# H2muller/CROPSR

Hardware: NVIDIA B200
Metric: genome Gbp/s scanned+scored (higher is better)
Workload: dtype f64

## Files before the change

### cropsr_b200/csrc/cropsr_b200.cu

```cuda

#include <cuda_runtime.h>
#include <stdint.h>
#include <stdio.h>
#include <stdarg.h>
#include <string.h>
#include <stdlib.h>
#include <algorithm>
#include <atomic>
#include <mutex>
#include <new>
#include <type_traits>
#include <utility>
#include <vector>

#include "../../include/cropsr_b200.h"

#ifndef CRP_CTAS_PER_SM
#define CRP_CTAS_PER_SM 4
#endif
#include "scan.cuh"
#include "primers.cuh"
#include "extras.cuh"
#include "offtarget.cuh"

#define CRP_ABI_VERSION 10

static constexpr size_t kScanSmemFixed = (size_t)kStages * kRecBytes + 2 * (size_t)kListCap * sizeof(uint16_t);

static thread_local char g_err[512] = "";
static int fail(int code, const char *fmt, ...) {
    va_list ap;
    va_start(ap, fmt);
    vsnprintf(g_err, sizeof g_err, fmt, ap);
    va_end(ap);
    return code;
}
#define CUDA_TRY(expr)                                                                      \
    do {                                                                                    \
        cudaError_t e_ = (expr);                                                            \
        if (e_ != cudaSuccess)                                                              \
            return fail(CRP_ERR_CUDA, "%s failed: %s (%s:%d)", #expr, cudaGetErrorString(e_), \
                        __FILE__, __LINE__);                                                \
    } while (0)

struct Context {
    bool ready = false;
    int device = -1;
    int sm_count = 0;
    cudaStream_t stream = nullptr;
    cudaStream_t lanes[3] = {nullptr, nullptr, nullptr};
    cudaStream_t lane_out = nullptr;
    std::atomic<uint64_t> launches{0};
    double *d_tables = nullptr;
    unsigned int *d_fault = nullptr;
};
static Context g_ctx;

struct Perf {
    std::atomic<uint64_t> commits{0}, scans{0}, sharded_scans{0}, fused_exchanges{0}, capacity_reruns{0};
    std::atomic<uint64_t> positions{0}, candidates{0}, h2d_bytes{0}, d2h_bytes{0}, cache_hits{0}, cache_misses{0};
    double ms_h2d = 0, ms_pack = 0, ms_scan = 0, ms_kernel = 0;
};
static Perf g_perf;

struct Segment {
    uint32_t token_id;
    const uint8_t *token;
    uint64_t token_len, begin, end;
    uint64_t stage_begin, stage_end;
    uint32_t first_tile, n_tiles;
    const uint8_t *raw = nullptr;
    uint64_t raw_bytes = 0;
    uint32_t width = 0, last = 0;
    uint64_t ascii_off = 0;
};

struct crp_genome {
    std::vector<Segment> segs;
    cudaStream_t st = nullptr;
    cudaEvent_t ev[3] = {nullptr, nullptr, nullptr};
    bool committed = false;
    uint64_t n_positions = 0;
    uint4 *records = nullptr;
    unsigned char *pam = nullptr;
    TileHdr *hdr = nullptr;
    uint32_t n_tiles = 0;
    uint32_t *d_seg_first = nullptr, *d_seg_count = nullptr;
    float ms_h2d = 0.f, ms_pack = 0.f;
    uint8_t *d_ascii = nullptr;
    bool fasta = false;
    unsigned int *h_bad = nullptr;
};

struct crp_result {
    const crp_genome *g = nullptr;
    cudaStream_t st = nullptr;
    cudaEvent_t ev[3] = {nullptr, nullptr, nullptr};
    cudaEvent_t ev_kernel = nullptr;
    unsigned long long *h_counts = nullptr;
    uint32_t stride = 0;
    unsigned long long *d_gather = nullptr;
    unsigned long long *h_gather = nullptr;
    bool fused = false;
    uint32_t epoch = 0;
    unsigned int *h_xchg_error = nullptr;
    float ms_kernel = 0.f;
    int guide_len = 0;
    uint32_t flags = 0;
    uint64_t capacity = 0;
    uint64_t n_plus = 0, n_minus = 0;
    bool scored = false;
    uint32_t *pos[2] = {nullptr, nullptr};
    unsigned long long *packed[2] = {nullptr, nullptr};
    double *x[2] = {nullptr, nullptr};
    unsigned char *state = nullptr;
    size_t state_bytes = 0, zero_offset = 0;
    unsigned long long *d_counts = nullptr;
    std::vector<uint64_t> seg_plus, seg_minus;
    float ms_scan = 0.f;
    uint32_t n_launches = 0;
};

#include <chrono>
struct Trace {
    const char *what;
    bool on;
    std::chrono::steady_clock::time_point t0;
    explicit Trace(const char *w) : what(w), on(getenv("CRP_TRACE") != nullptr), t0(std::chrono::steady_clock::now()) {}
    void lap(const char *stage) {
        if (!on) return;
        const auto t1 = std::chrono::steady_clock::now();
        fprintf(stderr, "[crp] %s: %s %.3f ms\n", what, stage, std::chrono::duration<double, std::milli>(t1 - t0).count());
        t0 = t1;
    }
};

static int need_ctx() {
    if (!g_ctx.ready) return fail(CRP_ERR_STATE, "crp_init has not been called");
    return 0;
}

struct DevBlock {
    void *ptr;
    size_t bytes;
    cudaEvent_t ev;
};
static std::vector<DevBlock> g_dev_free;
static std::vector<DevBlock> g_dev_live;
static std::mutex g_mem_mu;
template <typename T>
static cudaError_t dev_alloc(T **ptr, size_t bytes, cudaStream_t st) {
    std::lock_guard<std::mutex> lock(g_mem_mu);
    const size_t want = (bytes ? bytes : 16) + 255 & ~(size_t)255;
    size_t best = g_dev_free.size(), busy = g_dev_free.size();
    for (size_t i = 0; i < g_dev_free.size(); ++i) {
        const size_t b = g_dev_free[i].bytes;
        if (b < want || b - want > want / 8 + 4096) continue;
        if (cudaEventQuery(g_dev_free[i].ev) == cudaSuccess) {
            best = i;
            break;
        } else {
            cudaGetLastError();
            if (busy == g_dev_free.size() || b < g_dev_free[busy].bytes) busy = i;
        }
    }
    DevBlock blk;
    if (best < g_dev_free.size()) {
        blk = g_dev_free[best];
        g_dev_free.erase(g_dev_free.begin() + best);
        g_perf.cache_hits++;
    } else if (cudaMalloc(&blk.ptr, want) == cudaSuccess) {
        g_perf.cache_misses++;
        blk.bytes = want;
        if (cudaError_t e = cudaEventCreateWithFlags(&blk.ev, cudaEventDisableTiming)) {
            cudaFree(blk.ptr);
            return e;
        }
    } else if (busy < g_dev_free.size()) {
        cudaGetLastError();
        blk = g_dev_free[busy];
        g_dev_free.erase(g_dev_free.begin() + busy);
        if (cudaError_t e = cudaStreamWaitEvent(st, blk.ev, 0)) return e;
    } else {
        cudaGetLastError();
        blk.bytes = want;
        if (cudaMalloc(&blk.ptr, want) != cudaSuccess) {
            cudaGetLastError();
            cudaDeviceSynchronize();
            for (DevBlock &b : g_dev_free) {
                cudaFree(b.ptr);
                cudaEventDestroy(b.ev);
            }
            g_dev_free.clear();
            if (cudaError_t e = cudaMalloc(&blk.ptr, want)) return e;
        }
        if (cudaError_t e = cudaEventCreateWithFlags(&blk.ev, cudaEventDisableTiming)) {
            cudaFree(blk.ptr);
            return e;
        }
    }
    g_dev_live.push_back(blk);
    *ptr = reinterpret_cast<T *>(blk.ptr);
    return cudaSuccess;
}
static void dev_free(void *ptr, cudaStream_t st) {
    if (!ptr) return;
    std::lock_guard<std::mutex> lock(g_mem_mu);
    for (size_t i = g_dev_live.size(); i-- > 0;)
        if (g_dev_live[i].ptr == ptr) {
            DevBlock blk = g_dev_live[i];
            g_dev_live.erase(g_dev_live.begin() + i);
            cudaEventRecord(blk.ev, st);
            g_dev_free.push_back(blk);
            return;
        }
}
static void dev_cache_release() {
    std::lock_guard<std::mutex> lock(g_mem_mu);
    for (DevBlock &b : g_dev_free) {
        cudaFree(b.ptr);
        cudaEventDestroy(b.ev);
    }
    g_dev_free.clear();
}

static std::vector<std::pair<size_t, void *>> g_pinned_free;
static void *pinned_get(size_t bytes) {
    std::lock_guard<std::mutex> lock(g_mem_mu);
    for (size_t i = 0; i < g_pinned_free.size(); ++i)
        if (g_pinned_free[i].first >= bytes) {
            void *p = g_pinned_free[i].second;
            g_pinned_free.erase(g_pinned_free.begin() + i);
            return p;
        }
    const size_t want = bytes < 4096 ? 4096 : bytes;
    void *p = nullptr;
    if (cudaHostAlloc(&p, want + sizeof(size_t) * 2, cudaHostAllocMapped) != cudaSuccess) return nullptr;
    *reinterpret_cast<size_t *>(p) = want;
    return reinterpret_cast<char *>(p) + sizeof(size_t) * 2;
}
static void pinned_put(void *p) {
    if (!p) return;
    std::lock_guard<std::mutex> lock(g_mem_mu);
    const size_t cap = *reinterpret_cast<size_t *>(reinterpret_cast<char *>(p) - sizeof(size_t) * 2);
    g_pinned_free.emplace_back(cap, p);
}


#include <dlfcn.h>
#include <nccl.h>
struct Comm {
    void *dl = nullptr;
    ncclComm_t comm = nullptr;
    int rank = 0, world = 1;
    ncclResult_t (*GetUniqueId)(ncclUniqueId *) = nullptr;
    ncclResult_t (*CommInitRank)(ncclComm_t *, int, ncclUniqueId, int) = nullptr;
    ncclResult_t (*CommDestroy)(ncclComm_t) = nullptr;
    ncclResult_t (*AllGather)(const void *, void *, size_t, ncclDataType_t, ncclComm_t, cudaStream_t) = nullptr;
    ncclResult_t (*AllReduce)(const void *, void *, size_t, ncclDataType_t, ncclRedOp_t, ncclComm_t, cudaStream_t) = nullptr;
    const char *(*GetErrorString)(ncclResult_t) = nullptr;
    unsigned long long *d_scratch = nullptr;
    unsigned char *xchg = nullptr;
    unsigned char *peer[kMaxPeers] = {};
    bool fused = false;
    int mode = 0;
    uint32_t epoch = 0;
    char why_not_fused[160] = "";
};
static Comm g_comm;
static constexpr uint32_t kXchgSlots = 32768;
static size_t xchg_gather_bytes() { return (size_t)2 * kMaxPeers * 2 * kXchgSlots * sizeof(unsigned long long); }
static size_t xchg_bytes() { return xchg_gather_bytes() + 2 * kMaxPeers * sizeof(unsigned int) + 64; }
static unsigned long long *xchg_gather(unsigned char *base, uint32_t parity, uint32_t world, uint32_t stride) {
    (void)world;
    (void)stride;
    return reinterpret_cast<unsigned long long *>(base) + (size_t)parity * kMaxPeers * 2 * kXchgSlots;
}
static unsigned int *xchg_flags(unsigned char *base, uint32_t parity) {
    return reinterpret_cast<unsigned int *>(base + xchg_gather_bytes()) + (size_t)parity * kMaxPeers;
}
static unsigned int *xchg_error(unsigned char *base) {
    return reinterpret_cast<unsigned int *>(base + xchg_gather_bytes()) + 2 * kMaxPeers;
}

static int comm_load() {
    if (g_comm.dl) return 0;
    const char *names[] = {getenv("CRP_NCCL_LIB"), "libnccl.so.2", "libnccl.so"};
    for (const char *n : names) {
        if (!n) continue;
        if ((g_comm.dl = dlopen(n, RTLD_NOW | RTLD_GLOBAL))) break;
    }
    if (!g_comm.dl) return fail(CRP_ERR_STATE, "libnccl.so.2 not found: %s", dlerror());
#define CRP_NCCL_SYM(field, name)                                                         \
    if (!(*(void **)(&g_comm.field) = dlsym(g_comm.dl, name))) {                          \
        dlclose(g_comm.dl);                                                               \
        g_comm.dl = nullptr;                                                              \
        return fail(CRP_ERR_STATE, "NCCL symbol %s missing", name);                       \
    }
    CRP_NCCL_SYM(GetUniqueId, "ncclGetUniqueId")
    CRP_NCCL_SYM(CommInitRank, "ncclCommInitRank")
    CRP_NCCL_SYM(CommDestroy, "ncclCommDestroy")
    CRP_NCCL_SYM(AllGather, "ncclAllGather")
    CRP_NCCL_SYM(AllReduce, "ncclAllReduce")
    CRP_NCCL_SYM(GetErrorString, "ncclGetErrorString")
#undef CRP_NCCL_SYM
    return 0;
}
#define NCCL_TRY(expr)                                                                                \
    do {                                                                                              \
        ncclResult_t e_ = (expr);                                                                     \
        if (e_ != ncclSuccess) return fail(CRP_ERR_CUDA, "%s failed: %s", #expr, g_comm.GetErrorString(e_)); \
    } while (0)

static int comm_allgather_u64(const unsigned long long *send, unsigned long long *recv, size_t count, cudaStream_t st) {
    if (!g_comm.comm) return fail(CRP_ERR_STATE, "crp_comm_init has not been called");
    NCCL_TRY(g_comm.AllGather(send, recv, count, ncclUint64, g_comm.comm, st));
    return 0;
}

extern "C" {

int crp_result_free(crp_result *r);
int crp_comm_shutdown(void);


int crp_abi_version(void) { return CRP_ABI_VERSION; }

int crp_tile_size(void) { return kTile; }

int crp_checked_build(void) {
#ifdef CRP_CHECKED
    return 1;
#else
    return 0;
#endif
}

const char *crp_last_error(void) { return g_err; }

int crp_debug_set_times(void *dev_ptr) {
    unsigned long long *p = (unsigned long long *)dev_ptr;
    CUDA_TRY(cudaMemcpyToSymbol(g_dbg_times, &p, sizeof p));
    return 0;
}

int crp_device_count(int *count) {
    if (!count) return fail(CRP_ERR_ARG, "count is NULL");
    CUDA_TRY(cudaGetDeviceCount(count));
    return 0;
}

int crp_init(int device) {
    if (g_ctx.ready) {
        if (g_ctx.device == device) return 0;
        return fail(CRP_ERR_STATE, "already initialised on device %d", g_ctx.device);
    }
    CUDA_TRY(cudaSetDevice(device));
    cudaDeviceProp prop;
    CUDA_TRY(cudaGetDeviceProperties(&prop, device));
    if (prop.major != 10)
        return fail(CRP_ERR_CUDA, "device %d is sm_%d%d; this library is built for sm_100a only", device,
                    prop.major, prop.minor);
    CUDA_TRY(cudaStreamCreateWithFlags(&g_ctx.stream, cudaStreamNonBlocking));
    {
        std::vector<double> tab;
        char msg[128];
        if (build_rs1_tables(tab, msg, sizeof msg)) return fail(CRP_ERR_STATE, "%s", msg);
        CUDA_TRY(cudaMalloc(&g_ctx.d_tables, tab.size() * sizeof(double)));
        CUDA_TRY(cudaMemcpy(g_ctx.d_tables, tab.data(), tab.size() * sizeof(double), cudaMemcpyHostToDevice));
    }
#ifdef CRP_CHECKED
    CUDA_TRY(cudaMalloc(&g_ctx.d_fault, sizeof(unsigned int)));
    CUDA_TRY(cudaMemset(g_ctx.d_fault, 0, sizeof(unsigned int)));
#endif
    g_ctx.device = device;
    g_ctx.sm_count = prop.multiProcessorCount;
    g_ctx.launches = 0;
    g_ctx.ready = true;
    return 0;
}

int crp_shutdown(void) {
    if (!g_ctx.ready) return 0;
    crp_comm_shutdown();
    cudaStreamSynchronize(g_ctx.stream);
    cudaDeviceSynchronize();
    dev_cache_release();
    {
        std::lock_guard<std::mutex> lock(g_mem_mu);
        for (auto &pf : g_pinned_free) cudaFreeHost(reinterpret_cast<char *>(pf.second) - sizeof(size_t) * 2);
        g_pinned_free.clear();
    }
    cudaStreamDestroy(g_ctx.stream);
    for (cudaStream_t l : g_ctx.lanes)
        if (l) cudaStreamDestroy(l);
    if (g_ctx.lane_out) cudaStreamDestroy(g_ctx.lane_out);
    cudaFree(g_ctx.d_tables);
    if (g_ctx.d_fault) cudaFree(g_ctx.d_fault);
    g_ctx.d_fault = nullptr;
    g_ctx.ready = false;
    g_ctx.device = -1;
    g_ctx.stream = nullptr;
    for (cudaStream_t &l : g_ctx.lanes) l = nullptr;
    g_ctx.lane_out = nullptr;
    g_ctx.d_tables = nullptr;
    g_ctx.launches = 0;
    return 0;
}

int crp_perf_report(char *buf, uint64_t capacity, uint64_t *needed) {
    char tmp[1536];
    size_t live = 0, idle = 0, live_bytes = 0, idle_bytes = 0;
    {
        std::lock_guard<std::mutex> lock(g_mem_mu);
        live = g_dev_live.size();
        idle = g_dev_free.size();
        for (const DevBlock &b : g_dev_live) live_bytes += b.bytes;
        for (const DevBlock &b : g_dev_free) idle_bytes += b.bytes;
    }
    const int n = snprintf(
        tmp, sizeof tmp,
        "{\"abi\": %d, \"checked_build\": %d, \"device\": %d, \"sm_count\": %d, \"kernel_launches\": %llu, "
        "\"commits\": %llu, \"scans\": %llu, \"sharded_scans\": %llu, \"fused_exchanges\": %llu, \"capacity_reruns\": %llu, "
        "\"positions_packed\": %llu, \"candidates\": %llu, \"h2d_token_bytes\": %llu, \"d2h_row_bytes\": %llu, "
        "\"ms_h2d\": %.4f, \"ms_pack\": %.4f, \"ms_scan\": %.4f, \"ms_scan_kernels\": %.4f, "
        "\"comm\": {\"rank\": %d, \"world\": %d, \"fused_exchange\": %s}, "
        "\"block_cache\": {\"live_blocks\": %zu, \"live_bytes\": %zu, \"idle_blocks\": %zu, \"idle_bytes\": %zu, \"hits\": %llu, \"misses\": %llu}}",
        CRP_ABI_VERSION, crp_checked_build(), g_ctx.device, g_ctx.sm_count, (unsigned long long)g_ctx.launches.load(),
        (unsigned long long)g_perf.commits.load(), (unsigned long long)g_perf.scans.load(),
        (unsigned long long)g_perf.sharded_scans.load(), (unsigned long long)g_perf.fused_exchanges.load(),
        (unsigned long long)g_perf.capacity_reruns.load(), (unsigned long long)g_perf.positions.load(),
        (unsigned long long)g_perf.candidates.load(), (unsigned long long)g_perf.h2d_bytes.load(),
        (unsigned long long)g_perf.d2h_bytes.load(), g_perf.ms_h2d, g_perf.ms_pack, g_perf.ms_scan, g_perf.ms_kernel,
        g_comm.comm ? g_comm.rank : 0, g_comm.comm ? g_comm.world : 1, g_comm.comm && g_comm.fused && g_comm.mode == 0 ? "true" : "false",
        live, live_bytes, idle, idle_bytes, (unsigned long long)g_perf.cache_hits.load(), (unsigned long long)g_perf.cache_misses.load());
    if (needed) *needed = (uint64_t)n + 1;
    if (!buf || capacity < (uint64_t)n + 1) return fail(CRP_ERR_RANGE, "perf report needs %d bytes", n + 1);
    memcpy(buf, tmp, (size_t)n + 1);
    return 0;
}

int crp_launch_count(uint64_t *n) {
    if (!n) return fail(CRP_ERR_ARG, "n is NULL");
    *n = g_ctx.launches;
    return 0;
}

int crp_comm_unique_id(uint8_t *id) {
    if (!id) return fail(CRP_ERR_ARG, "id is NULL");
    if (int rc = comm_load()) return rc;
    ncclUniqueId u;
    NCCL_TRY(g_comm.GetUniqueId(&u));
    static_assert(sizeof u == CRP_COMM_ID_BYTES, "ncclUniqueId size");
    memcpy(id, &u, sizeof u);
    return 0;
}

int crp_comm_init(int rank, int world, const uint8_t *id) {
    if (int rc = need_ctx()) return rc;
    if (!id || world < 1 || rank < 0 || rank >= world) return fail(CRP_ERR_ARG, "bad rank %d / world %d", rank, world);
    if (g_comm.comm) return fail(CRP_ERR_STATE, "communicator already initialised (rank %d of %d)", g_comm.rank, g_comm.world);
    if (int rc = comm_load()) return rc;
    ncclUniqueId u;
    memcpy(&u, id, sizeof u);
    CUDA_TRY(cudaSetDevice(g_ctx.device));
    NCCL_TRY(g_comm.CommInitRank(&g_comm.comm, world, u, rank));
    g_comm.rank = rank;
    g_comm.world = world;
    CUDA_TRY(cudaMalloc(&g_comm.d_scratch, 2 * sizeof(unsigned long long)));
    CUDA_TRY(cudaMemset(g_comm.d_scratch, 0, 2 * sizeof(unsigned long long)));
    g_comm.epoch = 0;
    g_comm.mode = 0;
    if (const char *e = getenv("CRP_COMM_EXCHANGE")) g_comm.mode = !strcmp(e, "nccl") ? 1 : 0;
    g_comm.fused = false;
    g_comm.why_not_fused[0] = 0;
    bool ok = world <= kMaxPeers;
    if (!ok) snprintf(g_comm.why_not_fused, sizeof g_comm.why_not_fused, "world %d > %d", world, kMaxPeers);
    cudaIpcMemHandle_t mine;
    memset(&mine, 0, sizeof mine);
    if (ok) {
        if (cudaMalloc(&g_comm.xchg, xchg_bytes()) != cudaSuccess || cudaMemset(g_comm.xchg, 0, xchg_bytes()) != cudaSuccess ||
            cudaIpcGetMemHandle(&mine, g_comm.xchg) != cudaSuccess) {
            snprintf(g_comm.why_not_fused, sizeof g_comm.why_not_fused, "exchange buffer / IPC handle: %s",
                     cudaGetErrorString(cudaGetLastError()));
            ok = false;
        }
    }
    static_assert(sizeof(cudaIpcMemHandle_t) == 64, "IPC handle size");
    std::vector<uint64_t> handles((size_t)world * 8);
    {
        unsigned long long *d = nullptr;
        CUDA_TRY(cudaMalloc(&d, ((size_t)world + 1) * 64));
        CUDA_TRY(cudaMemcpy(d, &mine, 64, cudaMemcpyHostToDevice));
        NCCL_TRY(g_comm.AllGather(d, d + 8, 8, ncclUint64, g_comm.comm, g_ctx.stream));
        CUDA_TRY(cudaStreamSynchronize(g_ctx.stream));
        CUDA_TRY(cudaMemcpy(handles.data(), d + 8, (size_t)world * 64, cudaMemcpyDeviceToHost));
        cudaFree(d);
    }
    for (int q = 0; q < world && ok; ++q) {
        if (q == rank) {
            g_comm.peer[q] = g_comm.xchg;
            continue;
        }
        cudaIpcMemHandle_t h;
        memcpy(&h, &handles[(size_t)q * 8], 64);
        void *ptr = nullptr;
        if (cudaIpcOpenMemHandle(&ptr, h, cudaIpcMemLazyEnablePeerAccess) != cudaSuccess) {
            snprintf(g_comm.why_not_fused, sizeof g_comm.why_not_fused, "cudaIpcOpenMemHandle(rank %d): %s", q,
                     cudaGetErrorString(cudaGetLastError()));
            ok = false;
        } else {
            g_comm.peer[q] = static_cast<unsigned char *>(ptr);
        }
    }
    {
        unsigned long long v = ok ? 0ull : 1ull;
        CUDA_TRY(cudaMemcpy(g_comm.d_scratch, &v, sizeof v, cudaMemcpyHostToDevice));
        NCCL_TRY(g_comm.AllReduce(g_comm.d_scratch, g_comm.d_scratch + 1, 1, ncclUint64, ncclSum, g_comm.comm, g_ctx.stream));
        CUDA_TRY(cudaStreamSynchronize(g_ctx.stream));
        CUDA_TRY(cudaMemcpy(&v, g_comm.d_scratch + 1, sizeof v, cudaMemcpyDeviceToHost));
        CUDA_TRY(cudaMemset(g_comm.d_scratch, 0, 2 * sizeof(unsigned long long)));
        if (v && ok) snprintf(g_comm.why_not_fused, sizeof g_comm.why_not_fused, "%llu other rank(s) could not map the buffers", v);
        g_comm.fused = v == 0;
    }
    return 0;
}

int crp_comm_set_exchange(int mode) {
    if (mode != 0 && mode != 1) return fail(CRP_ERR_ARG, "mode must be 0 (fused) or 1 (nccl)");
    g_comm.mode = mode;
    return 0;
}

int crp_comm_exchange_info(int *fused, const char **why) {
    if (fused) *fused = g_comm.comm && g_comm.fused && g_comm.mode == 0 ? 1 : 0;
    if (why) *why = g_comm.mode == 1 ? "NCCL exchange selected" : g_comm.why_not_fused;
    return 0;
}

int crp_comm_info(int *rank, int *world) {
    if (rank) *rank = g_comm.comm ? g_comm.rank : 0;
    if (world) *world = g_comm.comm ? g_comm.world : 1;
    return 0;
}

int crp_comm_barrier(void) {
    if (int rc = need_ctx()) return rc;
    CUDA_TRY(cudaDeviceSynchronize());
    if (!g_comm.comm) return 0;
    NCCL_TRY(g_comm.AllReduce(g_comm.d_scratch, g_comm.d_scratch + 1, 1, ncclUint64, ncclSum, g_comm.comm, g_ctx.stream));
    CUDA_TRY(cudaStreamSynchronize(g_ctx.stream));
    return 0;
}

int crp_comm_max_f64(double *v, uint32_t n) {
    if (int rc = need_ctx()) return rc;
    if (!v && n) return fail(CRP_ERR_ARG, "v is NULL");
    if (!g_comm.comm || n == 0) return 0;
    double *d = nullptr;
    CUDA_TRY(dev_alloc(&d, n * sizeof(double), g_ctx.stream));
    CUDA_TRY(cudaMemcpyAsync(d, v, n * sizeof(double), cudaMemcpyHostToDevice, g_ctx.stream));
    NCCL_TRY(g_comm.AllReduce(d, d, n, ncclDouble, ncclMax, g_comm.comm, g_ctx.stream));
    CUDA_TRY(cudaMemcpyAsync(v, d, n * sizeof(double), cudaMemcpyDeviceToHost, g_ctx.stream));
    CUDA_TRY(cudaStreamSynchronize(g_ctx.stream));
    dev_free(d, g_ctx.stream);
    return 0;
}

int crp_comm_sum_f64(double *v, uint32_t n) {
    if (int rc = need_ctx()) return rc;
    if (!v && n) return fail(CRP_ERR_ARG, "v is NULL");
    if (!g_comm.comm || n == 0) return 0;
    double *d = nullptr;
    CUDA_TRY(dev_alloc(&d, n * sizeof(double), g_ctx.stream));
    CUDA_TRY(cudaMemcpyAsync(d, v, n * sizeof(double), cudaMemcpyHostToDevice, g_ctx.stream));
    NCCL_TRY(g_comm.AllReduce(d, d, n, ncclDouble, ncclSum, g_comm.comm, g_ctx.stream));
    CUDA_TRY(cudaMemcpyAsync(v, d, n * sizeof(double), cudaMemcpyDeviceToHost, g_ctx.stream));
    CUDA_TRY(cudaStreamSynchronize(g_ctx.stream));
    dev_free(d, g_ctx.stream);
    return 0;
}

int crp_comm_allgather_u64(const uint64_t *in, uint32_t n, uint64_t *out) {
    if (int rc = need_ctx()) return rc;
    if (n && (!in || !out)) return fail(CRP_ERR_ARG, "NULL argument");
    if (n == 0) return 0;
    if (!g_comm.comm) {
        memcpy(out, in, n * sizeof(uint64_t));
        return 0;
    }
    unsigned long long *d = nullptr;
    const size_t w = (size_t)g_comm.world;
    CUDA_TRY(dev_alloc(&d, (w + 1) * n * sizeof(uint64_t), g_ctx.stream));
    CUDA_TRY(cudaMemcpyAsync(d, in, n * sizeof(uint64_t), cudaMemcpyHostToDevice, g_ctx.stream));
    if (int rc = comm_allgather_u64(d, d + n, n, g_ctx.stream)) {
        dev_free(d, g_ctx.stream);
        return rc;
    }
    CUDA_TRY(cudaMemcpyAsync(out, d + n, w * n * sizeof(uint64_t), cudaMemcpyDeviceToHost, g_ctx.stream));
    CUDA_TRY(cudaStreamSynchronize(g_ctx.stream));
    dev_free(d, g_ctx.stream);
    return 0;
}

int crp_link_probe(uint64_t h2d_bytes, uint64_t d2h_bytes, uint32_t reps, float *ms) {
    if (int rc = need_ctx()) return rc;
    if (!ms || !reps) return fail(CRP_ERR_ARG, "bad argument");
    void *h_in = nullptr, *h_out = nullptr;
    unsigned char *d_in = nullptr, *d_out = nullptr;
    cudaStream_t s2 = nullptr;
    int rc = 0;
    do {
        if (cudaHostAlloc(&h_in, h2d_bytes + 16, cudaHostAllocDefault) != cudaSuccess ||
            cudaHostAlloc(&h_out, d2h_bytes + 16, cudaHostAllocDefault) != cudaSuccess) {
            rc = fail(CRP_ERR_NOMEM, "cudaHostAlloc of the probe buffers failed");
            break;
        }
        memset(h_in, 1, h2d_bytes + 16);
        memset(h_out, 1, d2h_bytes + 16);
        if (dev_alloc(&d_in, h2d_bytes + 16, g_ctx.stream) != cudaSuccess || dev_alloc(&d_out, d2h_bytes + 16, g_ctx.stream) != cudaSuccess ||
            cudaStreamCreateWithFlags(&s2, cudaStreamNonBlocking) != cudaSuccess) {
            rc = fail(CRP_ERR_NOMEM, "device buffers of the link probe failed");
            break;
        }
        cudaStreamSynchronize(g_ctx.stream);
        double total = 0.0;
        for (uint32_t i = 0; i <= reps; ++i) {
            const auto t0 = std::chrono::steady_clock::now();
            cudaMemcpyAsync(d_in, h_in, h2d_bytes, cudaMemcpyHostToDevice, g_ctx.stream);
            cudaMemcpyAsync(h_out, d_out, d2h_bytes, cudaMemcpyDeviceToHost, s2);
            cudaStreamSynchronize(g_ctx.stream);
            cudaStreamSynchronize(s2);
            if (i) total += std::chrono::duration<double, std::milli>(std::chrono::steady_clock::now() - t0).count();
        }
        if (cudaGetLastError() != cudaSuccess) rc = fail(CRP_ERR_CUDA, "link probe copies failed");
        *ms = (float)(total / reps);
    } while (0);
    if (s2) cudaStreamDestroy(s2);
    dev_free(d_in, g_ctx.stream);
    dev_free(d_out, g_ctx.stream);
    if (h_in) cudaFreeHost(h_in);
    if (h_out) cudaFreeHost(h_out);
    return rc;
}

int crp_comm_shutdown(void) {
    if (g_comm.comm) {
        cudaDeviceSynchronize();
        g_comm.AllReduce(g_comm.d_scratch, g_comm.d_scratch + 1, 1, ncclUint64, ncclSum, g_comm.comm, g_ctx.stream);
        cudaStreamSynchronize(g_ctx.stream);
        for (int q = 0; q < g_comm.world && q < kMaxPeers; ++q)
            if (g_comm.peer[q] && q != g_comm.rank) cudaIpcCloseMemHandle(g_comm.peer[q]);
        for (auto &pp : g_comm.peer) pp = nullptr;
        if (g_comm.xchg) cudaFree(g_comm.xchg);
        g_comm.xchg = nullptr;
        g_comm.fused = false;
        g_comm.CommDestroy(g_comm.comm);
        cudaFree(g_comm.d_scratch);
        g_comm.comm = nullptr;
        g_comm.d_scratch = nullptr;
        g_comm.rank = 0;
        g_comm.world = 1;
    }
    return 0;
}

int crp_flush_l2(void) {
    if (int rc = need_ctx()) return rc;
    unsigned char *buf = nullptr;
    const size_t bytes = 512ull << 20;
    CUDA_TRY(dev_alloc(&buf, bytes, g_ctx.stream));
    cudaError_t e = cudaMemsetAsync(buf, 0, bytes, g_ctx.stream);
    dev_free(buf, g_ctx.stream);
    CUDA_TRY(e);
    CUDA_TRY(cudaStreamSynchronize(g_ctx.stream));
    return 0;
}

int crp_device_synchronize(void) {
    if (int rc = need_ctx()) return rc;
    CUDA_TRY(cudaDeviceSynchronize());
    return 0;
}

int crp_host_alloc(void **ptr, uint64_t bytes) {
    if (!ptr) return fail(CRP_ERR_ARG, "ptr is NULL");
    if (int rc = need_ctx()) return rc;
    CUDA_TRY(cudaHostAlloc(ptr, bytes ? bytes : 1, cudaHostAllocDefault));
    return 0;
}

int crp_host_free(void *ptr) {
    if (ptr) CUDA_TRY(cudaFreeHost(ptr));
    return 0;
}

static cudaStream_t stream_of(const crp_genome *g) { return g->st ? g->st : g_ctx.stream; }

int crp_genome_new(crp_genome **g) {
    if (!g) return fail(CRP_ERR_ARG, "g is NULL");
    if (int rc = need_ctx()) return rc;
    *g = new (std::nothrow) crp_genome();
    if (!*g) return fail(CRP_ERR_NOMEM, "out of host memory");
    return 0;
}

int crp_genome_add_segment(crp_genome *g, uint32_t token_id, const uint8_t *token_ascii,
                           uint64_t token_len, uint64_t seg_begin, uint64_t seg_end) {
    if (!g) return fail(CRP_ERR_ARG, "g is NULL");
    if (g->committed) return fail(CRP_ERR_STATE, "genome already committed");
    if (!token_ascii && token_len) return fail(CRP_ERR_ARG, "token_ascii is NULL");
    if (seg_begin > seg_end || seg_end > token_len)
        return fail(CRP_ERR_ARG, "segment [%llu,%llu) outside token of length %llu",
                    (unsigned long long)seg_begin, (unsigned long long)seg_end, (unsigned long long)token_len);
    if (seg_begin % kAlign) return fail(CRP_ERR_ARG, "seg_begin must be a multiple of %u", kAlign);
    if (token_len >= (1ull << 31) - (1ull << 15))
        return fail(CRP_ERR_RANGE, "token of %llu positions exceeds the 31-bit position range",
                    (unsigned long long)token_len);
    Segment s{};
    s.token_id = token_id;
    s.token = token_ascii;
    s.token_len = token_len;
    s.begin = seg_begin;
    s.end = seg_end;
    g->segs.push_back(s);
    return 0;
}

int crp_genome_add_fasta_record(crp_genome *g, uint32_t token_id, const uint8_t *seq_bytes, uint64_t n_bytes,
                                uint32_t line_width, int last_record) {
    if (!g) return fail(CRP_ERR_ARG, "g is NULL");
    if (g->committed) return fail(CRP_ERR_STATE, "genome already committed");
    if (!seq_bytes || !n_bytes || !line_width) return fail(CRP_ERR_FORMAT, "empty FASTA record");
    const uint64_t body = seq_bytes[n_bytes - 1] == '\n' ? n_bytes - 1 : n_bytes;
    const uint64_t k = body / ((uint64_t)line_width + 1), r = body % ((uint64_t)line_width + 1);
    if (r == 0) return fail(CRP_ERR_FORMAT, "FASTA record is not made of %u-base lines", line_width);
    const uint64_t n_bases = k * line_width + r, token_len = n_bases + 4;
    if (token_len >= (1ull << 31) - (1ull << 15))
        return fail(CRP_ERR_RANGE, "token of %llu positions exceeds the 31-bit position range",
                    (unsigned long long)token_len);
    Segment s{};
    s.token_id = token_id;
    s.token = nullptr;
    s.token_len = token_len;
    s.begin = 0;
    s.end = token_len;
    s.raw = seq_bytes;
    s.raw_bytes = n_bytes;
    s.width = line_width;
    s.last = last_record ? 1u : 0u;
    g->segs.push_back(s);
    g->fasta = true;
    return 0;
}

int crp_genome_token_length(const crp_genome *g, uint32_t segment, uint64_t *token_len) {
    if (!g || !token_len) return fail(CRP_ERR_ARG, "NULL argument");
    if (segment >= g->segs.size()) return fail(CRP_ERR_ARG, "segment %u out of range", segment);
    *token_len = g->segs[segment].token_len;
    return 0;
}

int crp_genome_fetch_token(const crp_genome *g, uint32_t segment, uint8_t *dst, uint64_t capacity) {
    if (!g || !dst) return fail(CRP_ERR_ARG, "NULL argument");
    if (int rc = need_ctx()) return rc;
    if (!g->committed || !g->d_ascii) return fail(CRP_ERR_STATE, "the genome keeps no tokens on the device");
    if (segment >= g->segs.size()) return fail(CRP_ERR_ARG, "segment %u out of range", segment);
    const Segment &s = g->segs[segment];
    if (!s.raw) return fail(CRP_ERR_STATE, "segment %u was not ingested from FASTA bytes", segment);
    if (capacity < s.token_len) return fail(CRP_ERR_RANGE, "token needs %llu bytes", (unsigned long long)s.token_len);
    cudaStream_t st = g->st ? g->st : g_ctx.stream;
    CUDA_TRY(cudaMemcpyAsync(dst, g->d_ascii + s.ascii_off, s.token_len, cudaMemcpyDeviceToHost, st));
    CUDA_TRY(cudaStreamSynchronize(st));
    return 0;
}

int crp_genome_release_tokens(crp_genome *g) {
    if (!g) return fail(CRP_ERR_ARG, "g is NULL");
    dev_free(g->d_ascii, g->st ? g->st : g_ctx.stream);
    g->d_ascii = nullptr;
    return 0;
}

int crp_genome_num_segments(const crp_genome *g, uint32_t *n) {
    if (!g || !n) return fail(CRP_ERR_ARG, "NULL argument");
    *n = (uint32_t)g->segs.size();
    return 0;
}

int crp_genome_num_positions(const crp_genome *g, uint64_t *n) {
    if (!g || !n) return fail(CRP_ERR_ARG, "NULL argument");
    *n = g->n_positions;
    return 0;
}

static int commit_enqueue(crp_genome *g) {
    cudaStream_t st = stream_of(g);
    const bool one = g->segs.size() == 1;
    std::vector<PackDesc> descs;
    std::vector<uint64_t> seg_ascii;
    std::vector<uint32_t> seg_first, seg_count;
    uint64_t ascii_bytes = 0, n_tiles = 0;
    g->n_positions = 0;
    for (size_t si = 0; si < g->segs.size(); ++si) {
        Segment &s = g->segs[si];
        s.stage_begin = s.begin >= 32 ? s.begin - 32 : 0;
        s.stage_end = s.end + 32 < s.token_len ? s.end + 32 : s.token_len;
        seg_ascii.push_back(ascii_bytes);
        s.first_tile = (uint32_t)n_tiles;
        s.n_tiles = (uint32_t)((s.end - s.begin + kTile - 1) / kTile);
        n_tiles += s.n_tiles;
        if (n_tiles >= (1ull << 31)) return fail(CRP_ERR_RANGE, "shard has too many tiles");
        for (uint32_t j = 0; j < (one ? (s.n_tiles ? 1u : 0u) : s.n_tiles); ++j) {
            const uint64_t t = s.begin + (uint64_t)j * kTile;
            PackDesc pd;
            pd.ascii_off = ascii_bytes;
            pd.stage_begin = (uint32_t)s.stage_begin;
            pd.stage_end = (uint32_t)s.stage_end;
            pd.td.t_start = (uint32_t)t;
            pd.td.L = (uint32_t)s.token_len;
            pd.td.n = (uint32_t)((s.end - t) < (uint64_t)kTile ? (s.end - t) : (uint64_t)kTile);
            pd.td.segment = (uint32_t)si;
            descs.push_back(pd);
        }
        seg_first.push_back(s.first_tile);
        seg_count.push_back(s.n_tiles);
        g->n_positions += s.end - s.begin;
        ascii_bytes += (s.stage_end - s.stage_begin + 15) / 16 * 16;
    }
    if (g->n_positions >= (1ull << 32))
        return fail(CRP_ERR_RANGE, "shard of %llu positions exceeds the 32-bit candidate count range",
                    (unsigned long long)g->n_positions);
    g->n_tiles = (uint32_t)n_tiles;
    g_perf.commits++;
    g_perf.positions += g->n_positions;
    g_perf.h2d_bytes += ascii_bytes;

    uint8_t *d_ascii = nullptr;
    PackDesc *d_descs = nullptr;
    const size_t rec_bytes = (size_t)g->n_tiles * kRecBytes;
    if (dev_alloc(&d_ascii, ascii_bytes + 64, st) != cudaSuccess ||
        (!one && dev_alloc(&d_descs, (descs.size() + 1) * sizeof(PackDesc), st) != cudaSuccess) ||
        dev_alloc(&g->records, rec_bytes + 16, st) != cudaSuccess ||
        dev_alloc(&g->pam, (size_t)g->n_tiles * kPamBytes + 16, st) != cudaSuccess ||
        dev_alloc(&g->hdr, ((size_t)g->n_tiles + 1) * sizeof(TileHdr), st) != cudaSuccess) {
        cudaGetLastError();
        dev_free(d_ascii, st);
        dev_free(d_descs, st);
        return fail(CRP_ERR_NOMEM, "cudaMalloc of %llu record bytes + %llu staging bytes failed",
                    (unsigned long long)rec_bytes, (unsigned long long)ascii_bytes);
    }
    for (int i = 0; i < 3; ++i)
        if (!g->ev[i]) CUDA_TRY(cudaEventCreate(&g->ev[i]));
    CUDA_TRY(cudaEventRecord(g->ev[0], st));
    uint8_t *d_raw = nullptr;
    FastaRec *d_recs = nullptr;
    unsigned int *d_bad = nullptr;
    std::vector<FastaRec> frecs;
    uint64_t raw_total = 0, strip_items = 0;
    for (size_t si = 0; si < g->segs.size(); ++si) {
        Segment &s = g->segs[si];
        s.ascii_off = seg_ascii[si];
        if (!s.raw) continue;
        FastaRec fr{};
        fr.raw_off = raw_total;
        fr.ascii_off = seg_ascii[si];
        fr.first_item = strip_items;
        fr.n_bases = (uint32_t)(s.token_len - 4);
        fr.width = s.width;
        fr.last = s.last;
        frecs.push_back(fr);
        raw_total += (s.raw_bytes + 15) / 16 * 16;
        strip_items += (s.token_len + 15) / 16;
    }
    if (!frecs.empty()) {
        if (dev_alloc(&d_raw, raw_total + 64, st) != cudaSuccess ||
            dev_alloc(&d_recs, frecs.size() * sizeof(FastaRec), st) != cudaSuccess ||
            dev_alloc(&d_bad, sizeof(unsigned int), st) != cudaSuccess) {
            cudaGetLastError();
            return fail(CRP_ERR_NOMEM, "cudaMalloc of %llu FASTA bytes failed", (unsigned long long)raw_total);
        }
        CUDA_TRY(cudaMemsetAsync(d_bad, 0, sizeof(unsigned int), st));
    }
    for (size_t si = 0, fi = 0; si < g->segs.size(); ++si) {
        const Segment &s = g->segs[si];
        if (s.raw) {
            CUDA_TRY(cudaMemcpyAsync(d_raw + frecs[fi++].raw_off, s.raw, s.raw_bytes, cudaMemcpyHostToDevice, st));
        } else if (s.stage_end > s.stage_begin && s.n_tiles) {
            CUDA_TRY(cudaMemcpyAsync(d_ascii + seg_ascii[si], s.token + s.stage_begin, s.stage_end - s.stage_begin,
                                     cudaMemcpyHostToDevice, st));
        }
    }
    if (!frecs.empty()) {
        CUDA_TRY(cudaMemcpyAsync(d_recs, frecs.data(), frecs.size() * sizeof(FastaRec), cudaMemcpyHostToDevice, st));
        const uint64_t want = (strip_items + 255) / 256, cap = (uint64_t)g_ctx.sm_count * 16;
        k_fasta_strip<<<(unsigned)(want < cap ? want : cap), 256, 0, st>>>(d_raw, d_recs, (uint32_t)frecs.size(),
                                                                           strip_items, d_ascii, d_bad);
        g_ctx.launches++;
        CUDA_TRY(cudaGetLastError());
        if (!g->h_bad) g->h_bad = static_cast<unsigned int *>(pinned_get(sizeof(unsigned int)));
        if (!g->h_bad) return fail(CRP_ERR_NOMEM, "cudaHostAlloc failed");
        *g->h_bad = 0;
        CUDA_TRY(cudaMemcpyAsync(g->h_bad, d_bad, sizeof(unsigned int), cudaMemcpyDeviceToHost, st));
        dev_free(d_raw, st);
        dev_free(d_recs, st);
        dev_free(d_bad, st);
    }
    if (!one && !descs.empty())
        CUDA_TRY(cudaMemcpyAsync(d_descs, descs.data(), descs.size() * sizeof(PackDesc), cudaMemcpyHostToDevice, st));
    CUDA_TRY(cudaEventRecord(g->ev[1], st));
    const uint64_t n_items = (uint64_t)g->n_tiles * kPackItems;
    if (n_items) {
        PackDesc first = descs[0];
        if (one) first.td.n = (uint32_t)(g->segs[0].end - g->segs[0].begin);
        const uint64_t want = (n_items + 255) / 256, cap = (uint64_t)g_ctx.sm_count * 16;
        CUDA_TRY(cudaMemsetAsync(g->hdr, 0, (size_t)g->n_tiles * sizeof(TileHdr), st));
        k_pack<<<(unsigned)(want < cap ? want : cap), 256, 0, st>>>(d_ascii, d_descs, first, n_items, g->records, g->pam, g->hdr);
        g_ctx.launches++;
        CUDA_TRY(cudaGetLastError());
    }
    CUDA_TRY(cudaEventRecord(g->ev[2], st));
    if (!one && !g->segs.empty()) {
        const size_t nb = g->segs.size() * sizeof(uint32_t);
        CUDA_TRY(dev_alloc(&g->d_seg_first, nb, st));
        CUDA_TRY(dev_alloc(&g->d_seg_count, nb, st));
        CUDA_TRY(cudaMemcpyAsync(g->d_seg_first, seg_first.data(), nb, cudaMemcpyHostToDevice, st));
        CUDA_TRY(cudaMemcpyAsync(g->d_seg_count, seg_count.data(), nb, cudaMemcpyHostToDevice, st));
    }
    if (g->fasta) g->d_ascii = d_ascii;
    else dev_free(d_ascii, st);
    dev_free(d_descs, st);
    g->committed = true;
    return 0;
}

int crp_genome_commit(crp_genome *g) {
    if (!g) return fail(CRP_ERR_ARG, "g is NULL");
    if (int rc = need_ctx()) return rc;
    if (g->committed) return fail(CRP_ERR_STATE, "genome already committed");
    Trace tr("commit");
    if (int rc = commit_enqueue(g)) return rc;
    tr.lap("enqueue");
    CUDA_TRY(cudaStreamSynchronize(stream_of(g)));
    tr.lap("sync");
    CUDA_TRY(cudaEventElapsedTime(&g->ms_h2d, g->ev[0], g->ev[1]));
    CUDA_TRY(cudaEventElapsedTime(&g->ms_pack, g->ev[1], g->ev[2]));
    g_perf.ms_h2d += g->ms_h2d;
    g_perf.ms_pack += g->ms_pack;
    for (Segment &s : g->segs) s.token = nullptr;
    if (g->h_bad && *g->h_bad)
        return fail(CRP_ERR_FORMAT, "a FASTA record is not plain fixed-width text; use the host ingest for this file");
    return 0;
}

int crp_genome_timing(const crp_genome *g, float *ms_h2d, float *ms_pack) {
    if (!g) return fail(CRP_ERR_ARG, "g is NULL");
    if (ms_h2d) *ms_h2d = g->ms_h2d;
    if (ms_pack) *ms_pack = g->ms_pack;
    return 0;
}

int crp_genome_free(crp_genome *g) {
    if (!g) return 0;
    cudaStream_t st = stream_of(g);
    dev_free(g->records, st);
    dev_free(g->pam, st);
    dev_free(g->hdr, st);
    dev_free(g->d_ascii, st);
    pinned_put(g->h_bad);
    dev_free(g->d_seg_first, st);
    dev_free(g->d_seg_count, st);
    for (cudaEvent_t e : g->ev)
        if (e) cudaEventDestroy(e);
    delete g;
    return 0;
}

static void free_streams(crp_result *r) {
    for (int s = 0; s < 2; ++s) {
        dev_free(r->pos[s], r->st);
        dev_free(r->packed[s], r->st);
        dev_free(r->x[s], r->st);
        r->pos[s] = nullptr;
        r->packed[s] = nullptr;
        r->x[s] = nullptr;
    }
}

static int alloc_streams(crp_result *r, uint64_t cap, bool scored) {
    r->capacity = cap;
    const uint64_t n = cap ? cap : 1;
    for (int s = 0; s < 2; ++s) {
        if (dev_alloc(&r->pos[s], n * sizeof(uint32_t), r->st) != cudaSuccess) goto oom;
        if (scored) {
            if (dev_alloc(&r->packed[s], n * sizeof(unsigned long long), r->st) != cudaSuccess) goto oom;
            if (dev_alloc(&r->x[s], n * sizeof(double), r->st) != cudaSuccess) goto oom;
        }
    }
    return 0;
oom:
    cudaGetLastError();
    free_streams(r);
    return fail(CRP_ERR_NOMEM, "cudaMalloc of candidate streams (%llu entries per strand) failed",
                (unsigned long long)cap);
}

struct ScanPlan {
    const void *fn;
    unsigned grid, threads;
    size_t smem;
};

static int plan_scan(const crp_genome *g, bool scored, ScanPlan *p) {
    p->threads = kThreads;
    p->fn = scored ? (const void *)k_scan_score<true> : (const void *)k_scan_score<false>;
    const unsigned grid_max = (unsigned)g_ctx.sm_count * CRP_CTAS_PER_SM;
    p->smem = kScanSmemFixed + (size_t)grid_max * sizeof(unsigned long long);
    static_assert(kScanSmemFixed >= (size_t)kHdrBatch * sizeof(TileHdr), "the count phase stages its tile headers in the emit phase's tile slots");
    static int per_sm_cache[2] = {0, 0};
    int &per_sm = per_sm_cache[scored ? 1 : 0];
    if (per_sm == 0) {
        CUDA_TRY(cudaFuncSetAttribute(p->fn, cudaFuncAttributeMaxDynamicSharedMemorySize, (int)p->smem));
        CUDA_TRY(cudaOccupancyMaxActiveBlocksPerMultiprocessor(&per_sm, p->fn, kThreads, p->smem));
        if (per_sm < 1) return fail(CRP_ERR_CUDA, "scan kernel does not fit on an SM");
        if (per_sm > CRP_CTAS_PER_SM) per_sm = CRP_CTAS_PER_SM;
    }
    uint64_t grid = (uint64_t)g_ctx.sm_count * per_sm;
    if (const char *e = getenv("CRP_SCAN_GRID")) {
        const long v = atol(e);
        if (v > 0 && (uint64_t)v < grid) grid = (uint64_t)v;
    }
    if (grid > g->n_tiles) grid = g->n_tiles;
    if (grid < 1) grid = 1;
    p->grid = (unsigned)grid;
    return 0;
}

static int launch_scan(const crp_genome *g, crp_result *r, const ScanPlan &p) {
    cudaStream_t st = r->st;
    ScanArgs a;
    a.records = g->records;
    a.pam = g->pam;
    a.hdr = g->hdr;
    a.n_tiles = g->n_tiles;
    a.static_eighths = 4;
    if (const char *e = getenv("CRP_STATIC_EIGHTHS")) a.static_eighths = (uint32_t)atoi(e) > 8 ? 8 : (uint32_t)atoi(e);
    a.guide_len = r->guide_len;
    a.flags = r->flags;
    a.tables = g_ctx.d_tables;
    a.capacity = r->capacity < 0xFFFFFFFFull ? r->capacity : 0xFFFFFFFFull;
    a.pos_plus = r->pos[0];
    a.pos_minus = r->pos[1];
    a.packed_plus = r->packed[0];
    a.packed_minus = r->packed[1];
    a.x_plus = r->x[0];
    a.x_minus = r->x[1];
    const uint32_t n_seg = (uint32_t)g->segs.size();
    unsigned long long *s64 = reinterpret_cast<unsigned long long *>(r->state);
    a.warp_pref = s64;
    a.cta_tot = s64 + (size_t)g->n_tiles * kPrefWords;
    a.seg_counts = r->d_counts;
    a.tickets = reinterpret_cast<unsigned int *>(r->d_counts + 2 * (size_t)r->stride);
    a.n_seg = n_seg;
    a.seg_stride = r->stride;
    a.seg_first_tile = g->d_seg_first;
    a.seg_tile_count = g->d_seg_count;
    a.seg_counts_host = r->h_counts;
    a.fault = g_ctx.d_fault;
    a.world = 1;
    a.rank = 0;
    a.epoch = 0;
    a.xchg_error = nullptr;
    a.xchg_timeout_ns = 20ull * 1000 * 1000 * 1000;
    for (int q = 0; q < kMaxPeers; ++q) {
        a.peer_gather[q] = nullptr;
        a.peer_flags[q] = nullptr;
    }
    const unsigned long long *gathered = r->d_gather;
    if (r->fused) {
        a.world = (uint32_t)g_comm.world;
        a.rank = (uint32_t)g_comm.rank;
        a.epoch = r->epoch;
        a.xchg_error = xchg_error(g_comm.xchg);
        if (const char *e = getenv("CRP_XCHG_TIMEOUT_MS")) a.xchg_timeout_ns = strtoull(e, nullptr, 10) * 1000000ull;
        for (int q = 0; q < g_comm.world; ++q) {
            a.peer_gather[q] = xchg_gather(g_comm.peer[q], r->epoch & 1u, a.world, r->stride);
            a.peer_flags[q] = xchg_flags(g_comm.peer[q], r->epoch & 1u);
        }
        gathered = xchg_gather(g_comm.xchg, r->epoch & 1u, a.world, r->stride);
    }
    CUDA_TRY(cudaEventRecord(r->ev[0], st));
    if (g->n_tiles) {
        void *params[] = {(void *)&a};
        CUDA_TRY(cudaLaunchCooperativeKernel(p.fn, dim3(p.grid), dim3(p.threads), params, p.smem, st));
        g_ctx.launches++;
        CUDA_TRY(cudaGetLastError());
    } else if (r->fused) {
        k_exchange_empty<<<1, 256, 0, st>>>(a);
        g_ctx.launches++;
        CUDA_TRY(cudaGetLastError());
    } else if (r->stride) {
        CUDA_TRY(cudaMemsetAsync(r->d_counts, 0, 2 * (size_t)r->stride * sizeof(unsigned long long), st));
        memset(r->h_counts, 0, 2 * (size_t)r->stride * sizeof(unsigned long long));
    }
    if (r->ev_kernel) CUDA_TRY(cudaEventRecord(r->ev_kernel, st));
    if (r->d_gather && !r->fused) {
        if (int rc = comm_allgather_u64(r->d_counts, r->d_gather, 2 * (size_t)r->stride, st)) return rc;
    }
    CUDA_TRY(cudaEventRecord(r->ev[1], st));
    if (r->h_gather && gathered)
        CUDA_TRY(cudaMemcpyAsync(r->h_gather, gathered, (size_t)g_comm.world * 2 * r->stride * sizeof(unsigned long long),
                                 cudaMemcpyDeviceToHost, st));
    if (r->fused)
        CUDA_TRY(cudaMemcpyAsync(r->h_xchg_error, xchg_error(g_comm.xchg), sizeof(unsigned int), cudaMemcpyDeviceToHost, st));
    CUDA_TRY(cudaEventRecord(r->ev[2], st));
    return 0;
}

static int scan_enqueue(crp_genome *g, int guide_len, uint32_t flags, crp_result **res, uint32_t slots = 0) {
    crp_result *r = new (std::nothrow) crp_result();
    if (!r) return fail(CRP_ERR_NOMEM, "out of host memory");
    r->g = g;
    r->st = stream_of(g);
    r->guide_len = guide_len;
    r->flags = flags;
    r->scored = guide_len == 20 && !(flags & CRP_SCAN_NO_SCORE);
    const uint32_t n_seg = (uint32_t)g->segs.size();
    int rc = 0;
    auto bail = [&](int code) {
        crp_result_free(r);
        return code;
    };
    ScanPlan plan = {};
    if ((rc = plan_scan(g, r->scored, &plan))) return bail(rc);
    r->stride = slots ? slots : n_seg;
    r->zero_offset = ((size_t)g->n_tiles * kPrefWords + (size_t)plan.grid) * sizeof(unsigned long long);
    r->state_bytes = r->zero_offset + 2 * (size_t)r->stride * sizeof(unsigned long long) +
                     4 * sizeof(unsigned int);
    if (dev_alloc(&r->state, r->state_bytes, r->st) != cudaSuccess)
        return bail(fail(CRP_ERR_NOMEM, "cudaMalloc of scan state failed"));
    r->d_counts = reinterpret_cast<unsigned long long *>(r->state + r->zero_offset);
    r->h_counts = static_cast<unsigned long long *>(pinned_get((2 * (size_t)r->stride + 1) * sizeof(unsigned long long)));
    if (!r->h_counts) return bail(fail(CRP_ERR_NOMEM, "cudaHostAlloc of the counts failed"));
    if (slots) {
        const size_t gb = (size_t)g_comm.world * 2 * slots * sizeof(unsigned long long);
        r->fused = g_comm.fused && g_comm.mode == 0 && slots <= kXchgSlots;
        r->epoch = ++g_comm.epoch;
        if (r->fused) {
            r->h_xchg_error = static_cast<unsigned int *>(pinned_get(sizeof(unsigned int)));
            if (!r->h_xchg_error) return bail(fail(CRP_ERR_NOMEM, "cudaHostAlloc failed"));
            *r->h_xchg_error = 0;
        }
        if (dev_alloc(&r->d_gather, gb, r->st) != cudaSuccess)
            return bail(fail(CRP_ERR_NOMEM, "cudaMalloc of the gathered counts failed"));
        r->h_gather = static_cast<unsigned long long *>(pinned_get(gb));
        if (!r->h_gather) return bail(fail(CRP_ERR_NOMEM, "cudaHostAlloc of the gathered counts failed"));
        if (cudaEventCreate(&r->ev_kernel) != cudaSuccess) return bail(fail(CRP_ERR_CUDA, "cudaEventCreate failed"));
    }
    if (cudaEventCreate(&r->ev[0]) != cudaSuccess || cudaEventCreate(&r->ev[1]) != cudaSuccess ||
        cudaEventCreateWithFlags(&r->ev[2], cudaEventDisableTiming) != cudaSuccess)
        return bail(fail(CRP_ERR_CUDA, "cudaEventCreate failed"));
    if ((rc = alloc_streams(r, g->n_positions / 8 + 4096, r->scored))) return bail(rc);
    if ((rc = launch_scan(g, r, plan))) return bail(rc);
    *res = r;
    return 0;
}

static int scan_finish(crp_genome *g, crp_result *r, cudaStream_t post = nullptr) {
    const uint32_t n_seg = (uint32_t)g->segs.size();
    for (int attempt = 0; attempt < 2; ++attempt) {
        if (cudaError_t e = cudaEventSynchronize(r->ev[2]))
            return fail(CRP_ERR_CUDA, "scan kernels failed: %s", cudaGetErrorString(e));
        r->n_plus = r->n_minus = 0;
        r->seg_plus.assign(n_seg, 0);
        r->seg_minus.assign(n_seg, 0);
        for (uint32_t s = 0; s < n_seg; ++s) {
            r->seg_plus[s] = r->h_counts[s];
            r->seg_minus[s] = r->h_counts[r->stride + s];
            r->n_plus += r->seg_plus[s];
            r->n_minus += r->seg_minus[s];
        }
        {
            float ms = 0.f;
            cudaEventElapsedTime(&ms, r->ev[0], r->ev[1]);
            r->ms_scan += ms;
            if (r->ev_kernel) cudaEventElapsedTime(&ms, r->ev[0], r->ev_kernel);
            r->ms_kernel += ms;
            r->n_launches++;
        }
#ifdef CRP_CHECKED
        {
            unsigned int fault = 0;
            cudaMemcpy(&fault, g_ctx.d_fault, sizeof fault, cudaMemcpyDeviceToHost);
            if (fault) {
                cudaMemset(g_ctx.d_fault, 0, sizeof fault);
                return fail(CRP_ERR_STATE, "checked build: kernel invariant %u violated (scan.cuh:%u)", fault & 0xFFu, fault >> 8);
            }
        }
#endif
        if (r->fused && *r->h_xchg_error)
            return fail(CRP_ERR_CUDA, "sharded scan: the counts of rank %u did not arrive (peer not scanning?)", *r->h_xchg_error - 1);
        const uint64_t need = r->n_plus > r->n_minus ? r->n_plus : r->n_minus;
        if (need <= r->capacity) break;
        if (attempt == 1) return fail(CRP_ERR_STATE, "candidate streams overflowed twice");
        r->fused = false;
        if (r->d_gather) {
            dev_free(r->d_gather, r->st);
            r->d_gather = nullptr;
        }
        free_streams(r);
        if (int rc = alloc_streams(r, need, r->scored)) return rc;
        ScanPlan plan = {};
        if (int rc = plan_scan(g, r->scored, &plan)) return rc;
        if (int rc = launch_scan(g, r, plan)) return rc;
    }
    g_perf.scans++;
    if (r->stride != (uint32_t)g->segs.size() || r->h_gather) g_perf.sharded_scans++;
    if (r->epoch && g_comm.fused && g_comm.mode == 0) g_perf.fused_exchanges++;
    g_perf.capacity_reruns += r->n_launches - 1;
    g_perf.candidates += r->n_plus + r->n_minus;
    g_perf.ms_scan += r->ms_scan;
    g_perf.ms_kernel += r->ms_kernel;
    if (r->scored && (r->flags & CRP_SCAN_LOGISTIC)) {
        const uint64_t n[2] = {r->n_plus, r->n_minus};
        for (int s = 0; s < 2; ++s)
            if (n[s]) {
                const uint64_t want = (n[s] + 255) / 256, cap = (uint64_t)g_ctx.sm_count * 16;
                k_logistic<<<(unsigned)(want < cap ? want : cap), 256, 0, post ? post : r->st>>>(r->x[s], n[s]);
                g_ctx.launches++;
            }
        CUDA_TRY(cudaGetLastError());
        CUDA_TRY(cudaEventRecord(r->ev[2], post ? post : r->st));
    }
    return 0;
}

int crp_scan_score(crp_genome *g, int guide_len, uint32_t flags, crp_result **res) {
    if (!g || !res) return fail(CRP_ERR_ARG, "NULL argument");
    if (int rc = need_ctx()) return rc;
    if (!g->committed) return fail(CRP_ERR_STATE, "genome not committed");
    if (guide_len < 1 || guide_len > 1000000) return fail(CRP_ERR_ARG, "guide_len %d out of range", guide_len);
    Trace tr("scan");
    crp_result *r = nullptr;
    if (int rc = scan_enqueue(g, guide_len, flags, &r)) return rc;
    tr.lap("enqueue");
    if (int rc = scan_finish(g, r)) {
        crp_result_free(r);
        return rc;
    }
    tr.lap("finish");
    *res = r;
    return 0;
}

int crp_scan_score_sharded(crp_genome *g, int guide_len, uint32_t flags, uint32_t slots, crp_result **res) {
    if (!g || !res) return fail(CRP_ERR_ARG, "NULL argument");
    if (int rc = need_ctx()) return rc;
    if (!g_comm.comm) return fail(CRP_ERR_STATE, "crp_comm_init has not been called");
    if (!g->committed) return fail(CRP_ERR_STATE, "genome not committed");
    if (guide_len < 1 || guide_len > 1000000) return fail(CRP_ERR_ARG, "guide_len %d out of range", guide_len);
    if (slots == 0 || slots < g->segs.size())
        return fail(CRP_ERR_ARG, "slots = %u is smaller than the %zu segments of this shard", slots, g->segs.size());
    crp_result *r = nullptr;
    if (int rc = scan_enqueue(g, guide_len, flags, &r, slots)) return rc;
    if (int rc = scan_finish(g, r)) {
        crp_result_free(r);
        return rc;
    }
    *res = r;
    return 0;
}

int crp_result_gathered_counts(const crp_result *res, uint64_t *counts) {
    if (!res || !counts) return fail(CRP_ERR_ARG, "NULL argument");
    if (!res->h_gather) return fail(CRP_ERR_STATE, "not the result of a sharded scan");
    memcpy(counts, res->h_gather, (size_t)g_comm.world * 2 * res->stride * sizeof(uint64_t));
    return 0;
}

static int rs1_rows(uint64_t n, const uint8_t *rows, const uint8_t *cls, double *score, int logistic);
int crp_rs1_score(uint64_t n, const uint8_t *rows, const uint8_t *cls, double *score) {
    return rs1_rows(n, rows, cls, score, 1);
}
int crp_rs1_preactivation(uint64_t n, const uint8_t *rows, const uint8_t *cls, double *x) {
    return rs1_rows(n, rows, cls, x, 0);
}
static int rs1_rows(uint64_t n, const uint8_t *rows, const uint8_t *cls, double *score, int logistic) {
    if (n && (!rows || !cls || !score)) return fail(CRP_ERR_ARG, "NULL argument");
    if (int rc = need_ctx()) return rc;
    if (!n) return 0;
    cudaStream_t st = g_ctx.stream;
    uint8_t *d_rows = nullptr;
    double *d_out = nullptr;
    if (dev_alloc(&d_rows, 31 * n, st) != cudaSuccess || dev_alloc(&d_out, n * sizeof(double), st) != cudaSuccess) {
        cudaGetLastError();
        dev_free(d_rows, st);
        return fail(CRP_ERR_NOMEM, "cudaMalloc for %llu rows failed", (unsigned long long)n);
    }
    CUDA_TRY(cudaMemcpyAsync(d_rows, rows, 30 * n, cudaMemcpyHostToDevice, st));
    CUDA_TRY(cudaMemcpyAsync(d_rows + 30 * n, cls, n, cudaMemcpyHostToDevice, st));
    k_rs1_rows<<<(unsigned)((n + 127) / 128), 128, 0, st>>>(d_rows, d_rows + 30 * n, n, d_out, logistic);
    g_ctx.launches++;
    CUDA_TRY(cudaGetLastError());
    CUDA_TRY(cudaMemcpyAsync(score, d_out, n * sizeof(double), cudaMemcpyDeviceToHost, st));
    dev_free(d_rows, st);
    dev_free(d_out, st);
    CUDA_TRY(cudaStreamSynchronize(st));
    return 0;
}

int crp_logistic(uint64_t n, const double *x, double *score) {
    if (n && (!x || !score)) return fail(CRP_ERR_ARG, "NULL argument");
    if (int rc = need_ctx()) return rc;
    if (!n) return 0;
    cudaStream_t st = g_ctx.stream;
    double *d = nullptr;
    if (dev_alloc(&d, n * sizeof(double), st) != cudaSuccess) {
        cudaGetLastError();
        return fail(CRP_ERR_NOMEM, "cudaMalloc of %llu doubles failed", (unsigned long long)n);
    }
    CUDA_TRY(cudaMemcpyAsync(d, x, n * sizeof(double), cudaMemcpyHostToDevice, st));
    const uint64_t want = (n + 255) / 256, cap = (uint64_t)g_ctx.sm_count * 16;
    k_logistic<<<(unsigned)(want < cap ? want : cap), 256, 0, st>>>(d, n);
    g_ctx.launches++;
    CUDA_TRY(cudaGetLastError());
    CUDA_TRY(cudaMemcpyAsync(score, d, n * sizeof(double), cudaMemcpyDeviceToHost, st));
    dev_free(d, st);
    CUDA_TRY(cudaStreamSynchronize(st));
    return 0;
}

int crp_result_totals(const crp_result *res, uint64_t *n_plus, uint64_t *n_minus) {
    if (!res) return fail(CRP_ERR_ARG, "res is NULL");
    if (n_plus) *n_plus = res->n_plus;
    if (n_minus) *n_minus = res->n_minus;
    return 0;
}

int crp_result_segment_counts(const crp_result *res, uint64_t *n_plus, uint64_t *n_minus) {
    if (!res) return fail(CRP_ERR_ARG, "res is NULL");
    for (size_t s = 0; s < res->seg_plus.size(); ++s) {
        if (n_plus) n_plus[s] = res->seg_plus[s];
        if (n_minus) n_minus[s] = res->seg_minus[s];
    }
    return 0;
}

int crp_result_device_counts(const crp_result *res, void **dev_ptr) {
    if (!res || !dev_ptr) return fail(CRP_ERR_ARG, "NULL argument");
    *dev_ptr = res->d_counts;
    return 0;
}

static int fetch_enqueue(const crp_result *res, int s, uint64_t first, uint64_t count, uint32_t *pos, uint64_t *packed,
                         double *x, cudaStream_t st = nullptr) {
    if (!st) st = res->st;
    g_perf.d2h_bytes += count * ((pos ? 4 : 0) + (packed ? 8 : 0) + (x ? 8 : 0));
    if (count) {
        if (pos) CUDA_TRY(cudaMemcpyAsync(pos, res->pos[s] + first, count * sizeof(uint32_t), cudaMemcpyDeviceToHost, st));
        if (packed)
            CUDA_TRY(cudaMemcpyAsync(packed, res->packed[s] + first, count * sizeof(uint64_t), cudaMemcpyDeviceToHost, st));
        if (x) CUDA_TRY(cudaMemcpyAsync(x, res->x[s] + first, count * sizeof(double), cudaMemcpyDeviceToHost, st));
    }
    return 0;
}

int crp_result_fetch(const crp_result *res, char strand, uint64_t first, uint64_t count, uint32_t *pos,
                     uint64_t *packed, double *x) {
    if (!res) return fail(CRP_ERR_ARG, "res is NULL");
    if (int rc = need_ctx()) return rc;
    if (strand != '+' && strand != '-') return fail(CRP_ERR_ARG, "strand must be '+' or '-'");
    const int s = strand == '+' ? 0 : 1;
    const uint64_t total = s == 0 ? res->n_plus : res->n_minus;
    if (first > total || count > total - first)
        return fail(CRP_ERR_ARG, "range [%llu,+%llu) outside stream of %llu candidates", (unsigned long long)first,
                    (unsigned long long)count, (unsigned long long)total);
    if ((packed || x) && !res->scored && count)
        return fail(CRP_ERR_STATE, "this result carries positions only (guide_len != 20 or CRP_SCAN_NO_SCORE)");
    if (int rc = fetch_enqueue(res, s, first, count, pos, packed, x)) return rc;
    CUDA_TRY(cudaStreamSynchronize(res->st));
    return 0;
}

int crp_result_timing(const crp_result *res, float *ms_scan) {
    if (!res) return fail(CRP_ERR_ARG, "res is NULL");
    if (ms_scan) *ms_scan = res->ms_scan;
    return 0;
}

int crp_result_timing_detail(const crp_result *res, float *ms_kernels, float *ms_total, uint32_t *n_launches) {
    if (!res) return fail(CRP_ERR_ARG, "res is NULL");
    if (ms_kernels) *ms_kernels = res->ms_kernel;
    if (ms_total) *ms_total = res->ms_scan;
    if (n_launches) *n_launches = res->n_launches;
    return 0;
}

int crp_result_free(crp_result *r) {
    if (!r) return 0;
    free_streams(r);
    dev_free(r->state, r->st);
    dev_free(r->d_gather, r->st);
    pinned_put(r->h_counts);
    pinned_put(r->h_gather);
    pinned_put(r->h_xchg_error);
    if (r->ev_kernel) cudaEventDestroy(r->ev_kernel);
    for (cudaEvent_t e : r->ev)
        if (e) cudaEventDestroy(e);
    delete r;
    return 0;
}

int crp_scan_segments(uint32_t n_segments, const crp_segment_desc *segments, int guide_len, uint32_t flags,
                      uint64_t capacity, uint32_t *pos_plus, uint64_t *packed_plus, double *x_plus,
                      uint32_t *pos_minus, uint64_t *packed_minus, double *x_minus, uint64_t *n_plus,
                      uint64_t *n_minus, float *ms_device) {
    if (int rc = need_ctx()) return rc;
    if (n_segments && (!segments || !n_plus || !n_minus)) return fail(CRP_ERR_ARG, "NULL argument");
    if (guide_len < 1 || guide_len > 1000000) return fail(CRP_ERR_ARG, "guide_len %d out of range", guide_len);
    const bool scored = guide_len == 20 && !(flags & CRP_SCAN_NO_SCORE);
    for (uint32_t k = 0; k < n_segments; ++k) n_plus[k] = n_minus[k] = 0;
    for (uint32_t k = 0; k < n_segments; ++k) {
        const crp_segment_desc &sd = segments[k];
        if (!sd.token && sd.token_len) return fail(CRP_ERR_ARG, "segment %u: token is NULL", k);
        if (sd.begin > sd.end || sd.end > sd.token_len)
            return fail(CRP_ERR_ARG, "segment %u: [%llu,%llu) outside token of length %llu", k,
                        (unsigned long long)sd.begin, (unsigned long long)sd.end, (unsigned long long)sd.token_len);
        if (sd.begin % kAlign) return fail(CRP_ERR_ARG, "segment %u: begin must be a multiple of %u", k, kAlign);
        if (sd.token_len >= (1ull << 31) - (1ull << 15))
            return fail(CRP_ERR_ARG, "segment %u: token of %llu positions exceeds the 31-bit position range", k,
                        (unsigned long long)sd.token_len);
    }
    constexpr int kLanes = 3;
    if (!g_ctx.lanes[0])
        for (int i = 0; i < kLanes; ++i) CUDA_TRY(cudaStreamCreateWithFlags(&g_ctx.lanes[i], cudaStreamNonBlocking));
    Trace tr("scan_segments");
    uint64_t piece_bytes = 32ull << 20;
    if (const char *e = getenv("CRP_PIECE_POSITIONS")) {
        const unsigned long long v = strtoull(e, nullptr, 10);
        if (v >= (unsigned long long)kTile) piece_bytes = v / kTile * kTile;
    }
    struct Piece {
        uint32_t seg;
        uint64_t begin, end;
    };
    std::vector<Piece> pieces;
    for (uint32_t k = 0; k < n_segments; ++k) {
        const uint64_t end = segments[k].end;
        uint64_t b0 = segments[k].begin;
        if (end <= b0) {
            pieces.push_back(Piece{k, b0, end});
            continue;
        }
        while (b0 < end) {
            uint64_t e0 = b0 + piece_bytes;
            if (e0 + piece_bytes / 4 >= end) e0 = end;
            pieces.push_back(Piece{k, b0, e0});
            b0 = e0;
        }
    }
    struct Group {
        uint32_t first, count;
        uint64_t bytes;
    };
    std::vector<Group> groups;
    for (uint32_t k = 0; k < (uint32_t)pieces.size(); ++k) {
        const uint64_t nb = pieces[k].end > pieces[k].begin ? pieces[k].end - pieces[k].begin : 0;
        if (groups.empty() || groups.back().bytes + nb > piece_bytes + piece_bytes / 4 || groups.back().count >= 4096)
            groups.push_back(Group{k, 0, 0});
        groups.back().count++;
        groups.back().bytes += nb;
    }
    const uint32_t n_groups = (uint32_t)groups.size();
    std::vector<crp_genome *> gs(n_groups, nullptr);
    std::vector<crp_result *> rs(n_groups, nullptr);
    int rc = 0;
    uint64_t off[2] = {0, 0};
    float ms = 0.f;
    bool overflow = false;
    constexpr uint64_t kAheadBytes = 512ull << 20;
    if (!g_ctx.lane_out) CUDA_TRY(cudaStreamCreateWithFlags(&g_ctx.lane_out, cudaStreamNonBlocking));
    auto finish = [&](uint32_t q) -> int {
        if (int e = scan_finish(gs[q], rs[q], g_ctx.lane_out)) return e;
        for (uint32_t j = 0; j < groups[q].count; ++j) {
            n_plus[pieces[groups[q].first + j].seg] += rs[q]->seg_plus[j];
            n_minus[pieces[groups[q].first + j].seg] += rs[q]->seg_minus[j];
        }
        ms += rs[q]->ms_scan;
        if (off[0] + rs[q]->n_plus > capacity || off[1] + rs[q]->n_minus > capacity) {
            overflow = true;
        } else {
            if (cudaError_t e = cudaStreamWaitEvent(g_ctx.lane_out, rs[q]->ev[2], 0))
                return fail(CRP_ERR_CUDA, "cudaStreamWaitEvent failed: %s", cudaGetErrorString(e));
            if (int e = fetch_enqueue(rs[q], 0, 0, rs[q]->n_plus, pos_plus ? pos_plus + off[0] : nullptr,
                                      scored && packed_plus ? packed_plus + off[0] : nullptr,
                                      scored && x_plus ? x_plus + off[0] : nullptr, g_ctx.lane_out)) return e;
            if (int e = fetch_enqueue(rs[q], 1, 0, rs[q]->n_minus, pos_minus ? pos_minus + off[1] : nullptr,
                                      scored && packed_minus ? packed_minus + off[1] : nullptr,
                                      scored && x_minus ? x_minus + off[1] : nullptr, g_ctx.lane_out)) return e;
        }
        off[0] += rs[q]->n_plus;
        off[1] += rs[q]->n_minus;
        return 0;
    };
    auto enqueue = [&](uint32_t q) -> int {
        if (int e = crp_genome_new(&gs[q])) return e;
        gs[q]->st = g_ctx.lanes[q % kLanes];
        for (uint32_t j = 0; j < groups[q].count; ++j) {
            const Piece &pc = pieces[groups[q].first + j];
            const crp_segment_desc &sd = segments[pc.seg];
            if (int e = crp_genome_add_segment(gs[q], sd.token_id, sd.token, sd.token_len, pc.begin, pc.end)) return e;
        }
        if (int e = commit_enqueue(gs[q])) return e;
        return scan_enqueue(gs[q], guide_len, flags, &rs[q]);
    };
    uint32_t next_enq = 0;
    uint64_t ahead = 0;
    for (uint32_t q = 0; q < n_groups && !rc; ++q) {
        while (!rc && next_enq < n_groups && (next_enq < q + 2 || ahead + groups[next_enq].bytes <= kAheadBytes)) {
            rc = enqueue(next_enq);
            ahead += groups[next_enq].bytes;
            ++next_enq;
        }
        tr.lap("enqueue");
        if (!rc) rc = finish(q);
        ahead -= groups[q].bytes;
        tr.lap("finish");
    }
    for (int i = 0; i < kLanes; ++i) cudaStreamSynchronize(g_ctx.lanes[i]);
    cudaStreamSynchronize(g_ctx.lane_out);
    tr.lap("drain");
    for (uint32_t q = 0; q < n_groups; ++q) {
        crp_result_free(rs[q]);
        crp_genome_free(gs[q]);
    }
    tr.lap("free");
    if (ms_device) *ms_device = ms;
    if (rc) return rc;
    if (overflow)
        return fail(CRP_ERR_RANGE, "arena capacity %llu rows per strand is too small: need %llu / %llu",
                    (unsigned long long)capacity, (unsigned long long)off[0], (unsigned long long)off[1]);
    return 0;
}

static int segment_rows(const crp_result *res, uint32_t segment, char strand, uint64_t *first, uint64_t *count) {
    if (strand != '+' && strand != '-') return fail(CRP_ERR_ARG, "strand must be '+' or '-'");
    const std::vector<uint64_t> &c = strand == '+' ? res->seg_plus : res->seg_minus;
    if (segment >= c.size()) return fail(CRP_ERR_ARG, "segment %u out of range", segment);
    uint64_t f = 0;
    for (uint32_t s = 0; s < segment; ++s) f += c[s];
    *first = f;
    *count = c[segment];
    return 0;
}

int crp_result_extras(const crp_result *res, uint32_t segment, char strand, uint32_t flank, uint8_t *gc,
                      uint8_t *flags, uint8_t *run, uint32_t *cut, uint32_t *flank_lo, uint32_t *flank_hi) {
    if (!res) return fail(CRP_ERR_ARG, "res is NULL");
    if (int rc = need_ctx()) return rc;
    if (res->guide_len != 20) return fail(CRP_ERR_STATE, "extras are defined for guide_len 20 (30-base windows) only");
    uint64_t first = 0, n = 0;
    if (int rc = segment_rows(res, segment, strand, &first, &n)) return rc;
    if (n == 0) return 0;
    const crp_genome *g = res->g;
    const Segment &sg = g->segs[segment];
    cudaStream_t st = res->st;
    const int s = strand == '+' ? 0 : 1;
    uint8_t *d8 = nullptr;
    uint32_t *d32 = nullptr;
    CUDA_TRY(dev_alloc(&d8, 3 * n, st));
    if (dev_alloc(&d32, 3 * n * sizeof(uint32_t), st) != cudaSuccess) {
        dev_free(d8, st);
        return fail(CRP_ERR_NOMEM, "cudaMalloc failed");
    }
    ExtrasArgs a;
    a.records = g->records;
    a.pos = res->pos[s] + first;
    a.n = n;
    a.first_tile = sg.first_tile;
    a.seg_begin = (uint32_t)sg.begin;
    a.L = (uint32_t)sg.token_len;
    a.flank = flank;
    a.minus = s;
    a.gc = d8;
    a.flags = d8 + n;
    a.run = d8 + 2 * n;
    a.cut = d32;
    a.flank_lo = d32 + n;
    a.flank_hi = d32 + 2 * n;
    k_extras<<<(unsigned)((n + 255) / 256), 256, 0, st>>>(a);
    g_ctx.launches++;
    int rc = 0;
    auto back = [&](void *dst, const void *src, size_t bytes) {
        if (dst && !rc && cudaMemcpyAsync(dst, src, bytes, cudaMemcpyDeviceToHost, st) != cudaSuccess)
            rc = fail(CRP_ERR_CUDA, "D2H of extras failed");
    };
    back(gc, a.gc, n);
    back(flags, a.flags, n);
    back(run, a.run, n);
    back(cut, a.cut, n * 4);
    back(flank_lo, a.flank_lo, n * 4);
    back(flank_hi, a.flank_hi, n * 4);
    if (!rc && cudaStreamSynchronize(st) != cudaSuccess)
        rc = fail(CRP_ERR_CUDA, "extras kernel failed: %s", cudaGetErrorString(cudaGetLastError()));
    dev_free(d8, st);
    dev_free(d32, st);
    return rc;
}

int crp_result_extras_strand(const crp_result *res, char strand, uint32_t flank, uint8_t *gc, uint8_t *flags,
                             uint8_t *run, uint32_t *cut, uint32_t *flank_lo, uint32_t *flank_hi) {
    if (!res) return fail(CRP_ERR_ARG, "res is NULL");
    if (int rc = need_ctx()) return rc;
    if (strand != '+' && strand != '-') return fail(CRP_ERR_ARG, "strand must be '+' or '-'");
    if (res->guide_len != 20) return fail(CRP_ERR_STATE, "extras are defined for guide_len 20 (30-base windows) only");
    const int s = strand == '+' ? 0 : 1;
    const uint64_t n = s == 0 ? res->n_plus : res->n_minus;
    if (n == 0) return 0;
    const crp_genome *g = res->g;
    const std::vector<uint64_t> &cnt = s == 0 ? res->seg_plus : res->seg_minus;
    cudaStream_t st = res->st;
    uint8_t *d8 = nullptr;
    uint32_t *d32 = nullptr;
    CUDA_TRY(dev_alloc(&d8, 3 * n, st));
    if (dev_alloc(&d32, 3 * n * sizeof(uint32_t), st) != cudaSuccess) {
        dev_free(d8, st);
        return fail(CRP_ERR_NOMEM, "cudaMalloc failed");
    }
    uint64_t first = 0;
    for (size_t sgi = 0; sgi < cnt.size(); ++sgi) {
        const uint64_t m = cnt[sgi];
        if (m) {
            const Segment &sg = g->segs[sgi];
            ExtrasArgs a;
            a.records = g->records;
            a.pos = res->pos[s] + first;
            a.n = m;
            a.first_tile = sg.first_tile;
            a.seg_begin = (uint32_t)sg.begin;
            a.L = (uint32_t)sg.token_len;
            a.flank = flank;
            a.minus = s;
            a.gc = d8 + first;
            a.flags = d8 + n + first;
            a.run = d8 + 2 * n + first;
            a.cut = d32 + first;
            a.flank_lo = d32 + n + first;
            a.flank_hi = d32 + 2 * n + first;
            k_extras<<<(unsigned)((m + 255) / 256), 256, 0, st>>>(a);
            g_ctx.launches++;
        }
        first += m;
    }
    int rc = 0;
    auto back = [&](void *dst, const void *src, size_t bytes) {
        if (dst && !rc && cudaMemcpyAsync(dst, src, bytes, cudaMemcpyDeviceToHost, st) != cudaSuccess)
            rc = fail(CRP_ERR_CUDA, "D2H of extras failed");
    };
    back(gc, d8, n);
    back(flags, d8 + n, n);
    back(run, d8 + 2 * n, n);
    back(cut, d32, n * 4);
    back(flank_lo, d32 + n, n * 4);
    back(flank_hi, d32 + 2 * n, n * 4);
    if (!rc && cudaStreamSynchronize(st) != cudaSuccess)
        rc = fail(CRP_ERR_CUDA, "extras kernels failed: %s", cudaGetErrorString(cudaGetLastError()));
    dev_free(d8, st);
    dev_free(d32, st);
    return rc;
}

int crp_result_annotate_strand(const crp_result *res, char strand, const uint64_t *iv_offset, const uint32_t *start,
                               const uint32_t *end, int32_t *feature) {
    if (!res) return fail(CRP_ERR_ARG, "res is NULL");
    if (int rc = need_ctx()) return rc;
    if (strand != '+' && strand != '-') return fail(CRP_ERR_ARG, "strand must be '+' or '-'");
    const int s = strand == '+' ? 0 : 1;
    const uint64_t n = s == 0 ? res->n_plus : res->n_minus;
    if (n == 0) return 0;
    if (!feature || !iv_offset) return fail(CRP_ERR_ARG, "NULL argument");
    const std::vector<uint64_t> &cnt = s == 0 ? res->seg_plus : res->seg_minus;
    const uint64_t n_iv = iv_offset[cnt.size()];
    if (n_iv && (!start || !end)) return fail(CRP_ERR_ARG, "NULL interval arrays");
    std::vector<uint32_t> host(3 * (size_t)n_iv + 1);
    for (size_t sgi = 0; sgi < cnt.size(); ++sgi) {
        uint32_t running = 0;
        if (iv_offset[sgi + 1] < iv_offset[sgi]) return fail(CRP_ERR_ARG, "iv_offset must not decrease");
        for (uint64_t j = iv_offset[sgi]; j < iv_offset[sgi + 1]; ++j) {
            if (j > iv_offset[sgi] && start[j] < start[j - 1]) return fail(CRP_ERR_ARG, "intervals must be sorted by start");
            if (end[j] < start[j]) return fail(CRP_ERR_ARG, "interval %llu has end < start", (unsigned long long)j);
            running = end[j] > running ? end[j] : running;
            host[j] = start[j];
            host[n_iv + j] = end[j];
            host[2 * (size_t)n_iv + j] = running;
        }
    }
    cudaStream_t st = res->st;
    uint32_t *d_iv = nullptr;
    int32_t *d_f = nullptr;
    CUDA_TRY(dev_alloc(&d_iv, host.size() * sizeof(uint32_t), st));
    if (dev_alloc(&d_f, n * sizeof(int32_t), st) != cudaSuccess) {
        dev_free(d_iv, st);
        return fail(CRP_ERR_NOMEM, "cudaMalloc failed");
    }
    int rc = 0;
    if (cudaMemcpyAsync(d_iv, host.data(), host.size() * sizeof(uint32_t), cudaMemcpyHostToDevice, st) != cudaSuccess)
        rc = fail(CRP_ERR_CUDA, "H2D of intervals failed");
    uint64_t first = 0;
    for (size_t sgi = 0; sgi < cnt.size() && !rc; ++sgi) {
        const uint64_t m = cnt[sgi];
        if (m) {
            const uint64_t o = iv_offset[sgi];
            k_annotate<<<(unsigned)((m + 255) / 256), 256, 0, st>>>(res->pos[s] + first, m, s, d_iv + o, d_iv + n_iv + o,
                                                                   d_iv + 2 * (size_t)n_iv + o,
                                                                   (uint32_t)(iv_offset[sgi + 1] - o), d_f + first);
            g_ctx.launches++;
        }
        first += m;
    }
    if (!rc && (cudaMemcpyAsync(feature, d_f, n * sizeof(int32_t), cudaMemcpyDeviceToHost, st) != cudaSuccess ||
                cudaStreamSynchronize(st) != cudaSuccess))
        rc = fail(CRP_ERR_CUDA, "annotate failed: %s", cudaGetErrorString(cudaGetLastError()));
    dev_free(d_iv, st);
    dev_free(d_f, st);
    return rc;
}

int crp_genome_other_runs(const crp_genome *g, uint32_t segment, uint32_t min_len, uint64_t capacity, uint32_t *start,
                          uint32_t *length, uint64_t *n_runs) {
    if (!g || !n_runs) return fail(CRP_ERR_ARG, "NULL argument");
    if (int rc = need_ctx()) return rc;
    if (!g->committed) return fail(CRP_ERR_STATE, "genome is not committed");
    if (segment >= g->segs.size()) return fail(CRP_ERR_ARG, "segment %u out of range", segment);
    if (capacity && (!start || !length)) return fail(CRP_ERR_ARG, "NULL output arrays");
    const Segment &sg = g->segs[segment];
    *n_runs = 0;
    if (!sg.n_tiles) return 0;
    cudaStream_t st = stream_of(g);
    uint32_t cap = 1u << 16;
    std::vector<uint32_t> hs, he;
    for (int attempt = 0; attempt < 2; ++attempt) {
        uint32_t *d = nullptr;
        unsigned int *d_n = nullptr;
        CUDA_TRY(dev_alloc(&d, 2 * (size_t)cap * sizeof(uint32_t), st));
        if (dev_alloc(&d_n, 2 * sizeof(unsigned int), st) != cudaSuccess) {
            dev_free(d, st);
            return fail(CRP_ERR_NOMEM, "cudaMalloc failed");
        }
        RunArgs a;
        a.records = g->records;
        a.first_tile = sg.first_tile;
        a.n_tiles = sg.n_tiles;
        a.seg_begin = (uint32_t)sg.begin;
        a.seg_end = (uint32_t)sg.end;
        a.starts = d;
        a.ends = d + cap;
        a.n_starts = d_n;
        a.n_ends = d_n + 1;
        a.capacity = cap;
        unsigned int n[2] = {0, 0};
        int rc = 0;
        const uint64_t items = (uint64_t)sg.n_tiles * kTileWords;
        if (cudaMemsetAsync(d_n, 0, 2 * sizeof(unsigned int), st) != cudaSuccess) rc = fail(CRP_ERR_CUDA, "memset failed");
        if (!rc) {
            k_other_runs<<<(unsigned)((items + 255) / 256), 256, 0, st>>>(a);
            g_ctx.launches++;
            if (cudaMemcpyAsync(n, d_n, sizeof n, cudaMemcpyDeviceToHost, st) != cudaSuccess || cudaStreamSynchronize(st) != cudaSuccess)
                rc = fail(CRP_ERR_CUDA, "run kernel failed: %s", cudaGetErrorString(cudaGetLastError()));
        }
        if (!rc && n[0] != n[1]) rc = fail(CRP_ERR_STATE, "run boundaries do not pair up (%u starts, %u ends)", n[0], n[1]);
        if (!rc && n[0] <= cap) {
            hs.resize(n[0]);
            he.resize(n[0]);
            if (n[0] && (cudaMemcpyAsync(hs.data(), a.starts, n[0] * sizeof(uint32_t), cudaMemcpyDeviceToHost, st) != cudaSuccess ||
                         cudaMemcpyAsync(he.data(), a.ends, n[0] * sizeof(uint32_t), cudaMemcpyDeviceToHost, st) != cudaSuccess ||
                         cudaStreamSynchronize(st) != cudaSuccess))
                rc = fail(CRP_ERR_CUDA, "D2H of run boundaries failed");
        }
        dev_free(d, st);
        dev_free(d_n, st);
        if (rc) return rc;
        if (n[0] <= cap) break;
        if (attempt == 1) return fail(CRP_ERR_RANGE, "more than %u runs in one segment", cap);
        cap = n[0];
    }
    std::sort(hs.begin(), hs.end());
    std::sort(he.begin(), he.end());
    uint64_t kept = 0;
    for (size_t i = 0; i < hs.size(); ++i) {
        const uint32_t len = he[i] - hs[i] + 1;
        if (len < min_len) continue;
        if (kept < capacity) {
            start[kept] = hs[i];
            length[kept] = len;
        }
        ++kept;
    }
    *n_runs = kept;
    if (kept > capacity) return fail(CRP_ERR_RANGE, "%llu runs, room for %llu", (unsigned long long)kept, (unsigned long long)capacity);
    return 0;
}

int crp_primer_windows(const crp_genome *g, uint64_t n, const uint32_t *segment, const uint32_t *lo, const uint32_t *hi,
                       const crp_primer_params *prm, uint32_t *n_fwd, uint32_t *n_rev, uint64_t *n_pairs,
                       uint16_t *first, uint8_t *status) {
    if (!g || !prm) return fail(CRP_ERR_ARG, "NULL argument");
    if (int rc = need_ctx()) return rc;
    if (!g->committed) return fail(CRP_ERR_STATE, "genome is not committed");
    if (n == 0) return 0;
    if (!segment || !lo || !hi) return fail(CRP_ERR_ARG, "NULL window arrays");
    if (prm->e < 1 || prm->e + prm->l > (uint32_t)kPrimerMaxRegion)
        return fail(CRP_ERR_ARG, "primer extension e=%u with l=%u unsupported: need 1 <= e and e + l <= %d", prm->e, prm->l,
                    kPrimerMaxRegion);
    PrimerClasses pc;
    memset(&pc, 0, sizeof pc);
    char msg[160];
    if (build_primer_classes((int)prm->s, (int)prm->l, prm->m, prm->x, prm->M, prm->X, prm->D, &pc, msg, sizeof msg))
        return fail(CRP_ERR_ARG, "%s", msg);
    std::vector<uint32_t> h(4 * n);
    for (uint64_t i = 0; i < n; ++i) {
        if (segment[i] >= g->segs.size()) return fail(CRP_ERR_ARG, "window %llu: segment %u out of range", (unsigned long long)i, segment[i]);
        const Segment &sg = g->segs[segment[i]];
        if (lo[i] > hi[i] || lo[i] < sg.begin || hi[i] > sg.end)
            return fail(CRP_ERR_ARG, "window %llu [%u, %u) is not inside the positions [%llu, %llu) segment %u owns",
                        (unsigned long long)i, lo[i], hi[i], (unsigned long long)sg.begin, (unsigned long long)sg.end, segment[i]);
        h[i] = sg.first_tile;
        h[n + i] = (uint32_t)sg.begin;
        h[2 * n + i] = lo[i];
        h[3 * n + i] = hi[i];
    }
    cudaStream_t st = stream_of(g);
    uint32_t *d_in = nullptr, *d_cnt = nullptr;
    unsigned long long *d_pairs = nullptr;
    uint16_t *d_first = nullptr;
    uint8_t *d_status = nullptr;
    PrimerClasses *d_cls = nullptr;
    int rc = 0;
    if (dev_alloc(&d_in, 4 * n * sizeof(uint32_t), st) || dev_alloc(&d_cnt, 2 * n * sizeof(uint32_t), st) ||
        dev_alloc(&d_pairs, n * sizeof(unsigned long long), st) || dev_alloc(&d_first, 4 * n * sizeof(uint16_t), st) ||
        dev_alloc(&d_status, n, st) || dev_alloc(&d_cls, sizeof(PrimerClasses), st)) {
        cudaGetLastError();
        rc = fail(CRP_ERR_NOMEM, "cudaMalloc of primer buffers failed");
    }
    if (!rc) {
        PrimerArgs a;
        a.records = g->records;
        a.cls = d_cls;
        a.first_tile = d_in;
        a.seg_begin = d_in + n;
        a.lo = d_in + 2 * n;
        a.hi = d_in + 3 * n;
        a.n = n;
        a.e = prm->e;
        a.n_fwd = d_cnt;
        a.n_rev = d_cnt + n;
        a.n_pairs = d_pairs;
        a.first = d_first;
        a.status = d_status;
        const uint64_t want = (n + 7) / 8, cap = (uint64_t)g_ctx.sm_count * 8;
        if (cudaMemcpyAsync(d_in, h.data(), 4 * n * sizeof(uint32_t), cudaMemcpyHostToDevice, st) != cudaSuccess ||
            cudaMemcpyAsync(d_cls, &pc, sizeof pc, cudaMemcpyHostToDevice, st) != cudaSuccess)
            rc = fail(CRP_ERR_CUDA, "H2D of primer windows failed");
        if (!rc) {
            k_primers<<<(unsigned)(want < cap ? want : cap), 256, 0, st>>>(a);
            g_ctx.launches++;
            auto back = [&](void *dst, const void *src, size_t bytes) {
                if (dst && !rc && cudaMemcpyAsync(dst, src, bytes, cudaMemcpyDeviceToHost, st) != cudaSuccess)
                    rc = fail(CRP_ERR_CUDA, "D2H of primer results failed");
            };
            back(n_fwd, a.n_fwd, n * 4);
            back(n_rev, a.n_rev, n * 4);
            back(n_pairs, a.n_pairs, n * 8);
            back(first, a.first, n * 8);
            back(status, a.status, n);
            if (!rc && cudaStreamSynchronize(st) != cudaSuccess)
                rc = fail(CRP_ERR_CUDA, "primer kernel failed: %s", cudaGetErrorString(cudaGetLastError()));
        }
    }
    dev_free(d_in, st);
    dev_free(d_cnt, st);
    dev_free(d_pairs, st);
    dev_free(d_first, st);
    dev_free(d_status, st);
    dev_free(d_cls, st);
    return rc;
}

int crp_result_annotate(const crp_result *res, uint32_t segment, char strand, uint32_t n_intervals,
                        const uint32_t *start, const uint32_t *end, int32_t *feature) {
    if (!res) return fail(CRP_ERR_ARG, "res is NULL");
    if (int rc = need_ctx()) return rc;
    uint64_t first = 0, n = 0;
    if (int rc = segment_rows(res, segment, strand, &first, &n)) return rc;
    if (n == 0) return 0;
    if (!feature || (n_intervals && (!start || !end))) return fail(CRP_ERR_ARG, "NULL argument");
    std::vector<uint32_t> host(3 * (size_t)n_intervals + 1);
    uint32_t running = 0;
    for (uint32_t j = 0; j < n_intervals; ++j) {
        if (j && start[j] < start[j - 1]) return fail(CRP_ERR_ARG, "intervals must be sorted by start");
        if (end[j] < start[j]) return fail(CRP_ERR_ARG, "interval %u has end < start", j);
        running = end[j] > running ? end[j] : running;
        host[j] = start[j];
        host[n_intervals + j] = end[j];
        host[2 * (size_t)n_intervals + j] = running;
    }
    cudaStream_t st = res->st;
    uint32_t *d_iv = nullptr;
    int32_t *d_f = nullptr;
    CUDA_TRY(dev_alloc(&d_iv, host.size() * sizeof(uint32_t), st));
    if (dev_alloc(&d_f, n * sizeof(int32_t), st) != cudaSuccess) {
        dev_free(d_iv, st);
        return fail(CRP_ERR_NOMEM, "cudaMalloc failed");
    }
    int rc = 0;
    const int s = strand == '+' ? 0 : 1;
    if (cudaMemcpyAsync(d_iv, host.data(), host.size() * sizeof(uint32_t), cudaMemcpyHostToDevice, st) != cudaSuccess)
        rc = fail(CRP_ERR_CUDA, "H2D of intervals failed");
    if (!rc) {
        k_annotate<<<(unsigned)((n + 255) / 256), 256, 0, st>>>(res->pos[s] + first, n, s, d_iv, d_iv + n_intervals,
                                                               d_iv + 2 * (size_t)n_intervals, n_intervals, d_f);
        g_ctx.launches++;
        if (cudaMemcpyAsync(feature, d_f, n * sizeof(int32_t), cudaMemcpyDeviceToHost, st) != cudaSuccess ||
            cudaStreamSynchronize(st) != cudaSuccess)
            rc = fail(CRP_ERR_CUDA, "annotate failed: %s", cudaGetErrorString(cudaGetLastError()));
    }
    dev_free(d_iv, st);
    dev_free(d_f, st);
    return rc;
}

int crp_rescore(const crp_genome *g, uint64_t n, const uint32_t *segment, const uint32_t *t, const char *strand,
                const uint8_t *cls, double *x_out) {
    if (!g) return fail(CRP_ERR_ARG, "g is NULL");
    if (int rc = need_ctx()) return rc;
    if (!g->committed) return fail(CRP_ERR_STATE, "genome not committed");
    if (n == 0) return 0;
    if (!segment || !t || !strand || !cls || !x_out) return fail(CRP_ERR_ARG, "NULL argument");
    std::vector<RescoreItem> items(n);
    for (uint64_t i = 0; i < n; ++i) {
        if (segment[i] >= g->segs.size()) return fail(CRP_ERR_ARG, "item %llu: bad segment", (unsigned long long)i);
        const Segment &s = g->segs[segment[i]];
        if (t[i] < s.begin || t[i] >= s.end)
            return fail(CRP_ERR_ARG, "item %llu: t=%u outside segment", (unsigned long long)i, t[i]);
        if (strand[i] != '+' && strand[i] != '-') return fail(CRP_ERR_ARG, "item %llu: bad strand", (unsigned long long)i);
        if ((cls[i] & 15u) > CRP_CLASS_SINGLE || (cls[i] >> 4) > CRP_CLASS_SINGLE) return fail(CRP_ERR_ARG, "item %llu: bad class", (unsigned long long)i);
        const uint64_t rel = t[i] - s.begin;
        items[i].tile = s.first_tile + (uint32_t)(rel / kTile);
        items[i].pl = (uint32_t)(rel % kTile);
        items[i].strand = (uint32_t)strand[i];
        items[i].cls = cls[i];
    }
    cudaStream_t st = stream_of(g);
    RescoreItem *d_items = nullptr;
    double *d_x = nullptr;
    CUDA_TRY(dev_alloc(&d_items, n * sizeof(RescoreItem), st));
    if (dev_alloc(&d_x, n * sizeof(double), st) != cudaSuccess) {
        dev_free(d_items, st);
        return fail(CRP_ERR_NOMEM, "cudaMalloc failed");
    }
    int rc = 0;
    do {
        if (cudaMemcpyAsync(d_items, items.data(), n * sizeof(RescoreItem), cudaMemcpyHostToDevice, st) != cudaSuccess) {
            rc = fail(CRP_ERR_CUDA, "H2D of rescore items failed");
            break;
        }
        k_rescore<<<(unsigned)((n + 127) / 128), 128, 0, st>>>(g->records, d_items, n, d_x);
        g_ctx.launches++;
        if (cudaMemcpyAsync(x_out, d_x, n * sizeof(double), cudaMemcpyDeviceToHost, st) != cudaSuccess ||
            cudaStreamSynchronize(st) != cudaSuccess) {
            rc = fail(CRP_ERR_CUDA, "rescore failed: %s", cudaGetErrorString(cudaGetLastError()));
            break;
        }
    } while (0);
    dev_free(d_items, st);
    dev_free(d_x, st);
    return rc;
}

}


static std::vector<uint32_t> ot_segment_table(const crp_result *res, int s) {
    const std::vector<uint64_t> &cnt = s == 0 ? res->seg_plus : res->seg_minus;
    const uint32_t n_seg = (uint32_t)cnt.size();
    std::vector<uint32_t> seg(3 * (size_t)n_seg + 1);
    uint64_t row = 0;
    for (uint32_t i = 0; i < n_seg; ++i) {
        seg[i] = (uint32_t)row;
        row += cnt[i];
        seg[n_seg + 1 + i] = res->g->segs[i].first_tile;
        seg[2 * (size_t)n_seg + 1 + i] = (uint32_t)res->g->segs[i].begin;
    }
    seg[n_seg] = (uint32_t)row;
    return seg;
}

struct crp_offtarget {
    cudaStream_t st = nullptr;
    cudaEvent_t ev[5] = {nullptr, nullptr, nullptr, nullptr, nullptr};
    std::vector<const crp_genome *> genomes;
    unsigned long long *keys = nullptr;
    unsigned long long *loci = nullptr;
    bool with_loci = false;
    uint64_t n_sites = 0;
    float ms_sites = 0.f, ms_count = 0.f;
    uint64_t comparisons = 0;
};

template <class Op>
static int ot_join(crp_offtarget *ix, const unsigned long long *d_keys, uint64_t n, uint32_t k, const Op &op) {
    using Site = typename Op::Site;
    cudaStream_t st = ix->st;
    const size_t tbl = kOtBuckets + 1;
    uint32_t *d_tbl = nullptr;
    Site *d_sites = nullptr;
    uint2 *d_q = nullptr;
    unsigned long long *d_misc = nullptr;
    if (dev_alloc(&d_tbl, 7 * tbl * sizeof(uint32_t), st) != cudaSuccess ||
        dev_alloc(&d_sites, (ix->n_sites + 8) * sizeof(Site), st) != cudaSuccess ||
        dev_alloc(&d_q, (n + 1) * sizeof(uint2), st) != cudaSuccess ||
        dev_alloc(&d_misc, 2 * sizeof(unsigned long long), st) != cudaSuccess) {
        cudaGetLastError();
        dev_free(d_tbl, st);
        dev_free(d_sites, st);
        dev_free(d_q, st);
        return fail(CRP_ERR_NOMEM, "cudaMalloc of the off-target work buffers failed");
    }
    uint32_t *hist_s = d_tbl, *hist_q = d_tbl + tbl;
    OtScanArgs sa;
    sa.hist[0] = hist_s;
    sa.hist[1] = hist_q;
    sa.off[0] = d_tbl + 2 * tbl;
    sa.off[1] = d_tbl + 3 * tbl;
    sa.cursor[0] = d_tbl + 4 * tbl;
    sa.cursor[1] = d_tbl + 5 * tbl;
    sa.item_off = d_tbl + 6 * tbl;
    sa.comparisons = d_misc;
    sa.overflow = reinterpret_cast<unsigned int *>(d_misc + 1);
    OtJoin ja;
    ja.sites = d_sites;
    ja.queries = d_q;
    ja.soff = sa.off[0];
    ja.qoff = sa.off[1];
    ja.item_off = sa.item_off;
    ja.k = k;
    auto grid = [](uint64_t items) { return (unsigned)std::max<uint64_t>(1, std::min<uint64_t>((items + 255) / 256, (uint64_t)g_ctx.sm_count * 16)); };
    int rc = 0;
    unsigned long long misc[2] = {0, 0};
    if (cudaMemsetAsync(d_misc, 0, 2 * sizeof(unsigned long long), st) != cudaSuccess ||
        cudaEventRecord(ix->ev[2], st) != cudaSuccess)
        rc = fail(CRP_ERR_CUDA, "off-target setup failed");
    for (int p = 0; p < kOtPairs && !rc && n && ix->n_sites; ++p) {
        int i = 0, j = 0;
        ot_pair(p, i, j);
        ja.jm1 = (uint32_t)(j - 1);
        ja.pi = i;
        ja.pj = j;
        if (cudaMemsetAsync(d_tbl, 0, 2 * tbl * sizeof(uint32_t), st) != cudaSuccess) {
            rc = fail(CRP_ERR_CUDA, "memset failed");
            break;
        }
        k_ot_hist<<<grid(ix->n_sites), 256, 0, st>>>(ix->keys, ix->n_sites, i, j, hist_s);
        k_ot_hist<<<grid(n), 256, 0, st>>>(d_keys, n, i, j, hist_q);
        k_ot_scan<<<3, kOtScanThreads, 0, st>>>(sa);
        if constexpr (std::is_same_v<Site, uint2>)
            k_ot_scatter<<<grid(ix->n_sites), 256, 0, st>>>(ix->keys, ix->n_sites, i, j, sa.cursor[0], nullptr, d_sites);
        else
            k_ot_scatter<<<grid(ix->n_sites), 256, 0, st>>>(ix->keys, ix->n_sites, i, j, sa.cursor[0], d_sites, nullptr);
        k_ot_scatter<<<grid(n), 256, 0, st>>>(d_keys, n, i, j, sa.cursor[1], nullptr, d_q);
        k_ot_join<Op><<<(unsigned)g_ctx.sm_count * 8, kOtThreads, 0, st>>>(ja, op);
        g_ctx.launches += 6;
        if (cudaGetLastError() != cudaSuccess) rc = fail(CRP_ERR_CUDA, "off-target launch failed");
    }
    if (!rc && (cudaEventRecord(ix->ev[3], st) != cudaSuccess ||
                cudaMemcpyAsync(misc, d_misc, sizeof misc, cudaMemcpyDeviceToHost, st) != cudaSuccess ||
                cudaStreamSynchronize(st) != cudaSuccess ||
                cudaEventElapsedTime(&ix->ms_count, ix->ev[2], ix->ev[3]) != cudaSuccess))
        rc = fail(CRP_ERR_CUDA, "off-target join failed: %s", cudaGetErrorString(cudaGetLastError()));
    if (!rc && misc[1]) rc = fail(CRP_ERR_RANGE, "a part pair needs 2^32 work items or more");
    if (!rc) ix->comparisons = misc[0];
    dev_free(d_tbl, st);
    dev_free(d_sites, st);
    dev_free(d_q, st);
    dev_free(d_misc, st);
    return rc;
}

static int ot_check_candidates(const crp_offtarget *ix, const crp_result *res, char strand, uint32_t max_mm,
                               const char *what, bool loci) {
    if (!ix || !res) return fail(CRP_ERR_ARG, "NULL argument");
    if (int rc = need_ctx()) return rc;
    if (strand != '+' && strand != '-') return fail(CRP_ERR_ARG, "strand must be '+' or '-'");
    if (max_mm > 3) return fail(CRP_ERR_ARG, "max_mm %u: at most 3 mismatches", max_mm);
    if (loci && !ix->with_loci) return fail(CRP_ERR_STATE, "listing needs an index with loci (crp_offtarget_new_with_loci)");
    if (res->guide_len != 20) return fail(CRP_ERR_STATE, "off-target %s are defined for guide_len 20 only", what);
    if (std::find(ix->genomes.begin(), ix->genomes.end(), res->g) == ix->genomes.end())
        return fail(CRP_ERR_STATE, "the result's genome has not been added to the index");
    return 0;
}

static int ot_candidate_keys(crp_offtarget *ix, const crp_result *res, int s, uint32_t *d_counts, uint32_t k1,
                             unsigned long long **d_keys, uint32_t **d_seg) {
    const uint64_t n = s == 0 ? res->n_plus : res->n_minus;
    const uint32_t n_seg = (uint32_t)(s == 0 ? res->seg_plus : res->seg_minus).size();
    const std::vector<uint32_t> seg = ot_segment_table(res, s);
    cudaStream_t st = ix->st;
    CUDA_TRY(cudaEventRecord(ix->ev[4], res->st));
    CUDA_TRY(cudaStreamWaitEvent(st, ix->ev[4], 0));
    if (dev_alloc(d_seg, seg.size() * sizeof(uint32_t), st) != cudaSuccess ||
        dev_alloc(d_keys, n * sizeof(unsigned long long), st) != cudaSuccess) {
        cudaGetLastError();
        return fail(CRP_ERR_NOMEM, "cudaMalloc of %llu query rows failed", (unsigned long long)n);
    }
    if (cudaMemcpyAsync(*d_seg, seg.data(), seg.size() * sizeof(uint32_t), cudaMemcpyHostToDevice, st) != cudaSuccess)
        return fail(CRP_ERR_CUDA, "H2D of the segment table failed");
    OtQueryArgs a;
    a.records = res->g->records;
    a.pos = res->pos[s];
    a.n = n;
    a.seg_row = *d_seg;
    a.seg_tile = *d_seg + n_seg + 1;
    a.seg_begin = *d_seg + 2 * (size_t)n_seg + 1;
    a.n_seg = n_seg;
    a.k1 = k1;
    a.minus = s;
    a.keys = *d_keys;
    a.counts = d_counts;
    k_ot_queries<<<(unsigned)((n + 255) / 256), 256, 0, st>>>(a);
    g_ctx.launches++;
    if (cudaGetLastError() != cudaSuccess) return fail(CRP_ERR_CUDA, "off-target query keys failed");
    return 0;
}

static int ot_check_keys(uint64_t n, const uint64_t *keys) {
    if (!keys) return fail(CRP_ERR_ARG, "keys is NULL");
    if (n > 0xFFFFFFFFull) return fail(CRP_ERR_RANGE, "at most 2^32 - 1 keys per call");
    for (uint64_t i = 0; i < n; ++i)
        if (keys[i] >> 40) return fail(CRP_ERR_ARG, "key %llu has bits above bit 39", (unsigned long long)i);
    return 0;
}

static int ot_upload_keys(crp_offtarget *ix, uint64_t n, const uint64_t *keys, unsigned long long **d_keys) {
    if (dev_alloc(d_keys, n * sizeof(unsigned long long), ix->st) != cudaSuccess) {
        cudaGetLastError();
        return fail(CRP_ERR_NOMEM, "cudaMalloc of %llu keys failed", (unsigned long long)n);
    }
    if (cudaMemcpyAsync(*d_keys, keys, n * sizeof(uint64_t), cudaMemcpyHostToDevice, ix->st) != cudaSuccess)
        return fail(CRP_ERR_CUDA, "H2D of the keys failed");
    return 0;
}

static int ot_count(crp_offtarget *ix, const unsigned long long *d_keys, uint64_t n, uint32_t k, uint32_t *d_counts,
                    uint32_t *counts) {
    cudaStream_t st = ix->st;
    int rc = ot_join(ix, d_keys, n, k, OtCount{d_counts});
    if (!rc && (cudaMemcpyAsync(counts, d_counts, n * (k + 1) * sizeof(uint32_t), cudaMemcpyDeviceToHost, st) != cudaSuccess ||
                cudaStreamSynchronize(st) != cudaSuccess))
        rc = fail(CRP_ERR_CUDA, "D2H of the off-target counts failed");
    return rc;
}

extern "C" {

int crp_offtarget_new(crp_offtarget **ix) {
    if (!ix) return fail(CRP_ERR_ARG, "ix is NULL");
    if (int rc = need_ctx()) return rc;
    crp_offtarget *o = new (std::nothrow) crp_offtarget();
    if (!o) return fail(CRP_ERR_NOMEM, "out of host memory");
    if (cudaStreamCreateWithFlags(&o->st, cudaStreamNonBlocking) != cudaSuccess) {
        delete o;
        return fail(CRP_ERR_CUDA, "cudaStreamCreate failed");
    }
    for (int i = 0; i < 5; ++i)
        if (cudaEventCreateWithFlags(&o->ev[i], i == 4 ? cudaEventDisableTiming : cudaEventDefault) != cudaSuccess) {
            crp_offtarget_free(o);
            return fail(CRP_ERR_CUDA, "cudaEventCreate failed");
        }
    *ix = o;
    return 0;
}

int crp_offtarget_new_with_loci(crp_offtarget **ix) {
    if (int rc = crp_offtarget_new(ix)) return rc;
    (*ix)->with_loci = true;
    return 0;
}

int crp_offtarget_add_genome(crp_offtarget *ix, const crp_genome *g) {
    if (!ix || !g) return fail(CRP_ERR_ARG, "NULL argument");
    if (int rc = need_ctx()) return rc;
    if (!g->committed) return fail(CRP_ERR_STATE, "genome is not committed");
    if (std::find(ix->genomes.begin(), ix->genomes.end(), g) != ix->genomes.end())
        return fail(CRP_ERR_STATE, "genome already added to this index");
    if (ix->with_loci && g->segs.size() >= kOtMaxSegments)
        return fail(CRP_ERR_RANGE, "%zu segments: a locus holds 24 bits of segment index", g->segs.size());
    if (ix->with_loci && ix->genomes.size() >= kOtMaxGenomes)
        return fail(CRP_ERR_RANGE, "an index with loci takes at most %u genome handles", kOtMaxGenomes);
    cudaStream_t st = ix->st;
    CUDA_TRY(cudaEventRecord(ix->ev[4], stream_of(g)));
    CUDA_TRY(cudaStreamWaitEvent(st, ix->ev[4], 0));
    const uint64_t items = (uint64_t)g->n_tiles * kTileWords;
    unsigned long long *d_n = nullptr, *h_n = static_cast<unsigned long long *>(pinned_get(sizeof(unsigned long long)));
    if (!h_n) return fail(CRP_ERR_NOMEM, "cudaHostAlloc failed");
    CUDA_TRY(dev_alloc(&d_n, sizeof(unsigned long long), st));
    OtSiteArgs a;
    a.records = g->records;
    a.n_tiles = g->n_tiles;
    a.keys = nullptr;
    a.base = ix->n_sites;
    a.n = d_n;
    a.loci = nullptr;
    a.genome = (uint32_t)ix->genomes.size();
    int rc = 0;
    *h_n = 0;
    if (cudaEventRecord(ix->ev[0], st) != cudaSuccess || cudaMemsetAsync(d_n, 0, sizeof *d_n, st) != cudaSuccess)
        rc = fail(CRP_ERR_CUDA, "off-target setup failed");
    if (!rc && items) {
        k_ot_sites<false><<<(unsigned)((items + 255) / 256), 256, 0, st>>>(a);
        g_ctx.launches++;
    }
    if (!rc && (cudaMemcpyAsync(h_n, d_n, sizeof *d_n, cudaMemcpyDeviceToHost, st) != cudaSuccess ||
                cudaStreamSynchronize(st) != cudaSuccess))
        rc = fail(CRP_ERR_CUDA, "site count failed: %s", cudaGetErrorString(cudaGetLastError()));
    const uint64_t add = *h_n, total = ix->n_sites + add;
    if (!rc && total > 0xFFFFFFFFull) rc = fail(CRP_ERR_RANGE, "%llu sites exceed 2^32 - 1", (unsigned long long)total);
    if (!rc && add) {
        unsigned long long *keys = nullptr, *loci = nullptr;
        if (dev_alloc(&keys, total * sizeof(unsigned long long), st) != cudaSuccess ||
            (ix->with_loci && dev_alloc(&loci, total * sizeof(unsigned long long), st) != cudaSuccess)) {
            cudaGetLastError();
            dev_free(keys, st);
            rc = fail(CRP_ERR_NOMEM, "cudaMalloc of %llu site keys failed", (unsigned long long)total);
        } else {
            if (ix->n_sites && cudaMemcpyAsync(keys, ix->keys, ix->n_sites * sizeof(unsigned long long), cudaMemcpyDeviceToDevice,
                                               st) != cudaSuccess)
                rc = fail(CRP_ERR_CUDA, "copy of the site keys failed");
            if (!rc && loci && ix->n_sites &&
                cudaMemcpyAsync(loci, ix->loci, ix->n_sites * sizeof(unsigned long long), cudaMemcpyDeviceToDevice, st) != cudaSuccess)
                rc = fail(CRP_ERR_CUDA, "copy of the site loci failed");
            dev_free(ix->keys, st);
            dev_free(ix->loci, st);
            ix->keys = keys;
            ix->loci = loci;
            a.keys = keys;
            a.loci = loci;
            if (!rc && cudaMemsetAsync(d_n, 0, sizeof *d_n, st) != cudaSuccess) rc = fail(CRP_ERR_CUDA, "memset failed");
            if (!rc) {
                if (loci)
                    k_ot_sites<true><<<(unsigned)((items + 255) / 256), 256, 0, st>>>(a);
                else
                    k_ot_sites<false><<<(unsigned)((items + 255) / 256), 256, 0, st>>>(a);
                g_ctx.launches++;
            }
            if (!rc && (cudaMemcpyAsync(h_n, d_n, sizeof *d_n, cudaMemcpyDeviceToHost, st) != cudaSuccess ||
                        cudaEventRecord(ix->ev[1], st) != cudaSuccess || cudaStreamSynchronize(st) != cudaSuccess))
                rc = fail(CRP_ERR_CUDA, "site keys failed: %s", cudaGetErrorString(cudaGetLastError()));
            if (!rc && *h_n != add) rc = fail(CRP_ERR_STATE, "site passes disagree (%llu, %llu)", (unsigned long long)add, *h_n);
            if (rc) {
                dev_free(ix->keys, st);
                dev_free(ix->loci, st);
                ix->keys = nullptr;
                ix->loci = nullptr;
                ix->n_sites = 0;
                ix->genomes.clear();
            }
        }
    } else if (!rc) {
        rc = cudaEventRecord(ix->ev[1], st) == cudaSuccess && cudaEventSynchronize(ix->ev[1]) == cudaSuccess
                 ? 0 : fail(CRP_ERR_CUDA, "event failed");
    }
    float ms = 0.f;
    if (!rc && cudaEventElapsedTime(&ms, ix->ev[0], ix->ev[1]) == cudaSuccess) ix->ms_sites += ms;
    if (!rc) {
        ix->n_sites = total;
        ix->genomes.push_back(g);
    }
    dev_free(d_n, st);
    pinned_put(h_n);
    return rc;
}

int crp_offtarget_num_sites(const crp_offtarget *ix, uint64_t *n) {
    if (!ix || !n) return fail(CRP_ERR_ARG, "NULL argument");
    *n = ix->n_sites;
    return 0;
}

int crp_offtarget_fetch_sites(const crp_offtarget *ix, uint64_t capacity, uint64_t *keys, uint64_t *n) {
    if (!ix || !n) return fail(CRP_ERR_ARG, "NULL argument");
    *n = ix->n_sites;
    if (capacity < ix->n_sites) return fail(CRP_ERR_RANGE, "%llu sites, room for %llu", (unsigned long long)ix->n_sites,
                                            (unsigned long long)capacity);
    if (!ix->n_sites) return 0;
    if (!keys) return fail(CRP_ERR_ARG, "keys is NULL");
    CUDA_TRY(cudaMemcpyAsync(keys, ix->keys, ix->n_sites * sizeof(uint64_t), cudaMemcpyDeviceToHost, ix->st));
    CUDA_TRY(cudaStreamSynchronize(ix->st));
    return 0;
}

int crp_offtarget_count_candidates(crp_offtarget *ix, const crp_result *res, char strand, uint32_t max_mm, uint32_t *counts) {
    if (int rc = ot_check_candidates(ix, res, strand, max_mm, "counts", false)) return rc;
    const int s = strand == '+' ? 0 : 1;
    const uint64_t n = s == 0 ? res->n_plus : res->n_minus;
    if (n == 0) return 0;
    if (!counts) return fail(CRP_ERR_ARG, "counts is NULL");
    cudaStream_t st = ix->st;
    const uint32_t k1 = max_mm + 1;
    uint32_t *d_seg = nullptr, *d_counts = nullptr;
    unsigned long long *d_keys = nullptr;
    int rc = 0;
    if (dev_alloc(&d_counts, n * k1 * sizeof(uint32_t), st) != cudaSuccess) {
        cudaGetLastError();
        rc = fail(CRP_ERR_NOMEM, "cudaMalloc of %llu query rows failed", (unsigned long long)n);
    }
    if (!rc) rc = ot_candidate_keys(ix, res, s, d_counts, k1, &d_keys, &d_seg);
    if (!rc) rc = ot_count(ix, d_keys, n, max_mm, d_counts, counts);
    dev_free(d_seg, st);
    dev_free(d_keys, st);
    dev_free(d_counts, st);
    return rc;
}

int crp_offtarget_count_keys(crp_offtarget *ix, uint64_t n, const uint64_t *keys, uint32_t max_mm, uint32_t *counts) {
    if (!ix) return fail(CRP_ERR_ARG, "ix is NULL");
    if (int rc = need_ctx()) return rc;
    if (max_mm > 3) return fail(CRP_ERR_ARG, "max_mm %u: at most 3 mismatches", max_mm);
    if (n == 0) return 0;
    if (!counts) return fail(CRP_ERR_ARG, "counts is NULL");
    if (int rc = ot_check_keys(n, keys)) return rc;
    cudaStream_t st = ix->st;
    const uint32_t k1 = max_mm + 1;
    unsigned long long *d_keys = nullptr;
    uint32_t *d_counts = nullptr;
    int rc = ot_upload_keys(ix, n, keys, &d_keys);
    if (!rc && dev_alloc(&d_counts, n * k1 * sizeof(uint32_t), st) != cudaSuccess) {
        cudaGetLastError();
        rc = fail(CRP_ERR_NOMEM, "cudaMalloc of %llu keys failed", (unsigned long long)n);
    }
    if (!rc && cudaMemsetAsync(d_counts, 0, n * k1 * sizeof(uint32_t), st) != cudaSuccess)
        rc = fail(CRP_ERR_CUDA, "memset failed");
    if (!rc) rc = ot_count(ix, d_keys, n, max_mm, d_counts, counts);
    dev_free(d_keys, st);
    dev_free(d_counts, st);
    return rc;
}

int crp_offtarget_fetch_loci(const crp_offtarget *ix, uint64_t capacity, uint64_t *loci, uint64_t *n) {
    if (!ix || !n) return fail(CRP_ERR_ARG, "NULL argument");
    if (!ix->with_loci) return fail(CRP_ERR_STATE, "the index keeps no loci (crp_offtarget_new_with_loci)");
    *n = ix->n_sites;
    if (capacity < ix->n_sites) return fail(CRP_ERR_RANGE, "%llu sites, room for %llu", (unsigned long long)ix->n_sites,
                                            (unsigned long long)capacity);
    if (!ix->n_sites) return 0;
    if (!loci) return fail(CRP_ERR_ARG, "loci is NULL");
    CUDA_TRY(cudaMemcpyAsync(loci, ix->loci, ix->n_sites * sizeof(uint64_t), cudaMemcpyDeviceToHost, ix->st));
    CUDA_TRY(cudaStreamSynchronize(ix->st));
    return 0;
}

}

static int ot_list(crp_offtarget *ix, const unsigned long long *d_keys, const unsigned long long *d_own, uint64_t n,
                   uint32_t k, const uint64_t *first, uint32_t *sites) {
    cudaStream_t st = ix->st;
    const uint64_t total = first[n];
    unsigned long long *d_first = nullptr;
    uint32_t *d_cursor = nullptr, *d_out = nullptr;
    unsigned int *d_flag = nullptr;
    if (dev_alloc(&d_first, (n + 1) * sizeof(unsigned long long), st) != cudaSuccess ||
        dev_alloc(&d_cursor, n * sizeof(uint32_t), st) != cudaSuccess ||
        dev_alloc(&d_out, std::max<uint64_t>(total, 1) * sizeof(uint32_t), st) != cudaSuccess ||
        dev_alloc(&d_flag, sizeof(unsigned int), st) != cudaSuccess) {
        cudaGetLastError();
        dev_free(d_first, st);
        dev_free(d_cursor, st);
        dev_free(d_out, st);
        return fail(CRP_ERR_NOMEM, "cudaMalloc of a listing of %llu sites failed", (unsigned long long)total);
    }
    int rc = 0;
    if (cudaMemcpyAsync(d_first, first, (n + 1) * sizeof(uint64_t), cudaMemcpyHostToDevice, st) != cudaSuccess ||
        cudaMemsetAsync(d_cursor, 0, n * sizeof(uint32_t), st) != cudaSuccess ||
        cudaMemsetAsync(d_flag, 0, sizeof(unsigned int), st) != cudaSuccess)
        rc = fail(CRP_ERR_CUDA, "listing setup failed");
    if (!rc) rc = ot_join(ix, d_keys, n, k, OtList{ix->loci, d_own, d_first, d_cursor, d_out, d_flag});
    std::vector<uint32_t> found(rc ? 0 : n);
    unsigned int flag = 0;
    if (!rc && (cudaMemcpyAsync(found.data(), d_cursor, n * sizeof(uint32_t), cudaMemcpyDeviceToHost, st) != cudaSuccess ||
                cudaMemcpyAsync(&flag, d_flag, sizeof flag, cudaMemcpyDeviceToHost, st) != cudaSuccess ||
                cudaStreamSynchronize(st) != cudaSuccess))
        rc = fail(CRP_ERR_CUDA, "D2H of the listing cursors failed");
    for (uint64_t i = 0; i < n && !rc; ++i)
        if (found[i] != first[i + 1] - first[i])
            rc = fail(CRP_ERR_STATE, "row %llu: %u sites found, its slice holds %llu", (unsigned long long)i, found[i],
                      (unsigned long long)(first[i + 1] - first[i]));
    if (!rc && flag) rc = fail(CRP_ERR_STATE, "a row found more sites than its slice holds");
    if (!rc && total && (cudaMemcpyAsync(sites, d_out, total * sizeof(uint32_t), cudaMemcpyDeviceToHost, st) != cudaSuccess ||
                         cudaStreamSynchronize(st) != cudaSuccess))
        rc = fail(CRP_ERR_CUDA, "D2H of the listing failed");
    dev_free(d_first, st);
    dev_free(d_cursor, st);
    dev_free(d_out, st);
    dev_free(d_flag, st);
    return rc;
}

static int ot_check_first(uint64_t n, const uint64_t *first) {
    if (!first) return fail(CRP_ERR_ARG, "first is NULL");
    if (first[0] != 0) return fail(CRP_ERR_ARG, "first[0] must be 0");
    for (uint64_t i = 0; i < n; ++i)
        if (first[i + 1] < first[i]) return fail(CRP_ERR_ARG, "first[%llu] < first[%llu]", (unsigned long long)i + 1,
                                                 (unsigned long long)i);
    return 0;
}

extern "C" {

int crp_offtarget_list_candidates(crp_offtarget *ix, const crp_result *res, char strand, uint32_t max_mm, uint64_t n_rows,
                                  const uint32_t *rows, const uint64_t *first, uint32_t *sites) {
    if (int rc = ot_check_candidates(ix, res, strand, max_mm, "listings", true)) return rc;
    if (n_rows == 0) return 0;
    if (!rows) return fail(CRP_ERR_ARG, "rows is NULL");
    if (int rc = ot_check_first(n_rows, first)) return rc;
    if (first[n_rows] && !sites) return fail(CRP_ERR_ARG, "sites is NULL");
    const int s = strand == '+' ? 0 : 1;
    const uint64_t n = s == 0 ? res->n_plus : res->n_minus;
    for (uint64_t i = 0; i < n_rows; ++i)
        if (rows[i] >= n || (i && rows[i] <= rows[i - 1]))
            return fail(CRP_ERR_ARG, "rows[%llu] = %u: rows must be ascending, distinct and below %llu", (unsigned long long)i,
                        rows[i], (unsigned long long)n);
    cudaStream_t st = ix->st;
    uint32_t *d_seg = nullptr, *d_rows = nullptr;
    unsigned long long *d_keys = nullptr, *d_sel = nullptr;
    unsigned int *d_invalid = nullptr;
    int rc = ot_candidate_keys(ix, res, s, nullptr, 0, &d_keys, &d_seg);
    if (!rc && (dev_alloc(&d_rows, n_rows * sizeof(uint32_t), st) != cudaSuccess ||
                dev_alloc(&d_sel, 2 * n_rows * sizeof(unsigned long long), st) != cudaSuccess ||
                dev_alloc(&d_invalid, sizeof(unsigned int), st) != cudaSuccess)) {
        cudaGetLastError();
        rc = fail(CRP_ERR_NOMEM, "cudaMalloc of %llu selected rows failed", (unsigned long long)n_rows);
    }
    if (!rc && (cudaMemcpyAsync(d_rows, rows, n_rows * sizeof(uint32_t), cudaMemcpyHostToDevice, st) != cudaSuccess ||
                cudaMemsetAsync(d_invalid, 0, sizeof(unsigned int), st) != cudaSuccess))
        rc = fail(CRP_ERR_CUDA, "H2D of the listing rows failed");
    unsigned int invalid = 0;
    if (!rc) {
        OtGatherArgs ga;
        ga.keys = d_keys;
        ga.pos = res->pos[s];
        ga.rows = d_rows;
        ga.seg_row = d_seg;
        ga.n = n_rows;
        ga.n_seg = (uint32_t)(s == 0 ? res->seg_plus : res->seg_minus).size();
        ga.genome = (uint32_t)(std::find(ix->genomes.begin(), ix->genomes.end(), res->g) - ix->genomes.begin());
        ga.minus = s;
        ga.sel_keys = d_sel;
        ga.own = d_sel + n_rows;
        ga.invalid = d_invalid;
        k_ot_gather<<<(unsigned)((n_rows + 255) / 256), 256, 0, st>>>(ga);
        g_ctx.launches++;
        if (cudaGetLastError() != cudaSuccess ||
            cudaMemcpyAsync(&invalid, d_invalid, sizeof invalid, cudaMemcpyDeviceToHost, st) != cudaSuccess ||
            cudaStreamSynchronize(st) != cudaSuccess)
            rc = fail(CRP_ERR_CUDA, "off-target query keys failed: %s", cudaGetErrorString(cudaGetLastError()));
    }
    if (!rc && invalid) rc = fail(CRP_ERR_ARG, "a selected row has no protospacer (its counts are 0xFFFFFFFF)");
    if (!rc) rc = ot_list(ix, d_sel, d_sel + n_rows, n_rows, max_mm, first, sites);
    dev_free(d_seg, st);
    dev_free(d_keys, st);
    dev_free(d_rows, st);
    dev_free(d_sel, st);
    dev_free(d_invalid, st);
    return rc;
}

int crp_offtarget_list_keys(crp_offtarget *ix, uint64_t n, const uint64_t *keys, uint32_t max_mm, const uint64_t *first,
                            uint32_t *sites) {
    if (!ix) return fail(CRP_ERR_ARG, "ix is NULL");
    if (int rc = need_ctx()) return rc;
    if (max_mm > 3) return fail(CRP_ERR_ARG, "max_mm %u: at most 3 mismatches", max_mm);
    if (!ix->with_loci) return fail(CRP_ERR_STATE, "listing needs an index with loci (crp_offtarget_new_with_loci)");
    if (n == 0) return 0;
    if (int rc = ot_check_keys(n, keys)) return rc;
    if (int rc = ot_check_first(n, first)) return rc;
    if (first[n] && !sites) return fail(CRP_ERR_ARG, "sites is NULL");
    unsigned long long *d_keys = nullptr;
    int rc = ot_upload_keys(ix, n, keys, &d_keys);
    if (!rc) rc = ot_list(ix, d_keys, nullptr, n, max_mm, first, sites);
    dev_free(d_keys, ix->st);
    return rc;
}

}

static int ot_check_weights(uint32_t k, const uint32_t *weights) {
    static const uint32_t used[4] = {1, 21, 211, kOtScoreSets};
    if (!weights) return fail(CRP_ERR_ARG, "weights is NULL");
    for (uint32_t r = 0; r < used[k]; ++r)
        if (weights[r] >> 31) return fail(CRP_ERR_ARG, "weights[%u] = %u: at most 2^31 - 1", r, weights[r]);
    return 0;
}

static int ot_score(crp_offtarget *ix, const unsigned long long *d_keys, uint64_t n, uint32_t k, const uint32_t *weights,
                    unsigned long long *d_sums, uint64_t *sums) {
    cudaStream_t st = ix->st;
    uint32_t *d_w = nullptr;
    if (dev_alloc(&d_w, kOtScoreSets * sizeof(uint32_t), st) != cudaSuccess) {
        cudaGetLastError();
        return fail(CRP_ERR_NOMEM, "cudaMalloc of the weight table failed");
    }
    int rc = 0;
    if (cudaMemcpyAsync(d_w, weights, kOtScoreSets * sizeof(uint32_t), cudaMemcpyHostToDevice, st) != cudaSuccess)
        rc = fail(CRP_ERR_CUDA, "H2D of the weight table failed");
    if (!rc) rc = ot_join(ix, d_keys, n, k, OtScore{d_w, d_sums});
    if (!rc && (cudaMemcpyAsync(sums, d_sums, n * sizeof(uint64_t), cudaMemcpyDeviceToHost, st) != cudaSuccess ||
                cudaStreamSynchronize(st) != cudaSuccess))
        rc = fail(CRP_ERR_CUDA, "D2H of the off-target scores failed");
    dev_free(d_w, st);
    return rc;
}

extern "C" {

int crp_offtarget_score_candidates(crp_offtarget *ix, const crp_result *res, char strand, uint32_t max_mm,
                                   const uint32_t *weights, uint64_t *sums) {
    if (int rc = ot_check_candidates(ix, res, strand, max_mm, "scores", false)) return rc;
    if (int rc = ot_check_weights(max_mm, weights)) return rc;
    const int s = strand == '+' ? 0 : 1;
    const uint64_t n = s == 0 ? res->n_plus : res->n_minus;
    if (n == 0) return 0;
    if (!sums) return fail(CRP_ERR_ARG, "sums is NULL");
    cudaStream_t st = ix->st;
    uint32_t *d_seg = nullptr;
    unsigned long long *d_keys = nullptr, *d_sums = nullptr;
    int rc = 0;
    if (dev_alloc(&d_sums, n * sizeof(unsigned long long), st) != cudaSuccess) {
        cudaGetLastError();
        rc = fail(CRP_ERR_NOMEM, "cudaMalloc of %llu query rows failed", (unsigned long long)n);
    }
    if (!rc) rc = ot_candidate_keys(ix, res, s, nullptr, 0, &d_keys, &d_seg);
    if (!rc) {
        k_ot_score_prime<<<(unsigned)((n + 255) / 256), 256, 0, st>>>(d_keys, n, 0ull - weights[0], d_sums);
        g_ctx.launches++;
        if (cudaGetLastError() != cudaSuccess) rc = fail(CRP_ERR_CUDA, "off-target score priming failed");
    }
    if (!rc) rc = ot_score(ix, d_keys, n, max_mm, weights, d_sums, sums);
    dev_free(d_seg, st);
    dev_free(d_keys, st);
    dev_free(d_sums, st);
    return rc;
}

int crp_offtarget_score_keys(crp_offtarget *ix, uint64_t n, const uint64_t *keys, uint32_t max_mm, const uint32_t *weights,
                             uint64_t *sums) {
    if (!ix) return fail(CRP_ERR_ARG, "ix is NULL");
    if (int rc = need_ctx()) return rc;
    if (max_mm > 3) return fail(CRP_ERR_ARG, "max_mm %u: at most 3 mismatches", max_mm);
    if (int rc = ot_check_weights(max_mm, weights)) return rc;
    if (n == 0) return 0;
    if (!sums) return fail(CRP_ERR_ARG, "sums is NULL");
    if (int rc = ot_check_keys(n, keys)) return rc;
    cudaStream_t st = ix->st;
    unsigned long long *d_keys = nullptr, *d_sums = nullptr;
    int rc = ot_upload_keys(ix, n, keys, &d_keys);
    if (!rc && dev_alloc(&d_sums, n * sizeof(unsigned long long), st) != cudaSuccess) {
        cudaGetLastError();
        rc = fail(CRP_ERR_NOMEM, "cudaMalloc of %llu keys failed", (unsigned long long)n);
    }
    if (!rc && cudaMemsetAsync(d_sums, 0, n * sizeof(unsigned long long), st) != cudaSuccess)
        rc = fail(CRP_ERR_CUDA, "memset failed");
    if (!rc) rc = ot_score(ix, d_keys, n, max_mm, weights, d_sums, sums);
    dev_free(d_keys, st);
    dev_free(d_sums, st);
    return rc;
}

int crp_offtarget_timing(const crp_offtarget *ix, float *ms_sites, float *ms_count, uint64_t *comparisons) {
    if (!ix) return fail(CRP_ERR_ARG, "ix is NULL");
    if (ms_sites) *ms_sites = ix->ms_sites;
    if (ms_count) *ms_count = ix->ms_count;
    if (comparisons) *comparisons = ix->comparisons;
    return 0;
}

int crp_offtarget_free(crp_offtarget *ix) {
    if (!ix) return 0;
    if (ix->st) {
        dev_free(ix->keys, ix->st);
        dev_free(ix->loci, ix->st);
        cudaStreamSynchronize(ix->st);
    }
    for (cudaEvent_t e : ix->ev)
        if (e) cudaEventDestroy(e);
    if (ix->st) cudaStreamDestroy(ix->st);
    delete ix;
    return 0;
}

}
```

### cropsr_b200/csrc/scan.cuh

```cuda
#pragma once
#include <cooperative_groups.h>
#include <cuda_runtime.h>
#include <stdint.h>

#include "npexp.cuh"
#include "rs1.cuh"

namespace cg = cooperative_groups;

#ifndef CRP_CTAS_PER_SM
#define CRP_CTAS_PER_SM 4
#endif
static constexpr int kThreads = 256;
static constexpr int kWarps = kThreads / 32;
static constexpr int kTileWords = 2 * kThreads;
static constexpr int kTile = kTileWords * 32;
static constexpr int kRecWords = kTileWords + 3;
static constexpr uint32_t kRecBytes = kRecWords * 16;
static constexpr int kStages = 2;
static constexpr int kListCap = 1024;
static constexpr int kPrefWords = 10;
static constexpr uint32_t kNoTile = 0xFFFFFFFFu;
static constexpr int kMaxPeers = 8;
static constexpr uint32_t kAlign = 128;

static constexpr int kPamWords = kTileWords + 1;
static constexpr uint32_t kPamBytes = (16 + kPamWords * 8 + 15) / 16 * 16;
static constexpr int kCountStages = 6;
struct __align__(16) TileHdr {
    uint4 desc;
    uint32_t cnt[8];
};
static_assert(sizeof(TileHdr) == 48, "bulk copies move multiples of 16 bytes");
static constexpr uint32_t kPackItems = 544;
static_assert(kPackItems % 32 == 0 && kPackItems >= (uint32_t)kRecWords, "whole warps per tile");
static constexpr int kHdrBatch = 256;
static_assert(kRecBytes % 16 == 0, "bulk copies move multiples of 16 bytes");

struct TileDesc {
    uint32_t t_start;
    uint32_t L;
    uint32_t n;
    uint32_t segment;
};

struct PackDesc {
    uint64_t ascii_off;
    uint32_t stage_begin, stage_end;
    TileDesc td;
};

CRP_HD uint32_t range_mask(int32_t t0, int32_t lo, int32_t hi) {
    int32_t a = lo - t0, b = hi - t0;
    if (a < 0) a = 0;
    if (b > 31) b = 31;
    if (a > b) return 0u;
    return (0xFFFFFFFFu >> (31 - b)) & (0xFFFFFFFFu << a);
}

CRP_HD uint32_t pack_word_hits(uint32_t g, uint32_t c, uint32_t gn, uint32_t cn, int32_t tw, const TileDesc td) {
    uint32_t hp = crp_funnel_r(g, gn, 1) & crp_funnel_r(g, gn, 2), hm = c & crp_funnel_r(c, cn, 1);
    const int32_t hi_p = min((int32_t)td.L - 3, (int32_t)td.t_start + (int32_t)td.n - 1);
    if (tw < 2 || tw + 31 > hi_p) {
        hp &= range_mask(tw, 0, hi_p);
        hm &= range_mask(tw, 2, hi_p);
    }
    return (uint32_t)crp_popc(hp) | ((uint32_t)crp_popc(hm) << 16);
}

__host__ __device__ inline uint32_t classify(uint32_t c) {
    uint32_t up = c & 0xDFu;
    uint32_t r = 8u;
    if (up == 'A') r = 0u;
    else if (up == 'T') r = 1u;
    else if (up == 'C') r = 2u;
    else if (up == 'G') r = 3u;
    if (r < 8u) return r | ((c & 0x20u) >> 3);
    if (c == 'U') return 8u | 1u;
    if (c == 'Z') return 8u | 3u;
    return 8u;
}

__global__ void __launch_bounds__(256, 8)
k_pack(const uint8_t *__restrict__ ascii, const PackDesc *__restrict__ descs, const PackDesc one, uint64_t n_items,
       uint4 *__restrict__ records, unsigned char *__restrict__ pam, TileHdr *__restrict__ hdr) {
    __shared__ uint32_t lut[256];
    {
        const uint32_t nib = classify(threadIdx.x);
        lut[threadIdx.x] = (nib & 1u) | ((nib >> 1) & 1u) << 8 | ((nib >> 2) & 1u) << 16 | ((nib >> 3) & 1u) << 24;
    }
    __syncthreads();
    const uint64_t stride = (uint64_t)gridDim.x * blockDim.x;
    for (uint64_t item = (uint64_t)blockIdx.x * blockDim.x + threadIdx.x; item < n_items; item += stride) {
        const uint64_t tile = item / kPackItems;
        const uint32_t i = (uint32_t)(item - tile * kPackItems);
        const uint32_t k = i < (uint32_t)kTileWords ? i + 2u : i == (uint32_t)kTileWords ? 0u : i == (uint32_t)kTileWords + 1u ? 1u : (uint32_t)kTileWords + 2u;
        const uint64_t it = tile * kRecWords + k;
        uint32_t hits = 0;
        uint32_t pg = 0, pc = 0;
        TileDesc td = {0u, 0u, 0u, 0u};
        uint64_t ascii_off = 0;
        uint32_t stage_lo = 0, stage_hi = 0;
        if (i < (uint32_t)kTileWords + 3u) {
            PackDesc pd;
            if (descs) {
                pd = descs[tile];
            } else {
                pd = one;
                const uint32_t done = (uint32_t)tile * (uint32_t)kTile;
                pd.td.t_start = one.td.t_start + done;
                pd.td.n = one.td.n - done < (uint32_t)kTile ? one.td.n - done : (uint32_t)kTile;
            }
            td = pd.td, ascii_off = pd.ascii_off, stage_lo = pd.stage_begin, stage_hi = pd.stage_end;
            if (k == 0) {
                const uint4 d = make_uint4(pd.td.t_start, pd.td.L, pd.td.n, pd.td.segment);
                records[it] = d;
                *reinterpret_cast<uint4 *>(pam + tile * kPamBytes) = d;
                hdr[tile].desc = d;
            } else {
                const int64_t p0 = (int64_t)pd.td.t_start + ((int64_t)k - 2) * 32;
                const int64_t lo = pd.stage_begin, hi = pd.stage_end;
                uint32_t o0 = 0, o1 = 0, ol = 0, oo = 0;
                if (p0 >= lo && p0 + 32 <= hi) {
                    const uint4 *src = reinterpret_cast<const uint4 *>(ascii + pd.ascii_off + (uint64_t)(p0 - lo));
                    const uint4 a = __ldg(src), b = __ldg(src + 1);
                    const uint32_t v[8] = {a.x, a.y, a.z, a.w, b.x, b.y, b.z, b.w};
                    uint32_t acc[4];
#pragma unroll
                    for (int g = 0; g < 4; ++g) {
                        uint32_t s = 0;
#pragma unroll
                        for (int j = 0; j < 8; ++j) s += lut[(v[2 * g + (j >> 2)] >> (8 * (j & 3))) & 0xFFu] << j;
                        acc[g] = s;
                    }
                    const uint32_t t01 = __byte_perm(acc[0], acc[1], 0x5140), t23 = __byte_perm(acc[2], acc[3], 0x5140);
                    const uint32_t u01 = __byte_perm(acc[0], acc[1], 0x7362), u23 = __byte_perm(acc[2], acc[3], 0x7362);
                    o0 = __byte_perm(t01, t23, 0x5410);
                    o1 = __byte_perm(t01, t23, 0x7632);
                    ol = __byte_perm(u01, u23, 0x5410);
                    oo = __byte_perm(u01, u23, 0x7632);
                } else {
                    for (int bit = 0; bit < 32; ++bit) {
                        const int64_t p = p0 + bit;
                        uint32_t e = 1u << 24;
                        if (p >= lo && p < hi) e = lut[ascii[pd.ascii_off + (uint64_t)(p - lo)]];
                        o0 |= (e & 1u) << bit;
                        o1 |= ((e >> 8) & 1u) << bit;
                        ol |= ((e >> 16) & 1u) << bit;
                        oo |= ((e >> 24) & 1u) << bit;
                    }
                }
                records[it] = make_uint4(o0, o1, ol, oo);
                if (k >= 2) {
                    const uint32_t up = ~(ol | oo);
                    const uint32_t g = o0 & o1 & up, c = ~o0 & o1 & up;
                    reinterpret_cast<uint2 *>(pam + tile * kPamBytes + 16)[k - 2] = make_uint2(g, c);
                    pg = g, pc = c;
                }
            }
        }
        if (i < (uint32_t)kTileWords) {
            uint32_t gn = __shfl_down_sync(0xFFFFFFFFu, pg, 1), cn = __shfl_down_sync(0xFFFFFFFFu, pc, 1);
            const int64_t p0 = (int64_t)td.t_start + (int64_t)i * 32;
            if ((threadIdx.x & 31) == 31) {
                gn = 0, cn = 0;
#pragma unroll
                for (int j = 0; j < 2; ++j) {
                    const int64_t q = p0 + 32 + j;
                    if (q >= (int64_t)stage_lo && q < (int64_t)stage_hi) {
                        const uint32_t ch = ascii[ascii_off + (uint64_t)(q - stage_lo)];
                        gn |= (uint32_t)(ch == 'G') << j;
                        cn |= (uint32_t)(ch == 'C') << j;
                    }
                }
            }
            hits = pack_word_hits(pg, pc, gn, cn, (int32_t)p0, td);
        }
        const uint32_t sum = __reduce_add_sync(0xFFFFFFFFu, hits);
        if ((threadIdx.x & 31) == 0 && sum) atomicAdd(&hdr[tile].cnt[i / 64u], sum);
    }
}

struct FastaRec {
    uint64_t raw_off;
    uint64_t ascii_off;
    uint64_t first_item;
    uint32_t n_bases, width;
    uint32_t last, pad;
};

__global__ void __launch_bounds__(256)
k_fasta_strip(const uint8_t *__restrict__ raw, const FastaRec *__restrict__ recs, uint32_t n_recs, uint64_t n_items,
              uint8_t *__restrict__ ascii, unsigned int *__restrict__ bad) {
    const uint64_t stride = (uint64_t)gridDim.x * blockDim.x;
    for (uint64_t it = (uint64_t)blockIdx.x * blockDim.x + threadIdx.x; it < n_items; it += stride) {
        uint32_t lo = 0, hi = n_recs;
        while (hi - lo > 1) {
            const uint32_t mid = (lo + hi) >> 1;
            if (recs[mid].first_item <= it) lo = mid;
            else hi = mid;
        }
        const FastaRec r = recs[lo];
        const uint64_t p0 = (it - r.first_item) * 16;
        const uint64_t n = r.n_bases, L = n + 4;
        uint64_t b = p0 ? p0 - 1 : 0;
        uint64_t line = b / r.width;
        uint32_t col = (uint32_t)(b - line * r.width);
        const uint8_t *src = raw + r.raw_off + b + line;
        uint32_t w[4] = {0, 0, 0, 0};
        unsigned int err = 0;
#pragma unroll
        for (int i = 0; i < 16; ++i) {
            const uint64_t p = p0 + i;
            uint32_t c = 0;
            if (p == 0 || p == n + 1) c = '\'';
            else if (p == n + 2) c = ')';
            else if (p == n + 3) c = r.last ? ']' : ',';
            else if (p < L) {
                if (col == r.width) {
                    if (__ldg(src) != '\n') err = 1;
                    ++src;
                    col = 0;
                }
                c = __ldg(src++);
                ++col;
                if (c <= 0x20 || c >= 0x7F || c == '\'' || c == '"' || c == '\\' || c == '>') err = 1;
            }
            w[i >> 2] |= c << (8 * (i & 3));
        }
        *reinterpret_cast<uint4 *>(ascii + r.ascii_off + p0) = make_uint4(w[0], w[1], w[2], w[3]);
        if (err) atomicOr(bad, 1u);
    }
}

__device__ __forceinline__ uint32_t smem_u32(const void *p) { return (uint32_t)__cvta_generic_to_shared(p); }

__device__ __forceinline__ void mbar_init(unsigned long long *bar, uint32_t count) {
    asm volatile("mbarrier.init.shared::cta.b64 [%0], %1;" ::"r"(smem_u32(bar)), "r"(count) : "memory");
}
__device__ __forceinline__ void mbar_wait(unsigned long long *bar, uint32_t parity) {
    const uint32_t b = smem_u32(bar);
    asm volatile(
        "{\n"
        ".reg .pred p;\n"
        "WAIT_%=:\n"
        "mbarrier.try_wait.parity.shared::cta.b64 p, [%0], %1;\n"
        "@p bra DONE_%=;\n"
        "bra WAIT_%=;\n"
        "DONE_%=:\n"
        "}\n" ::"r"(b),
        "r"(parity)
        : "memory");
}

struct Hits {
    uint32_t pA, mA, pB, mB;
};

CRP_HD Hits hits_from_planes(uint32_t gA, uint32_t gAn, uint32_t cA, uint32_t cAn, uint32_t gB, uint32_t gBn, uint32_t cB,
                             uint32_t cBn, const TileDesc td, int l, int wordA) {
    Hits h;
    h.pA = crp_funnel_r(gA, gAn, 1) & crp_funnel_r(gA, gAn, 2);
    h.pB = crp_funnel_r(gB, gBn, 1) & crp_funnel_r(gB, gBn, 2);
    h.mA = cA & crp_funnel_r(cA, cAn, 1);
    h.mB = cB & crp_funnel_r(cB, cBn, 1);
    const int32_t t0 = (int32_t)td.t_start, L = (int32_t)td.L;
    const int32_t last_owned = t0 + (int32_t)td.n - 1;
    const int32_t hi_p = min(L - 3, last_owned);
    const int32_t hi_m = min(L - l + 7, hi_p);
    if (t0 < l + 5 || t0 + kTile - 1 > hi_m) {
        const int32_t tA = t0 + 32 * wordA, tB = tA + 32 * 32;
        h.pA &= range_mask(tA, l + 5, hi_p);
        h.pB &= range_mask(tB, l + 5, hi_p);
        h.mA &= range_mask(tA, 2, hi_m);
        h.mB &= range_mask(tB, 2, hi_m);
    }
    return h;
}

CRP_HD Hits tile_hits(const uint4 *__restrict__ rec, const TileDesc td, int l, int wordA) {
    const uint4 a = rec[2 + wordA], an = rec[3 + wordA], b = rec[34 + wordA], bn = rec[35 + wordA];
    const uint32_t uA = ~(a.z | a.w), uAn = ~(an.z | an.w), uB = ~(b.z | b.w), uBn = ~(bn.z | bn.w);
    return hits_from_planes(a.x & a.y & uA, an.x & an.y & uAn, ~a.x & a.y & uA, ~an.x & an.y & uAn, b.x & b.y & uB,
                            bn.x & bn.y & uBn, ~b.x & b.y & uB, ~bn.x & bn.y & uBn, td, l, wordA);
}

__device__ __forceinline__ void warp_count_tile(const unsigned char *__restrict__ rec, int l, int lane,
                                                uint32_t *__restrict__ cnt) {
    const uint4 d = __ldg(reinterpret_cast<const uint4 *>(rec));
    const uint2 *w = reinterpret_cast<const uint2 *>(rec + 16);
    const int32_t t0 = (int32_t)d.x, L = (int32_t)d.y;
    const int32_t last_owned = t0 + (int32_t)d.z - 1;
    const int32_t hi_p = min(L - 3, last_owned);
    const int32_t hi_m = min(L - l + 7, hi_p);
    const bool edge = t0 < l + 5 || t0 + kTile - 1 > hi_m;
#pragma unroll
    for (int half = 0; half < 2; ++half) {
        uint2 a[8], an[8];
#pragma unroll
        for (int i = 0; i < 8; ++i) {
            const int word = 32 * (8 * half + i) + lane;
            a[i] = __ldg(w + word);
            an[i] = __ldg(w + word + 1);
        }
#pragma unroll
        for (int c = 0; c < 4; ++c) {
            uint32_t n = 0;
#pragma unroll
            for (int h = 0; h < 2; ++h) {
                const int i = 2 * c + h, word = 32 * (8 * half + i) + lane;
                uint32_t p = __funnelshift_r(a[i].x, an[i].x, 1) & __funnelshift_r(a[i].x, an[i].x, 2);
                uint32_t m = a[i].y & __funnelshift_r(a[i].y, an[i].y, 1);
                if (edge) {
                    const int32_t tw = t0 + 32 * word;
                    p &= range_mask(tw, l + 5, hi_p);
                    m &= range_mask(tw, 2, hi_m);
                }
                n += __popc(p) | (__popc(m) << 16);
            }
            n = __reduce_add_sync(0xFFFFFFFFu, n);
            if (lane == 0) cnt[4 * half + c] = n;
        }
    }
}

struct ScanArgs {
    const uint4 *records;
    const unsigned char *pam;
    const TileHdr *hdr;
    uint32_t n_tiles;
    uint32_t static_eighths;
    int guide_len;
    uint32_t flags;
    const double *tables;
    uint64_t capacity;
    uint32_t *pos_plus, *pos_minus;
    unsigned long long *packed_plus, *packed_minus;
    double *x_plus, *x_minus;
    unsigned long long *warp_pref;
    unsigned long long *cta_tot;
    unsigned int *tickets;
    unsigned long long *seg_counts;
    unsigned long long *seg_counts_host;
    unsigned int *fault;
    const uint32_t *seg_first_tile, *seg_tile_count;
    uint32_t n_seg, seg_stride;
    uint32_t world, rank, epoch;
    unsigned long long *peer_gather[kMaxPeers];
    unsigned int *peer_flags[kMaxPeers];
    unsigned int *xchg_error;
    unsigned long long xchg_timeout_ns;
};

#ifdef CRP_CHECKED
#define CRP_CHECK(a, cond, code)                                                            \
    do {                                                                                    \
        if (!(cond) && (a).fault) atomicCAS((a).fault, 0u, (unsigned)(code) | ((unsigned)__LINE__ << 8)); \
    } while (0)
#else
#define CRP_CHECK(a, cond, code) \
    do {                         \
    } while (0)
#endif

__device__ __forceinline__ void xchg_wait(const ScanArgs &a) {
    if (threadIdx.x < a.world) {
        volatile unsigned int *flag = a.peer_flags[a.rank] + threadIdx.x;
        unsigned long long t0, t1;
        asm volatile("mov.u64 %0, %%globaltimer;" : "=l"(t0));
        while (*flag != a.epoch) {
            __nanosleep(200);
            asm volatile("mov.u64 %0, %%globaltimer;" : "=l"(t1));
            if (t1 - t0 > a.xchg_timeout_ns) {
                atomicExch(a.xchg_error, 1u + threadIdx.x);
                break;
            }
        }
        __threadfence_system();
    }
}

__device__ __forceinline__ void xchg_publish(const ScanArgs &a) {
    __threadfence_system();
    for (uint32_t p = 0; p < a.world; ++p) *reinterpret_cast<volatile unsigned int *>(a.peer_flags[p] + a.rank) = a.epoch;
}

__global__ void k_exchange_empty(const ScanArgs a) {
    for (uint32_t sg = threadIdx.x; sg < 2 * a.seg_stride; sg += blockDim.x) {
        a.seg_counts[sg] = 0ull;
        if (a.seg_counts_host) a.seg_counts_host[sg] = 0ull;
        for (uint32_t p = 0; p < a.world; ++p) a.peer_gather[p][(size_t)a.rank * 2 * a.seg_stride + sg] = 0ull;
    }
    __syncthreads();
    if (threadIdx.x == 0 && a.world > 1) xchg_publish(a);
    if (a.world > 1) xchg_wait(a);
}

__device__ unsigned long long *g_dbg_times = nullptr;
__device__ __forceinline__ void dbg_stamp(int slot) {
    unsigned long long *p = g_dbg_times;
    if (p && threadIdx.x == 0) {
        unsigned long long t;
        asm volatile("mov.u64 %0, %%globaltimer;" : "=l"(t));
        p[8ull * blockIdx.x + slot] = t;
    }
}

struct Window {
    uint32_t s0, s1, valid;
    unsigned long long packed;
};

static constexpr uint32_t kWinBiasPlus = 7u, kWinBiasMinus = 30u;
template <bool kMinus>
CRP_HD Window extract_window(const uint4 *__restrict__ rec, uint32_t ws, uint32_t t, uint32_t L) {
    const uint32_t wi = 1u + (ws >> 5), sh = ws;
    const uint4 lo = rec[wi], hi = rec[wi + 1];
    const uint32_t p0 = crp_funnel_r(lo.x, hi.x, sh), p1 = crp_funnel_r(lo.y, hi.y, sh);
    const uint32_t lw = crp_funnel_r(lo.z, hi.z, sh), ot = crp_funnel_r(lo.w, hi.w, sh);
    const uint32_t special = ot & p0;
    const uint32_t valid = ~ot | special;
    Window w;
    if (kMinus) {
        w.s0 = (p0 ^ special) & 0x3FFFFFFFu;
        w.s1 = p1 & 0x3FFFFFFFu;
        w.valid = valid & 0x3FFFFFFFu;
    } else {
        w.s0 = crp_brev(p0 ^ ~(lw | ot)) >> 2;
        w.s1 = crp_brev(p1) >> 2;
        w.valid = crp_brev(valid) >> 2;
    }
    const uint32_t hi32 = w.s1 | (~(w.valid + 1u) & (uint32_t)(CRP_PACKED_UNSCORED >> 32));
    const uint32_t irr = (lw | ot) & 0x3FFFFFFFu;
    uint32_t lo32 = w.s0 | ((irr + 0x3FFFFFFFu) & (uint32_t)CRP_PACKED_IRREGULAR);
    if (t + (kMinus ? 28u : 5u) > L) lo32 |= (uint32_t)CRP_PACKED_TRUNCATED;
    w.packed = ((unsigned long long)hi32 << 32) | lo32;
    return w;
}

__device__ __forceinline__ unsigned long long unpack_counts(uint32_t c) {
    return ((unsigned long long)(c & 0xFFFFu) << 32) | (c >> 16);
}

static constexpr uint32_t kWinBiasPlusHot = kWinBiasPlus - 2u;
template <bool kMinus>
CRP_HD double score_hit(const double *__restrict__ tab, const uint4 *__restrict__ rec, uint32_t ws, uint32_t xt,
                        unsigned long long &packed) {
    const uint32_t wbyte = crp_umulhi(ws, 1u << 27) * 16u;
    const uint4 lo = *reinterpret_cast<const uint4 *>(reinterpret_cast<const char *>(rec) + 16 + wbyte);
    const uint4 hi = *reinterpret_cast<const uint4 *>(reinterpret_cast<const char *>(rec) + 32 + wbyte);
    const uint32_t p0 = crp_funnel_r(lo.x, hi.x, ws), p1 = crp_funnel_r(lo.y, hi.y, ws);
    const uint32_t lw = crp_funnel_r(lo.z, hi.z, ws), ot = crp_funnel_r(lo.w, hi.w, ws);
    uint32_t xs;
#ifdef __CUDA_ARCH__
    asm("mad.lo.u32 %0, %1, 0xFFFFFFFF, %2;" : "=r"(xs) : "r"(ws), "r"(xt));
#else
    xs = xt - ws;
#endif
    const uint32_t trunc = crp_umulhi(xs, 2u);
    constexpr uint32_t kWin = kMinus ? 0x3FFFFFFFu : 0xFFFFFFFCu;
    uint32_t mA, mT, mC, mG, w0, w1;
    if (kMinus) {
        const uint32_t s0 = p0 & ~ot;
        const uint32_t e = ~(p0 ^ ot);
        mA = e & ~p1, mC = e & p1, mT = s0 & ~p1, mG = s0 & p1;
        w0 = s0, w1 = p1;
    } else {
        uint32_t q0;
#ifdef __CUDA_ARCH__
        asm("lop3.b32 %0, %1, %2, %3, 0xE1;" : "=r"(q0) : "r"(p0), "r"(lw), "r"(ot));
#else
        q0 = p0 ^ ~(lw | ot);
#endif
        const uint32_t s0 = crp_brev(q0), s1 = crp_brev(p1), valid = crp_brev(~ot | p0);
        mA = ~s1 & ~s0 & valid, mT = ~s1 & s0 & valid, mC = s1 & ~s0 & valid, mG = s1 & s0 & valid;
        w0 = s0, w1 = s1;
    }
    const uint32_t irr = (lw | ot) & kWin, uns = ot & ~p0 & kWin;
    const uint32_t y0 = (kMinus ? irr : crp_umulhi(irr, 1u << 30)) + 0x3FFFFFFFu;
    const uint32_t f1 = (kMinus ? uns : crp_umulhi(uns, 1u << 30)) + 0x3FFFFFFFu;
    static_assert(CRP_PACKED_IRREGULAR == (1ull << 30) && CRP_PACKED_TRUNCATED == (1ull << 31) && CRP_PACKED_UNSCORED == (1ull << 62),
                  "flag bits of the packed word");
    uint32_t f0, lo32, hi32;
#ifdef __CUDA_ARCH__
    asm("mad.lo.u32 %0, %1, 0x80000000, %2;" : "=r"(f0) : "r"(trunc), "r"(y0));
    asm("lop3.b32 %0, %1, 0x3FFFFFFF, %2, 0xE2;" : "=r"(lo32) : "r"(w0), "r"(f0));
    asm("lop3.b32 %0, %1, 0x3FFFFFFF, %2, 0xE2;" : "=r"(hi32) : "r"(w1), "r"(f1));
#else
    f0 = trunc * 0x80000000u + y0;
    lo32 = (w0 & 0x3FFFFFFFu) | (f0 & 0xC0000000u);
    hi32 = (w1 & 0x3FFFFFFFu) | (f1 & 0xC0000000u);
#endif
    packed = ((unsigned long long)hi32 << 32) | lo32;
    return rs1_canonical_masks(tab, mA, mT, mC, mG);
}

__device__ __forceinline__ void st_list_if(uint16_t *p, uint32_t cond, uint32_t v) {
    asm volatile(
        "{\n"
        ".reg .pred q;\n"
        "setp.ne.u32 q, %0, 0;\n"
        "@q st.shared.u16 [%1], %2;\n"
        "}\n" ::"r"(cond),
        "r"(smem_u32(p)), "h"((unsigned short)v)
        : "memory");
}
__device__ __forceinline__ void list_hits(uint16_t *__restrict__ first, uint32_t m, uint32_t pos0) {
    const uint32_t l0 = m & (0u - m);
    st_list_if(first, l0, pos0 + 31u - (uint32_t)__clz(l0));
    m ^= l0;
    const uint32_t l1 = m & (0u - m);
    st_list_if(first + 1, l1, pos0 + 31u - (uint32_t)__clz(l1));
    m ^= l1;
    const uint32_t l2 = m & (0u - m);
    st_list_if(first + 2, l2, pos0 + 31u - (uint32_t)__clz(l2));
    m ^= l2;
    first += 3;
    while (m) {
        const uint32_t lb = m & (0u - m);
        *first++ = (uint16_t)(pos0 + 31u - (uint32_t)__clz(lb));
        m ^= lb;
    }
}
__device__ __forceinline__ void list_hits_window(uint16_t *__restrict__ list, uint32_t m, uint32_t rank_first,
                                                 uint32_t pos0, uint32_t lo) {
    uint32_t r = rank_first;
    while (m) {
        const uint32_t lb = m & (0u - m);
        if (r - lo < (uint32_t)kListCap) list[r - lo] = (uint16_t)(pos0 + 31u - (uint32_t)__clz(lb));
        m ^= lb;
        ++r;
    }
}

template <bool kScore, bool kMinus>
__device__ __forceinline__ void emit_one(const ScanArgs &a, const double *__restrict__ tab, const uint4 *__restrict__ rec,
                                         const uint16_t *__restrict__ list, uint32_t i, uint32_t row0, uint32_t t_start,
                                         uint32_t L) {
    uint32_t *const pos = kMinus ? a.pos_minus : a.pos_plus;
    unsigned long long *const packed = kMinus ? a.packed_minus : a.packed_plus;
    double *const xs = kMinus ? a.x_minus : a.x_plus;
    constexpr uint32_t kBias = kMinus ? kWinBiasMinus : kWinBiasPlusHot;
    const uint32_t xt = L - (kMinus ? 28u : 5u) - (t_start - kBias);
    const uint32_t ws = list[i], t = t_start - kBias + ws;
    const uint32_t row = row0 + i;
    CRP_CHECK(a, i < (uint32_t)kListCap, 1);
    CRP_CHECK(a, ws >= kBias && 2u + (ws >> 5) < (uint32_t)kRecWords, 2);
    CRP_CHECK(a, row < (uint32_t)a.capacity && t < L, 3);
    CRP_CHECK(a, i == 0 || list[i - 1] < ws, 4);
    __stcs(pos + row, t);
    if (kScore) {
        unsigned long long word;
        const double x = score_hit<kMinus>(tab, rec, ws, xt, word);
#ifdef CRP_CHECKED
        {
            const Window w = extract_window<kMinus>(rec, ws + (kMinus ? 0u : 2u), t, L);
            CRP_CHECK(a, w.packed == word, 14);
            CRP_CHECK(a, __double_as_longlong(rs1_canonical(tab, w.s0, w.s1, w.valid)) == __double_as_longlong(x), 15);
        }
#endif
        __stcs(packed + row, word);
        __stcs(xs + row, x);
    }
}

__device__ __forceinline__ uint32_t rows_left(const ScanArgs &a, uint32_t count, uint32_t row0) {
    const uint32_t cap = (uint32_t)a.capacity;
    return row0 >= cap ? 0u : min(count, cap - row0);
}

template <bool kScore, bool kMinus>
__device__ __forceinline__ void emit_strand(const ScanArgs &a, const double *__restrict__ tab,
                                            const uint4 *__restrict__ rec, const uint16_t *__restrict__ list,
                                            uint32_t count, uint32_t row0, uint32_t t_start, uint32_t L, uint32_t slot) {
    count = rows_left(a, count, row0);
    for (uint32_t i = slot; i < count; i += kThreads) emit_one<kScore, kMinus>(a, tab, rec, list, i, row0, t_start, L);
}

struct __align__(16) Ring {
    unsigned long long pref[kStages][kPrefWords];
    unsigned long long full[kCountStages];
    unsigned long long pre;
    unsigned long long rbase[kStages];
    uint32_t tile[kCountStages];
    uint32_t done[kCountStages];
};
static_assert(kCountStages >= kStages, "the ring control block holds the emit phase's slots");

__device__ __forceinline__ void mbar_inval(unsigned long long *bar) {
    asm volatile("mbarrier.inval.shared::cta.b64 [%0];" ::"r"(smem_u32(bar)) : "memory");
}
__device__ __forceinline__ void mbar_arrive(unsigned long long *bar) {
    asm volatile("mbarrier.arrive.shared::cta.b64 _, [%0];" ::"r"(smem_u32(bar)) : "memory");
}
__device__ __forceinline__ void mbar_expect(unsigned long long *bar, uint32_t bytes) {
    asm volatile("mbarrier.arrive.expect_tx.shared::cta.b64 _, [%0], %1;" ::"r"(smem_u32(bar)), "r"(bytes) : "memory");
}
__device__ __forceinline__ void bulk_copy(void *dst, const void *src, uint32_t bytes, unsigned long long *bar) {
    asm volatile("cp.async.bulk.shared::cluster.global.mbarrier::complete_tx::bytes [%0], [%1], %2, [%3];" ::"r"(
                     smem_u32(dst)),
                 "l"(src), "r"(bytes), "r"(smem_u32(bar))
                 : "memory");
}

__device__ __forceinline__ void ring_reset(Ring &ring, bool first, bool wave_start) {
    __syncthreads();
    if (threadIdx.x == 0) {
#pragma unroll
        for (int s = 0; s < kCountStages; ++s) {
            if (!first) mbar_inval(&ring.full[s]);
            mbar_init(&ring.full[s], 1);
            ring.done[s] = 0;
            ring.tile[s] = kNoTile;
        }
        if (wave_start) {
            if (!first) mbar_inval(&ring.pre);
            mbar_init(&ring.pre, 1);
        }
        asm volatile("fence.mbarrier_init.release.cluster;" ::: "memory");
    }
    __syncthreads();
}

template <bool kScore>
__global__ void __launch_bounds__(kThreads, CRP_CTAS_PER_SM)
k_scan_score(const ScanArgs a) {
    extern __shared__ __align__(128) unsigned char s_dyn[];
    auto stage = [&](int s) { return reinterpret_cast<uint4 *>(s_dyn + (size_t)s * kRecBytes); };
    uint16_t *const s_list = reinterpret_cast<uint16_t *>(s_dyn + kStages * kRecBytes);
    unsigned long long *const s_rangepref =
        reinterpret_cast<unsigned long long *>(s_dyn + kStages * kRecBytes + 2 * (size_t)kListCap * sizeof(uint16_t));
    __shared__ __align__(16) double s_tab[kScore ? RS1_TABLE_DOUBLES : 1];
    __shared__ Ring ring;
    __shared__ unsigned long long s_scan[kWarps];

    cg::grid_group grid = cg::this_grid();
    const int tid = threadIdx.x, lane = tid & 31, warp = tid >> 5;
    const int l = a.guide_len;
    const uint32_t G = gridDim.x, cta = blockIdx.x;

    dbg_stamp(0);
    __shared__ __align__(8) unsigned long long s_tabbar;
    if (tid == 0) {
        mbar_init(&s_tabbar, 1);
        asm volatile("fence.mbarrier_init.release.cluster;" ::: "memory");
        if (kScore) {
            mbar_expect(&s_tabbar, (uint32_t)kRs1TableBytes);
            bulk_copy(s_tab, a.tables, (uint32_t)kRs1TableBytes, &s_tabbar);
        }
    }

    auto record = [&](uint32_t tile) { return a.records + (size_t)tile * kRecWords; };
    const uint32_t nt = a.n_tiles;
    const uint32_t k = (nt + G - 1) / G;

    const uint32_t r_lo = min(nt, cta * k), n_mine = min(nt, r_lo + k) - r_lo;
    if (cta == 0 && tid == 0) {
        a.tickets[0] = 0;
        a.tickets[1] = 0;
    }
    ring_reset(ring, true, true);
    dbg_stamp(1);
    TileHdr *const s_hdr = reinterpret_cast<TileHdr *>(s_dyn);
    static_assert(kHdrBatch == kThreads, "one tile header per thread");
    unsigned long long range_run = 0;
    for (uint32_t h_lo = 0, hb = 0; h_lo < n_mine; h_lo += kHdrBatch, ++hb) {
        const uint32_t h_n = min(n_mine - h_lo, (uint32_t)kHdrBatch);
        if (tid == 0) {
            mbar_expect(&ring.full[0], h_n * (uint32_t)sizeof(TileHdr));
            bulk_copy(s_dyn, a.hdr + (size_t)(r_lo + h_lo), h_n * (uint32_t)sizeof(TileHdr), &ring.full[0]);
        }
        mbar_wait(&ring.full[0], hb & 1u);
        for (uint32_t j = warp; j < h_n; j += kWarps) {
            const uint4 d = s_hdr[j].desc;
            const int32_t t0 = (int32_t)d.x, L = (int32_t)d.y;
            if (t0 < l + 5 || t0 + kTile - 1 > L - l + 7) {
                CRP_CHECK(a, r_lo + h_lo + j < nt, 5);
                CRP_CHECK(a, reinterpret_cast<const uint32_t *>(a.pam + (size_t)(r_lo + h_lo + j) * kPamBytes)[0] == d.x, 6);
                warp_count_tile(a.pam + (size_t)(r_lo + h_lo + j) * kPamBytes, l, lane, s_hdr[j].cnt);
            }
        }
        __syncthreads();
        {
            unsigned long long c[kWarps], mine = 0ull;
#pragma unroll
            for (int q = 0; q < kWarps; ++q) {
                c[q] = (uint32_t)tid < h_n ? unpack_counts(s_hdr[tid].cnt[q]) : 0ull;
                mine += c[q];
            }
            unsigned long long incl = mine;
#pragma unroll
            for (int o = 1; o < 32; o <<= 1) {
                const unsigned long long v = __shfl_up_sync(0xFFFFFFFFu, incl, o);
                if (lane >= o) incl += v;
            }
            if (lane == 31) s_scan[warp] = incl;
            __syncthreads();
            unsigned long long before = range_run, total = 0;
#pragma unroll
            for (int q = 0; q < kWarps; ++q) {
                const unsigned long long x = s_scan[q];
                if (q < warp) before += x;
                total += x;
            }
            if ((uint32_t)tid < h_n) {
                unsigned long long *pf = a.warp_pref + (size_t)(r_lo + h_lo + tid) * kPrefWords;
                unsigned long long run = before + incl - mine;
#pragma unroll
                for (int q = 0; q < kWarps; ++q) {
                    pf[q] = run;
                    run += c[q];
                }
                pf[kWarps] = run;
                asm volatile("fence.proxy.async.global;" ::: "memory");
            }
            range_run += total;
            __syncthreads();
        }
    }
    if (tid == 0) a.cta_tot[cta] = range_run;
    const uint32_t ns = (uint32_t)((unsigned long long)nt * a.static_eighths / 8 / G);
    const bool pre = ns > 0;
    const uint32_t t_pre = cta;
    if (pre && tid == 0) {
        mbar_expect(&ring.pre, kRecBytes + kPrefWords * 8);
        bulk_copy(stage(0), record(t_pre), kRecBytes, &ring.pre);
    }
    dbg_stamp(2);
    grid.sync();
    dbg_stamp(3);
    if (pre && tid == 0) bulk_copy(ring.pref[0], a.warp_pref + (size_t)t_pre * kPrefWords, kPrefWords * 8, &ring.pre);

    {
        unsigned long long v[4] = {0, 0, 0, 0}, mine = 0;
#pragma unroll
        for (int q = 0; q < 4; ++q) {
            const uint32_t i = 4u * tid + q;
            if (i < G) v[q] = a.cta_tot[i];
            mine += v[q];
        }
        unsigned long long incl = mine;
#pragma unroll
        for (int o = 1; o < 32; o <<= 1) {
            const unsigned long long x = __shfl_up_sync(0xFFFFFFFFu, incl, o);
            if (lane >= o) incl += x;
        }
        if (lane == 31) s_scan[warp] = incl;
        __syncthreads();
        unsigned long long before = 0;
#pragma unroll
        for (int q = 0; q < kWarps; ++q) {
            const unsigned long long x = s_scan[q];
            if (q < warp) before += x;
        }
        unsigned long long run = before + incl - mine;
#pragma unroll
        for (int q = 0; q < 4; ++q) {
            const uint32_t i = 4u * tid + q;
            if (i < G) s_rangepref[i] = run;
            run += v[q];
        }
    }

    const uint32_t dyn_lo = ns * G, n_dyn = nt - dyn_lo;
    unsigned int *const ticket = a.tickets;
    auto produce_emit = [&](uint32_t n, int s) {
        uint32_t t;
        if (n < ns) {
            t = n * G + cta;
        } else {
            const uint32_t q = atomicAdd(ticket, 1u);
            t = q < n_dyn ? dyn_lo + q : kNoTile;
        }
        ring.tile[s] = t;
        if (t != kNoTile) {
            CRP_CHECK(a, t < nt && t / k < G, 11);
            ring.rbase[s] = s_rangepref[t / k];
            mbar_expect(&ring.full[s], kRecBytes + kPrefWords * 8);
            bulk_copy(stage(s), record(t), kRecBytes, &ring.full[s]);
            bulk_copy(ring.pref[s], a.warp_pref + (size_t)t * kPrefWords, kPrefWords * 8, &ring.full[s]);
        } else {
            mbar_arrive(&ring.full[s]);
        }
    };
    ring_reset(ring, false, false);
    dbg_stamp(4);
    if (kScore) mbar_wait(&s_tabbar, 0);
    {
        const bool xchg = a.world > 1;
        for (uint32_t sg = cta * kThreads + tid; sg < a.seg_stride; sg += G * kThreads) {
            unsigned long long plus = 0, minus = 0;
            if (sg < a.n_seg) {
                const uint32_t f = a.seg_first_tile ? a.seg_first_tile[sg] : 0u;
                const uint32_t c = a.seg_tile_count ? a.seg_tile_count[sg] : a.n_tiles;
                if (c) {
                    const unsigned long long cnt = s_rangepref[(f + c - 1) / k] + a.warp_pref[(size_t)(f + c - 1) * kPrefWords + kWarps] -
                                                   (s_rangepref[f / k] + a.warp_pref[(size_t)f * kPrefWords]);
                    plus = cnt >> 32;
                    minus = cnt & 0xFFFFFFFFull;
                }
            }
            a.seg_counts[sg] = plus;
            a.seg_counts[a.seg_stride + sg] = minus;
            if (a.seg_counts_host) {
                a.seg_counts_host[sg] = plus;
                a.seg_counts_host[a.seg_stride + sg] = minus;
            }
            if (xchg) {
                CRP_CHECK(a, (size_t)(a.rank + 1) * 2 * a.seg_stride <= (size_t)kMaxPeers * 2 * 32768, 12);
                const size_t at = (size_t)a.rank * 2 * a.seg_stride + sg;
                for (uint32_t p = 0; p < a.world; ++p) {
                    a.peer_gather[p][at] = plus;
                    a.peer_gather[p][at + a.seg_stride] = minus;
                }
            }
        }
        if (xchg && cta * kThreads < a.seg_stride) {
            __threadfence_system();
            __syncthreads();
            if (tid == 0) {
                const uint32_t writers = min(G, (a.seg_stride + kThreads - 1) / kThreads);
                __threadfence_system();
                if (atomicAdd(a.tickets + 1, 1u) == writers - 1) xchg_publish(a);
            }
        }
    }
    if (tid == 0) {
        if (pre) mbar_arrive(&ring.full[0]);
        else produce_emit(0, 0);
    }
    uint16_t *const list_p = s_list, *const list_m = s_list + kListCap;
    for (uint32_t n = 0;; ++n) {
        const int s = n % kStages;
        if (tid == 0) produce_emit(n + 1, s ^ 1);
        const bool first_pre = pre && n == 0;
        if (first_pre) mbar_wait(&ring.pre, 0u);
        else mbar_wait(&ring.full[s], (n / kStages) & 1u);
        if (!first_pre && ring.tile[s] == kNoTile) break;
        const uint4 *rec = stage(s);
        const uint4 d = rec[0];
        const TileDesc td = {d.x, d.y, d.z, d.w};
        const unsigned long long tile_pref = ring.pref[s][0];
        const unsigned long long base = (first_pre ? s_rangepref[t_pre / k] : ring.rbase[s]) + tile_pref;
        const unsigned long long off = ring.pref[s][warp] - tile_pref;
        const unsigned long long tot = ring.pref[s][kWarps] - tile_pref;
        const uint32_t np = (uint32_t)(tot >> 32), nm = (uint32_t)tot;
        const uint32_t base_p = (uint32_t)(base >> 32), base_m = (uint32_t)base;
        const uint32_t wordA = 64 * warp + lane;
        const bool busy = ring.pref[s][warp + 1] != ring.pref[s][warp];
        Hits h = {0u, 0u, 0u, 0u};
        uint32_t epA = 0, emA = 0, epB = 0, emB = 0;
        if (busy) {
            h = tile_hits(rec, td, l, wordA);
            const uint32_t cA = __popc(h.pA) | (__popc(h.mA) << 16), cB = __popc(h.pB) | (__popc(h.mB) << 16);
            uint32_t iA = cA, iB = cB;
#pragma unroll
            for (int o = 1; o < 32; o <<= 1) {
                const uint32_t vA = __shfl_up_sync(0xFFFFFFFFu, iA, o), vB = __shfl_up_sync(0xFFFFFFFFu, iB, o);
                if (lane >= o) {
                    iA += vA;
                    iB += vB;
                }
            }
            const uint32_t totA = __shfl_sync(0xFFFFFFFFu, iA, 31);
            const uint32_t xA = iA - cA, xB = totA + iB - cB;
            const uint32_t op = (uint32_t)(off >> 32), om = (uint32_t)off;
            epA = op + (xA & 0xFFFFu), emA = om + (xA >> 16), epB = op + (xB & 0xFFFFu), emB = om + (xB >> 16);
#ifdef CRP_CHECKED
            {
                const uint32_t mine = totA + __shfl_sync(0xFFFFFFFFu, iB, 31);
                const unsigned long long nxt = ring.pref[s][warp + 1] - ring.pref[s][warp];
                CRP_CHECK(a, (uint32_t)(nxt >> 32) == (mine & 0xFFFFu) && (uint32_t)nxt == (mine >> 16), 7);
                if (np <= (uint32_t)kListCap && nm <= (uint32_t)kListCap)
                    CRP_CHECK(a, epA + __popc(h.pA) <= np && epB + __popc(h.pB) <= np && emA + __popc(h.mA) <= nm && emB + __popc(h.mB) <= nm, 10);
            }
#endif
        }
#ifdef CRP_CHECKED
        else {
            const Hits hh = tile_hits(rec, td, l, wordA);
            CRP_CHECK(a, (hh.pA | hh.pB | hh.mA | hh.mB) == 0u, 13);
        }
        CRP_CHECK(a, ring.tile[s] == kNoTile || first_pre || ring.tile[s] < nt, 8);
        CRP_CHECK(a, (unsigned long long)base_p + np <= 0xFFFFFFFFull && (unsigned long long)base_m + nm <= 0xFFFFFFFFull, 9);
#endif
        if (np <= (uint32_t)kListCap && nm <= (uint32_t)kListCap) {
            if (busy) {
                list_hits(list_p + epA, h.pA, 32u * wordA + kWinBiasPlusHot);
                list_hits(list_p + epB, h.pB, 32u * (wordA + 32) + kWinBiasPlusHot);
                list_hits(list_m + emA, h.mA, 32u * wordA + kWinBiasMinus);
                list_hits(list_m + emB, h.mB, 32u * (wordA + 32) + kWinBiasMinus);
            }
            __syncthreads();
            emit_strand<kScore, false>(a, s_tab, rec, list_p, np, base_p, td.t_start, td.L, tid);
            emit_strand<kScore, true>(a, s_tab, rec, list_m, nm, base_m, td.t_start, td.L, tid ^ (kThreads / 2));
        } else {
            for (uint32_t lo = 0; lo < np || lo < nm; lo += kListCap) {
                const uint32_t cp = np > lo ? min(np - lo, (uint32_t)kListCap) : 0u;
                const uint32_t cm = nm > lo ? min(nm - lo, (uint32_t)kListCap) : 0u;
                if (lo) __syncthreads();
                if (busy) {
                    list_hits_window(list_p, h.pA, epA, 32u * wordA + kWinBiasPlusHot, lo);
                    list_hits_window(list_p, h.pB, epB, 32u * (wordA + 32) + kWinBiasPlusHot, lo);
                    list_hits_window(list_m, h.mA, emA, 32u * wordA + kWinBiasMinus, lo);
                    list_hits_window(list_m, h.mB, emB, 32u * (wordA + 32) + kWinBiasMinus, lo);
                }
                __syncthreads();
                emit_strand<kScore, false>(a, s_tab, rec, list_p, cp, base_p + lo, td.t_start, td.L, tid);
                emit_strand<kScore, true>(a, s_tab, rec, list_m, cm, base_m + lo, td.t_start, td.L, tid);
            }
        }
        __syncthreads();
    }
    dbg_stamp(5);
    if (a.world > 1 && cta == 0) xchg_wait(a);
}

__global__ void k_logistic(double *__restrict__ x, uint64_t n) {
    const uint64_t stride = (uint64_t)gridDim.x * blockDim.x;
    for (uint64_t i = (uint64_t)blockIdx.x * blockDim.x + threadIdx.x; i < n; i += stride) x[i] = np_logistic_f64(x[i]);
}

__global__ void k_rs1_rows(const uint8_t *__restrict__ rows, const uint8_t *__restrict__ cls, uint64_t n,
                           double *__restrict__ score, int logistic) {
    const uint64_t i = (uint64_t)blockIdx.x * blockDim.x + threadIdx.x;
    if (i >= n) return;
    const uint8_t *r = rows + 30 * i;
    uint32_t s0 = 0, s1 = 0, valid = 0;
    for (int q = 0; q < 30; ++q) {
        const uint32_t c = r[q];
        const uint32_t code = c == 'A' ? 0u : c == 'T' ? 1u : c == 'C' ? 2u : c == 'G' ? 3u : 4u;
        if (code < 4u) {
            valid |= 1u << q;
            s0 |= (code & 1u) << q;
            s1 |= (code >> 1) << q;
        }
    }
    const double x = rs1_dense(s0, s1, valid, (int)(cls[i] & 15u), (int)(cls[i] >> 4));
    score[i] = logistic ? np_logistic_f64(x) : x;
}

struct RescoreItem {
    uint32_t tile;
    uint32_t pl;
    uint32_t strand;
    uint32_t cls;
};

__global__ void k_rescore(const uint4 *__restrict__ records, const RescoreItem *__restrict__ items, uint64_t n,
                          double *__restrict__ x_out) {
    const uint64_t i = (uint64_t)blockIdx.x * blockDim.x + threadIdx.x;
    if (i >= n) return;
    const RescoreItem it = items[i];
    const uint4 *rec = records + (size_t)it.tile * kRecWords;
    const Window w = it.strand == '-' ? extract_window<true>(rec, it.pl + kWinBiasMinus, 0u, 0xFFFFFFFFu)
                                      : extract_window<false>(rec, it.pl + kWinBiasPlus, 0u, 0xFFFFFFFFu);
    x_out[i] = rs1_dense(w.s0, w.s1, w.valid, (int)(it.cls & 15u), (int)(it.cls >> 4));
}
```

Baseline: 1630.

## Precompute tile prefix at commit and replace cooperative grid sync with edge kernel

The per-tile candidate prefix sums are now computed once, at genome commit time, by a single-block prefix kernel. They are no longer recomputed in every scan's count phase. The scan drops its cooperative launch and grid.sync. A small edge kernel recounts only the start and end zone tiles of each segment and writes correction values, and the main scan is launched with programmatic dependent launch so it can overlap. This removes a grid-wide barrier and repeated header scans per call, at the cost of a serial single-CTA prefix at commit and extra zone-pref loads for edge tiles.

After: 1651 (median of 6 runs). +1.2%, better.

```diff
diff --git a/cropsr_b200/csrc/cropsr_b200.cu b/cropsr_b200/csrc/cropsr_b200.cu
--- a/cropsr_b200/csrc/cropsr_b200.cu
+++ b/cropsr_b200/csrc/cropsr_b200.cu
@@ -84,8 +84,9 @@
     uint4 *records = nullptr;
     unsigned char *pam = nullptr;
     TileHdr *hdr = nullptr;
+    unsigned long long *pref = nullptr;
     uint32_t n_tiles = 0;
-    uint32_t *d_seg_first = nullptr, *d_seg_count = nullptr;
+    uint4 *d_seg_geo = nullptr;
     float ms_h2d = 0.f, ms_pack = 0.f;
     uint8_t *d_ascii = nullptr;
     bool fasta = false;
@@ -114,7 +115,7 @@
     unsigned long long *packed[2] = {nullptr, nullptr};
     double *x[2] = {nullptr, nullptr};
     unsigned char *state = nullptr;
-    size_t state_bytes = 0, zero_offset = 0;
+    size_t state_bytes = 0, counts_offset = 0;
     unsigned long long *d_counts = nullptr;
     std::vector<uint64_t> seg_plus, seg_minus;
     float ms_scan = 0.f;
@@ -799,7 +800,7 @@
     const bool one = g->segs.size() == 1;
     std::vector<PackDesc> descs;
     std::vector<uint64_t> seg_ascii;
-    std::vector<uint32_t> seg_first, seg_count;
+    std::vector<uint4> seg_geo;
     uint64_t ascii_bytes = 0, n_tiles = 0;
     g->n_positions = 0;
     for (size_t si = 0; si < g->segs.size(); ++si) {
@@ -823,8 +824,7 @@
             pd.td.segment = (uint32_t)si;
             descs.push_back(pd);
         }
-        seg_first.push_back(s.first_tile);
-        seg_count.push_back(s.n_tiles);
+        seg_geo.push_back(make_uint4(s.first_tile, s.n_tiles, (uint32_t)s.begin, (uint32_t)s.token_len));
         g->n_positions += s.end - s.begin;
         ascii_bytes += (s.stage_end - s.stage_begin + 15) / 16 * 16;
     }
@@ -843,7 +843,8 @@
         (!one && dev_alloc(&d_descs, (descs.size() + 1) * sizeof(PackDesc), st) != cudaSuccess) ||
         dev_alloc(&g->records, rec_bytes + 16, st) != cudaSuccess ||
         dev_alloc(&g->pam, (size_t)g->n_tiles * kPamBytes + 16, st) != cudaSuccess ||
-        dev_alloc(&g->hdr, ((size_t)g->n_tiles + 1) * sizeof(TileHdr), st) != cudaSuccess) {
+        dev_alloc(&g->hdr, ((size_t)g->n_tiles + 1) * sizeof(TileHdr), st) != cudaSuccess ||
+        dev_alloc(&g->pref, (size_t)g->n_tiles * kPrefWords * sizeof(unsigned long long) + 16, st) != cudaSuccess) {
         cudaGetLastError();
         dev_free(d_ascii, st);
         dev_free(d_descs, st);
@@ -918,14 +919,16 @@
         k_pack<<<(unsigned)(want < cap ? want : cap), 256, 0, st>>>(d_ascii, d_descs, first, n_items, g->records, g->pam, g->hdr);
         g_ctx.launches++;
         CUDA_TRY(cudaGetLastError());
-    }
+        k_tile_prefix<<<1, kPrefixThreads, 0, st>>>(g->hdr, g->n_tiles, g->pref);
+        g_ctx.launches++;
+        CUDA_TRY(cudaGetLastError());
+    }
+    CUDA_TRY(cudaMemsetAsync(g->pref + (size_t)g->n_tiles * kPrefWords, 0, sizeof(unsigned int), st));
     CUDA_TRY(cudaEventRecord(g->ev[2], st));
     if (!one && !g->segs.empty()) {
-        const size_t nb = g->segs.size() * sizeof(uint32_t);
-        CUDA_TRY(dev_alloc(&g->d_seg_first, nb, st));
-        CUDA_TRY(dev_alloc(&g->d_seg_count, nb, st));
-        CUDA_TRY(cudaMemcpyAsync(g->d_seg_first, seg_first.data(), nb, cudaMemcpyHostToDevice, st));
-        CUDA_TRY(cudaMemcpyAsync(g->d_seg_count, seg_count.data(), nb, cudaMemcpyHostToDevice, st));
+        const size_t nb = g->segs.size() * sizeof(uint4);
+        CUDA_TRY(dev_alloc(&g->d_seg_geo, nb, st));
+        CUDA_TRY(cudaMemcpyAsync(g->d_seg_geo, seg_geo.data(), nb, cudaMemcpyHostToDevice, st));
     }
     if (g->fasta) g->d_ascii = d_ascii;
     else dev_free(d_ascii, st);
@@ -966,10 +969,10 @@
     dev_free(g->records, st);
     dev_free(g->pam, st);
     dev_free(g->hdr, st);
+    dev_free(g->pref, st);
     dev_free(g->d_ascii, st);
     pinned_put(g->h_bad);
-    dev_free(g->d_seg_first, st);
-    dev_free(g->d_seg_count, st);
+    dev_free(g->d_seg_geo, st);
     for (cudaEvent_t e : g->ev)
         if (e) cudaEventDestroy(e);
     delete g;
@@ -1014,9 +1017,7 @@
 static int plan_scan(const crp_genome *g, bool scored, ScanPlan *p) {
     p->threads = kThreads;
     p->fn = scored ? (const void *)k_scan_score<true> : (const void *)k_scan_score<false>;
-    const unsigned grid_max = (unsigned)g_ctx.sm_count * CRP_CTAS_PER_SM;
-    p->smem = kScanSmemFixed + (size_t)grid_max * sizeof(unsigned long long);
-    static_assert(kScanSmemFixed >= (size_t)kHdrBatch * sizeof(TileHdr), "the count phase stages its tile headers in the emit phase's tile slots");
+    p->smem = kScanSmemFixed;
     static int per_sm_cache[2] = {0, 0};
     int &per_sm = per_sm_cache[scored ? 1 : 0];
     if (per_sm == 0) {
@@ -1041,7 +1042,7 @@
     ScanArgs a;
     a.records = g->records;
     a.pam = g->pam;
-    a.hdr = g->hdr;
+    a.pref = g->pref;
     a.n_tiles = g->n_tiles;
     a.static_eighths = 4;
     if (const char *e = getenv("CRP_STATIC_EIGHTHS")) a.static_eighths = (uint32_t)atoi(e) > 8 ? 8 : (uint32_t)atoi(e);
@@ -1057,14 +1058,19 @@
     a.x_minus = r->x[1];
     const uint32_t n_seg = (uint32_t)g->segs.size();
     unsigned long long *s64 = reinterpret_cast<unsigned long long *>(r->state);
-    a.warp_pref = s64;
-    a.cta_tot = s64 + (size_t)g->n_tiles * kPrefWords;
+    a.zone_pref = s64;
+    a.seg_corr = s64 + (size_t)g->n_tiles * kPrefWords;
+    a.side_corr = a.seg_corr + 2 * (size_t)n_seg;
+    a.edge_done = reinterpret_cast<unsigned int *>(g->pref + (size_t)g->n_tiles * kPrefWords);
     a.seg_counts = r->d_counts;
     a.tickets = reinterpret_cast<unsigned int *>(r->d_counts + 2 * (size_t)r->stride);
     a.n_seg = n_seg;
     a.seg_stride = r->stride;
-    a.seg_first_tile = g->d_seg_first;
-    a.seg_tile_count = g->d_seg_count;
+    a.seg_geo = g->d_seg_geo;
+    for (uint32_t sg = 0; sg < kGeoInline; ++sg) {
+        const Segment *s = sg < n_seg ? &g->segs[sg] : nullptr;
+        a.geo_inline[sg] = s ? make_uint4(s->first_tile, s->n_tiles, (uint32_t)s->begin, (uint32_t)s->token_len) : make_uint4(0u, 0u, 0u, 0u);
+    }
     a.seg_counts_host = r->h_counts;
     a.fault = g_ctx.d_fault;
     a.world = 1;
@@ -1091,8 +1097,24 @@
     }
     CUDA_TRY(cudaEventRecord(r->ev[0], st));
     if (g->n_tiles) {
+        const uint64_t items = 2 * (uint64_t)n_seg, per_cta = kEdgeThreads / 32;
+        uint64_t eg = (items + per_cta - 1) / per_cta;
+        if (eg > (uint64_t)g_ctx.sm_count) eg = (uint64_t)g_ctx.sm_count;
+        k_scan_edges<<<(unsigned)(eg ? eg : 1), kEdgeThreads, 0, st>>>(a);
+        g_ctx.launches++;
+        CUDA_TRY(cudaGetLastError());
+        cudaLaunchAttribute attr[1];
+        attr[0].id = cudaLaunchAttributeProgrammaticStreamSerialization;
+        attr[0].val.programmaticStreamSerializationAllowed = 1;
+        cudaLaunchConfig_t cfg = {};
+        cfg.gridDim = dim3(p.grid);
+        cfg.blockDim = dim3(p.threads);
+        cfg.dynamicSmemBytes = p.smem;
+        cfg.stream = st;
+        cfg.attrs = attr;
+        cfg.numAttrs = 1;
         void *params[] = {(void *)&a};
-        CUDA_TRY(cudaLaunchCooperativeKernel(p.fn, dim3(p.grid), dim3(p.threads), params, p.smem, st));
+        CUDA_TRY(cudaLaunchKernelExC(&cfg, p.fn, params));
         g_ctx.launches++;
         CUDA_TRY(cudaGetLastError());
     } else if (r->fused) {
@@ -1134,12 +1156,12 @@
     ScanPlan plan = {};
     if ((rc = plan_scan(g, r->scored, &plan))) return bail(rc);
     r->stride = slots ? slots : n_seg;
-    r->zero_offset = ((size_t)g->n_tiles * kPrefWords + (size_t)plan.grid) * sizeof(unsigned long long);
-    r->state_bytes = r->zero_offset + 2 * (size_t)r->stride * sizeof(unsigned long long) +
+    r->counts_offset = ((size_t)g->n_tiles * kPrefWords + 5 * (size_t)n_seg) * sizeof(unsigned long long);
+    r->state_bytes = r->counts_offset + 2 * (size_t)r->stride * sizeof(unsigned long long) +
                      4 * sizeof(unsigned int);
     if (dev_alloc(&r->state, r->state_bytes, r->st) != cudaSuccess)
         return bail(fail(CRP_ERR_NOMEM, "cudaMalloc of scan state failed"));
-    r->d_counts = reinterpret_cast<unsigned long long *>(r->state + r->zero_offset);
+    r->d_counts = reinterpret_cast<unsigned long long *>(r->state + r->counts_offset);
     r->h_counts = static_cast<unsigned long long *>(pinned_get((2 * (size_t)r->stride + 1) * sizeof(unsigned long long)));
     if (!r->h_counts) return bail(fail(CRP_ERR_NOMEM, "cudaHostAlloc of the counts failed"));
     if (slots) {
diff --git a/cropsr_b200/csrc/scan.cuh b/cropsr_b200/csrc/scan.cuh
--- a/cropsr_b200/csrc/scan.cuh
+++ b/cropsr_b200/csrc/scan.cuh
@@ -1,12 +1,9 @@
 #pragma once
-#include <cooperative_groups.h>
 #include <cuda_runtime.h>
 #include <stdint.h>
 
 #include "npexp.cuh"
 #include "rs1.cuh"
-
-namespace cg = cooperative_groups;
 
 #ifndef CRP_CTAS_PER_SM
 #define CRP_CTAS_PER_SM 4
@@ -26,7 +23,6 @@
 
 static constexpr int kPamWords = kTileWords + 1;
 static constexpr uint32_t kPamBytes = (16 + kPamWords * 8 + 15) / 16 * 16;
-static constexpr int kCountStages = 6;
 struct __align__(16) TileHdr {
     uint4 desc;
     uint32_t cnt[8];
@@ -34,8 +30,27 @@
 static_assert(sizeof(TileHdr) == 48, "bulk copies move multiples of 16 bytes");
 static constexpr uint32_t kPackItems = 544;
 static_assert(kPackItems % 32 == 0 && kPackItems >= (uint32_t)kRecWords, "whole warps per tile");
-static constexpr int kHdrBatch = 256;
 static_assert(kRecBytes % 16 == 0, "bulk copies move multiples of 16 bytes");
+static constexpr int kPrefixThreads = 512, kPrefixPer = 4;
+static constexpr int kEdgeThreads = 1024;
+static constexpr uint32_t kCorrCache = 64;
+static constexpr uint32_t kGeoInline = 32;
+
+CRP_HD bool tile_in_start_zone(int32_t t0, int l) { return t0 < l + 5; }
+CRP_HD bool tile_in_end_zone(int32_t t0, int32_t L, int l) { return t0 + kTile - 1 > L - l + 7; }
+struct ZoneSpan {
+    uint32_t ns, ne;
+};
+CRP_HD ZoneSpan zone_span(uint32_t begin, uint32_t L, uint32_t c, int l) {
+    ZoneSpan z;
+    const int64_t s = (int64_t)l + 5 - (int64_t)begin;
+    const int64_t ns = s <= 0 ? 0 : (s + kTile - 1) / kTile;
+    const int64_t e = (int64_t)L - l + 9 - kTile - (int64_t)begin;
+    const int64_t ne = e <= 0 ? 0 : (e + kTile - 1) / kTile;
+    z.ns = (uint32_t)(ns < (int64_t)c ? ns : (int64_t)c);
+    z.ne = (uint32_t)(ne < (int64_t)c ? ne : (int64_t)c);
+    return z;
+}
 
 struct TileDesc {
     uint32_t t_start;
@@ -181,6 +196,68 @@
     }
 }
 
+__host__ __device__ inline unsigned long long unpack_counts(uint32_t c) {
+    return ((unsigned long long)(c & 0xFFFFu) << 32) | (c >> 16);
+}
+
+__global__ void __launch_bounds__(kPrefixThreads)
+k_tile_prefix(const TileHdr *__restrict__ hdr, uint32_t nt, unsigned long long *__restrict__ pref) {
+    __shared__ unsigned long long s_warp[kPrefixThreads / 32];
+    const int tid = threadIdx.x, lane = tid & 31, warp = tid >> 5;
+    unsigned long long run = 0;
+    for (uint32_t lo = 0; lo < nt; lo += (uint32_t)(kPrefixThreads * kPrefixPer)) {
+        uint4 c[kPrefixPer][2];
+        unsigned long long mine = 0;
+#pragma unroll
+        for (int p = 0; p < kPrefixPer; ++p) {
+            const uint32_t t = lo + (uint32_t)(tid * kPrefixPer + p);
+            c[p][0] = c[p][1] = make_uint4(0u, 0u, 0u, 0u);
+            if (t < nt) {
+                const uint4 *src = reinterpret_cast<const uint4 *>(hdr[t].cnt);
+                c[p][0] = src[0];
+                c[p][1] = src[1];
+            }
+            mine += unpack_counts(c[p][0].x) + unpack_counts(c[p][0].y) + unpack_counts(c[p][0].z) + unpack_counts(c[p][0].w) +
+                    unpack_counts(c[p][1].x) + unpack_counts(c[p][1].y) + unpack_counts(c[p][1].z) + unpack_counts(c[p][1].w);
+        }
+        unsigned long long incl = mine;
+#pragma unroll
+        for (int o = 1; o < 32; o <<= 1) {
+            const unsigned long long v = __shfl_up_sync(0xFFFFFFFFu, incl, o);
+            if (lane >= o) incl += v;
+        }
+        if (lane == 31) s_warp[warp] = incl;
+        __syncthreads();
+        unsigned long long before = run, total = 0;
+        for (int q = 0; q < kPrefixThreads / 32; ++q) {
+            const unsigned long long x = s_warp[q];
+            if (q < warp) before += x;
+            total += x;
+        }
+        unsigned long long x = before + incl - mine;
+#pragma unroll
+        for (int p = 0; p < kPrefixPer; ++p) {
+            const uint32_t t = lo + (uint32_t)(tid * kPrefixPer + p);
+            if (t < nt) {
+                const uint32_t cc[8] = {c[p][0].x, c[p][0].y, c[p][0].z, c[p][0].w, c[p][1].x, c[p][1].y, c[p][1].z, c[p][1].w};
+                unsigned long long w[kPrefWords];
+#pragma unroll
+                for (int q = 0; q < 8; ++q) {
+                    w[q] = x;
+                    x += unpack_counts(cc[q]);
+                }
+                w[8] = x;
+                w[9] = 0ull;
+                ulonglong2 *dst = reinterpret_cast<ulonglong2 *>(pref + (size_t)t * kPrefWords);
+#pragma unroll
+                for (int q = 0; q < kPrefWords / 2; ++q) dst[q] = make_ulonglong2(w[2 * q], w[2 * q + 1]);
+            }
+        }
+        run += total;
+        __syncthreads();
+    }
+}
+
 struct FastaRec {
     uint64_t raw_off;
     uint64_t ascii_off;
@@ -327,7 +404,7 @@
 struct ScanArgs {
     const uint4 *records;
     const unsigned char *pam;
-    const TileHdr *hdr;
+    const unsigned long long *pref;
     uint32_t n_tiles;
     uint32_t static_eighths;
     int guide_len;
@@ -337,13 +414,16 @@
     uint32_t *pos_plus, *pos_minus;
     unsigned long long *packed_plus, *packed_minus;
     double *x_plus, *x_minus;
-    unsigned long long *warp_pref;
-    unsigned long long *cta_tot;
+    unsigned long long *zone_pref;
+    unsigned long long *seg_corr;
+    unsigned long long *side_corr;
+    unsigned int *edge_done;
     unsigned int *tickets;
     unsigned long long *seg_counts;
     unsigned long long *seg_counts_host;
     unsigned int *fault;
-    const uint32_t *seg_first_tile, *seg_tile_count;
+    const uint4 *seg_geo;
+    uint4 geo_inline[kGeoInline];
     uint32_t n_seg, seg_stride;
     uint32_t world, rank, epoch;
     unsigned long long *peer_gather[kMaxPeers];
@@ -362,6 +442,10 @@
     do {                         \
     } while (0)
 #endif
+
+__device__ __forceinline__ uint4 seg_geometry(const ScanArgs &a, uint32_t sg) {
+    return sg < kGeoInline ? a.geo_inline[sg] : a.seg_geo[sg];
+}
 
 __device__ __forceinline__ void xchg_wait(const ScanArgs &a) {
     if (threadIdx.x < a.world) {
@@ -404,6 +488,115 @@
         asm volatile("mov.u64 %0, %%globaltimer;" : "=l"(t));
         p[8ull * blockIdx.x + slot] = t;
     }
+}
+
+__global__ void __launch_bounds__(kEdgeThreads) k_scan_edges(const ScanArgs a) {
+    asm volatile("griddepcontrol.launch_dependents;" ::: "memory");
+    if (blockIdx.x == 0) dbg_stamp(6);
+    constexpr int kW = kEdgeThreads / 32;
+    __shared__ uint32_t s_cnt[kW][kWarps];
+    __shared__ unsigned long long s_scan[kW];
+    __shared__ unsigned int s_last;
+    __shared__ unsigned long long s_side[3 * (kW / 2)];
+    const bool local = gridDim.x == 1 && a.n_seg <= (uint32_t)(kW / 2);
+    const int tid = threadIdx.x, lane = tid & 31, warp = tid >> 5;
+    const int l = a.guide_len;
+    for (uint32_t item = blockIdx.x * kW + warp; item < 2 * a.n_seg; item += gridDim.x * kW) {
+        const uint32_t sg = item >> 1, side = item & 1u;
+        const uint4 geo = seg_geometry(a, sg);
+        const uint32_t f = geo.x, c = geo.y;
+        unsigned long long run = 0, gi_tot = 0;
+        if (c) {
+            unsigned long long g_lo = 0, g_hi = 0;
+            if (side == 0 && lane == 0) g_lo = __ldg(a.pref + (size_t)f * kPrefWords), g_hi = __ldg(a.pref + (size_t)(f + c - 1) * kPrefWords + kWarps);
+            const ZoneSpan z = zone_span(geo.z, geo.w, c, l);
+            const uint32_t j0 = side ? max(z.ne, z.ns) : 0u, j1 = side ? c : z.ns;
+            for (uint32_t j = j0; j < j1 && j < j0 + 8; ++j) {
+                const unsigned char *rec = a.pam + (size_t)(f + j) * kPamBytes;
+                for (uint32_t o = 128u * lane; o < kPamBytes; o += 32u * 128u) asm volatile("prefetch.global.L2 [%0];" ::"l"(rec + o));
+            }
+            for (uint32_t j = j0; j < j1; ++j) {
+                const uint32_t t = f + j;
+                CRP_CHECK(a, t < a.n_tiles, 5);
+                const unsigned long long *gi = a.pref + (size_t)t * kPrefWords;
+                const unsigned long long g0 = __ldg(gi), g_end = __ldg(gi + kWarps);
+                warp_count_tile(a.pam + (size_t)t * kPamBytes, l, lane, s_cnt[warp]);
+                __syncwarp();
+                const unsigned long long ex = lane < kWarps ? unpack_counts(s_cnt[warp][lane]) : 0ull;
+                unsigned long long incl = ex;
+#pragma unroll
+                for (int o = 1; o < 16; o <<= 1) {
+                    const unsigned long long v = __shfl_up_sync(0xFFFFFFFFu, incl, o);
+                    if (lane >= o) incl += v;
+                }
+                if (lane <= kWarps) a.zone_pref[(size_t)t * kPrefWords + lane] = g0 - run + (incl - ex);
+#ifdef CRP_CHECKED
+                if (lane < kWarps) {
+                    const unsigned long long gc = __ldg(gi + lane + 1) - __ldg(gi + lane);
+                    CRP_CHECK(a, (gc >> 32) >= (ex >> 32) && (gc & 0xFFFFFFFFull) >= (ex & 0xFFFFFFFFull), 6);
+                }
+#endif
+                run += (g_end - g0) - __shfl_sync(0xFFFFFFFFu, incl, kWarps - 1);
+                __syncwarp();
+            }
+            gi_tot = g_hi - g_lo;
+        }
+        if (lane == 0) {
+            a.side_corr[3 * sg + side] = run;
+            if (side == 0) a.side_corr[3 * sg + 2] = gi_tot;
+            if (local) {
+                s_side[3 * sg + side] = run;
+                if (side == 0) s_side[3 * sg + 2] = gi_tot;
+            }
+        }
+    }
+    if (blockIdx.x == 0) dbg_stamp(4);
+
+    if (gridDim.x > 1) {
+        __threadfence();
+        __syncthreads();
+        if (tid == 0) s_last = atomicAdd(a.edge_done, 1u) == gridDim.x - 1;
+        __syncthreads();
+        if (!s_last) return;
+        __threadfence();
+    } else {
+        __syncthreads();
+    }
+    if (tid == 0) {
+        a.tickets[0] = 0;
+        a.tickets[1] = 0;
+        if (gridDim.x > 1) *a.edge_done = 0;
+    }
+    const uint32_t per = (a.n_seg + kEdgeThreads - 1) / kEdgeThreads;
+    const uint32_t s_lo = min(a.n_seg, tid * per), s_hi = min(a.n_seg, s_lo + per);
+    unsigned long long mine = 0;
+    auto side = [&](uint32_t i) { return local ? s_side[i] : __ldcg(a.side_corr + i); };
+    for (uint32_t sg = s_lo; sg < s_hi; ++sg) mine += side(3 * sg) + side(3 * sg + 1);
+    unsigned long long incl = mine;
+#pragma unroll
+    for (int o = 1; o < 32; o <<= 1) {
+        const unsigned long long v = __shfl_up_sync(0xFFFFFFFFu, incl, o);
+        if (lane >= o) incl += v;
+    }
+    if (lane == 31) s_scan[warp] = incl;
+    __syncthreads();
+    unsigned long long before = 0;
+    for (int q = 0; q < warp; ++q) before += s_scan[q];
+    unsigned long long e = before + incl - mine;
+    for (uint32_t sg = s_lo; sg < s_hi; ++sg) {
+        const unsigned long long cs = side(3 * sg), ce = side(3 * sg + 1);
+        a.seg_corr[2 * sg] = e;
+        a.seg_corr[2 * sg + 1] = e + cs;
+        const unsigned long long cnt = side(3 * sg + 2) - cs - ce;
+        e += cs + ce;
+        a.seg_counts[sg] = cnt >> 32;
+        a.seg_counts[a.seg_stride + sg] = cnt & 0xFFFFFFFFull;
+    }
+    for (uint32_t sg = a.n_seg + tid; sg < a.seg_stride; sg += kEdgeThreads) {
+        a.seg_counts[sg] = 0ull;
+        a.seg_counts[a.seg_stride + sg] = 0ull;
+    }
+    dbg_stamp(5);
 }
 
 struct Window {
@@ -436,10 +629,6 @@
     if (t + (kMinus ? 28u : 5u) > L) lo32 |= (uint32_t)CRP_PACKED_TRUNCATED;
     w.packed = ((unsigned long long)hi32 << 32) | lo32;
     return w;
-}
-
-__device__ __forceinline__ unsigned long long unpack_counts(uint32_t c) {
-    return ((unsigned long long)(c & 0xFFFFu) << 32) | (c >> 16);
 }
 
 static constexpr uint32_t kWinBiasPlusHot = kWinBiasPlus - 2u;
@@ -579,17 +768,11 @@
 
 struct __align__(16) Ring {
     unsigned long long pref[kStages][kPrefWords];
-    unsigned long long full[kCountStages];
+    unsigned long long full[kStages];
     unsigned long long pre;
-    unsigned long long rbase[kStages];
-    uint32_t tile[kCountStages];
-    uint32_t done[kCountStages];
+    uint32_t tile[kStages];
 };
-static_assert(kCountStages >= kStages, "the ring control block holds the emit phase's slots");
-
-__device__ __forceinline__ void mbar_inval(unsigned long long *bar) {
-    asm volatile("mbarrier.inval.shared::cta.b64 [%0];" ::"r"(smem_u32(bar)) : "memory");
-}
+
 __device__ __forceinline__ void mbar_arrive(unsigned long long *bar) {
     asm volatile("mbarrier.arrive.shared::cta.b64 _, [%0];" ::"r"(smem_u32(bar)) : "memory");
 }
@@ -601,25 +784,6 @@
                      smem_u32(dst)),
                  "l"(src), "r"(bytes), "r"(smem_u32(bar))
                  : "memory");
-}
-
-__device__ __forceinline__ void ring_reset(Ring &ring, bool first, bool wave_start) {
-    __syncthreads();
-    if (threadIdx.x == 0) {
-#pragma unroll
-        for (int s = 0; s < kCountStages; ++s) {
-            if (!first) mbar_inval(&ring.full[s]);
-            mbar_init(&ring.full[s], 1);
-            ring.done[s] = 0;
-            ring.tile[s] = kNoTile;
-        }
-        if (wave_start) {
-            if (!first) mbar_inval(&ring.pre);
-            mbar_init(&ring.pre, 1);
-        }
-        asm volatile("fence.mbarrier_init.release.cluster;" ::: "memory");
-    }
-    __syncthreads();
 }
 
 template <bool kScore>
@@ -628,139 +792,72 @@
     extern __shared__ __align__(128) unsigned char s_dyn[];
     auto stage = [&](int s) { return reinterpret_cast<uint4 *>(s_dyn + (size_t)s * kRecBytes); };
     uint16_t *const s_list = reinterpret_cast<uint16_t *>(s_dyn + kStages * kRecBytes);
-    unsigned long long *const s_rangepref =
-        reinterpret_cast<unsigned long long *>(s_dyn + kStages * kRecBytes + 2 * (size_t)kListCap * sizeof(uint16_t));
     __shared__ __align__(16) double s_tab[kScore ? RS1_TABLE_DOUBLES : 1];
     __shared__ Ring ring;
-    __shared__ unsigned long long s_scan[kWarps];
-
-    cg::grid_group grid = cg::this_grid();
+    __shared__ __align__(8) unsigned long long s_tabbar;
+    __shared__ unsigned long long s_corr[2 * kCorrCache];
+
     const int tid = threadIdx.x, lane = tid & 31, warp = tid >> 5;
     const int l = a.guide_len;
     const uint32_t G = gridDim.x, cta = blockIdx.x;
+    const uint32_t nt = a.n_tiles;
+    auto record = [&](uint32_t tile) { return a.records + (size_t)tile * kRecWords; };
 
     dbg_stamp(0);
-    __shared__ __align__(8) unsigned long long s_tabbar;
+    const uint32_t ns = (uint32_t)((unsigned long long)nt * a.static_eighths / 8 / G);
+    const bool pre = ns > 0;
+    const uint32_t t_pre = cta;
     if (tid == 0) {
         mbar_init(&s_tabbar, 1);
+#pragma unroll
+        for (int s = 0; s < kStages; ++s) {
+            mbar_init(&ring.full[s], 1);
+            ring.tile[s] = kNoTile;
+        }
+        mbar_init(&ring.pre, 1);
         asm volatile("fence.mbarrier_init.release.cluster;" ::: "memory");
         if (kScore) {
             mbar_expect(&s_tabbar, (uint32_t)kRs1TableBytes);
             bulk_copy(s_tab, a.tables, (uint32_t)kRs1TableBytes, &s_tabbar);
         }
-    }
-
-    auto record = [&](uint32_t tile) { return a.records + (size_t)tile * kRecWords; };
-    const uint32_t nt = a.n_tiles;
-    const uint32_t k = (nt + G - 1) / G;
-
-    const uint32_t r_lo = min(nt, cta * k), n_mine = min(nt, r_lo + k) - r_lo;
-    if (cta == 0 && tid == 0) {
-        a.tickets[0] = 0;
-        a.tickets[1] = 0;
-    }
-    ring_reset(ring, true, true);
+        if (pre) {
+            mbar_expect(&ring.pre, kRecBytes + kPrefWords * 8);
+            bulk_copy(stage(0), record(t_pre), kRecBytes, &ring.pre);
+            bulk_copy(ring.pref[0], a.pref + (size_t)t_pre * kPrefWords, kPrefWords * 8, &ring.pre);
+        }
+    }
+    __syncthreads();
+    asm volatile("griddepcontrol.wait;" ::: "memory");
     dbg_stamp(1);
-    TileHdr *const s_hdr = reinterpret_cast<TileHdr *>(s_dyn);
-    static_assert(kHdrBatch == kThreads, "one tile header per thread");
-    unsigned long long range_run = 0;
-    for (uint32_t h_lo = 0, hb = 0; h_lo < n_mine; h_lo += kHdrBatch, ++hb) {
-        const uint32_t h_n = min(n_mine - h_lo, (uint32_t)kHdrBatch);
-        if (tid == 0) {
-            mbar_expect(&ring.full[0], h_n * (uint32_t)sizeof(TileHdr));
-            bulk_copy(s_dyn, a.hdr + (size_t)(r_lo + h_lo), h_n * (uint32_t)sizeof(TileHdr), &ring.full[0]);
-        }
-        mbar_wait(&ring.full[0], hb & 1u);
-        for (uint32_t j = warp; j < h_n; j += kWarps) {
-            const uint4 d = s_hdr[j].desc;
-            const int32_t t0 = (int32_t)d.x, L = (int32_t)d.y;
-            if (t0 < l + 5 || t0 + kTile - 1 > L - l + 7) {
-                CRP_CHECK(a, r_lo + h_lo + j < nt, 5);
-                CRP_CHECK(a, reinterpret_cast<const uint32_t *>(a.pam + (size_t)(r_lo + h_lo + j) * kPamBytes)[0] == d.x, 6);
-                warp_count_tile(a.pam + (size_t)(r_lo + h_lo + j) * kPamBytes, l, lane, s_hdr[j].cnt);
-            }
-        }
-        __syncthreads();
-        {
-            unsigned long long c[kWarps], mine = 0ull;
-#pragma unroll
-            for (int q = 0; q < kWarps; ++q) {
-                c[q] = (uint32_t)tid < h_n ? unpack_counts(s_hdr[tid].cnt[q]) : 0ull;
-                mine += c[q];
-            }
-            unsigned long long incl = mine;
-#pragma unroll
-            for (int o = 1; o < 32; o <<= 1) {
-                const unsigned long long v = __shfl_up_sync(0xFFFFFFFFu, incl, o);
-                if (lane >= o) incl += v;
-            }
-            if (lane == 31) s_scan[warp] = incl;
+    for (uint32_t i = tid; i < 2 * min(a.n_seg, kCorrCache); i += kThreads) s_corr[i] = __ldcg(a.seg_corr + i);
+    {
+        const bool xchg = a.world > 1;
+        for (uint32_t sg = cta * kThreads + tid; sg < a.seg_stride; sg += G * kThreads) {
+            const unsigned long long plus = __ldcg(a.seg_counts + sg), minus = __ldcg(a.seg_counts + a.seg_stride + sg);
+            if (a.seg_counts_host) {
+                a.seg_counts_host[sg] = plus;
+                a.seg_counts_host[a.seg_stride + sg] = minus;
+            }
+            if (xchg) {
+                CRP_CHECK(a, (size_t)(a.rank + 1) * 2 * a.seg_stride <= (size_t)kMaxPeers * 2 * 32768, 12);
+                const size_t at = (size_t)a.rank * 2 * a.seg_stride + sg;
+                for (uint32_t p = 0; p < a.world; ++p) {
+                    a.peer_gather[p][at] = plus;
+                    a.peer_gather[p][at + a.seg_stride] = minus;
+                }
+            }
+        }
+        if (xchg && cta * kThreads < a.seg_stride) {
+            __threadfence_system();
             __syncthreads();
-            unsigned long long before = range_run, total = 0;
-#pragma unroll
-            for (int q = 0; q < kWarps; ++q) {
-                const unsigned long long x = s_scan[q];
-                if (q < warp) before += x;
-                total += x;
-            }
-            if ((uint32_t)tid < h_n) {
-                unsigned long long *pf = a.warp_pref + (size_t)(r_lo + h_lo + tid) * kPrefWords;
-                unsigned long long run = before + incl - mine;
-#pragma unroll
-                for (int q = 0; q < kWarps; ++q) {
-                    pf[q] = run;
-                    run += c[q];
-                }
-                pf[kWarps] = run;
-                asm volatile("fence.proxy.async.global;" ::: "memory");
-            }
-            range_run += total;
-            __syncthreads();
-        }
-    }
-    if (tid == 0) a.cta_tot[cta] = range_run;
-    const uint32_t ns = (uint32_t)((unsigned long long)nt * a.static_eighths / 8 / G);
-    const bool pre = ns > 0;
-    const uint32_t t_pre = cta;
-    if (pre && tid == 0) {
-        mbar_expect(&ring.pre, kRecBytes + kPrefWords * 8);
-        bulk_copy(stage(0), record(t_pre), kRecBytes, &ring.pre);
-    }
-    dbg_stamp(2);
-    grid.sync();
-    dbg_stamp(3);
-    if (pre && tid == 0) bulk_copy(ring.pref[0], a.warp_pref + (size_t)t_pre * kPrefWords, kPrefWords * 8, &ring.pre);
-
-    {
-        unsigned long long v[4] = {0, 0, 0, 0}, mine = 0;
-#pragma unroll
-        for (int q = 0; q < 4; ++q) {
-            const uint32_t i = 4u * tid + q;
-            if (i < G) v[q] = a.cta_tot[i];
-            mine += v[q];
-        }
-        unsigned long long incl = mine;
-#pragma unroll
-        for (int o = 1; o < 32; o <<= 1) {
-            const unsigned long long x = __shfl_up_sync(0xFFFFFFFFu, incl, o);
-            if (lane >= o) incl += x;
-        }
-        if (lane == 31) s_scan[warp] = incl;
-        __syncthreads();
-        unsigned long long before = 0;
-#pragma unroll
-        for (int q = 0; q < kWarps; ++q) {
-            const unsigned long long x = s_scan[q];
-            if (q < warp) before += x;
-        }
-        unsigned long long run = before + incl - mine;
-#pragma unroll
-        for (int q = 0; q < 4; ++q) {
-            const uint32_t i = 4u * tid + q;
-            if (i < G) s_rangepref[i] = run;
-            run += v[q];
-        }
-    }
+            if (tid == 0) {
+                const uint32_t writers = min(G, (a.seg_stride + kThreads - 1) / kThreads);
+                __threadfence_system();
+                if (atomicAdd(a.tickets + 1, 1u) == writers - 1) xchg_publish(a);
+            }
+        }
+    }
+    __syncthreads();
 
     const uint32_t dyn_lo = ns * G, n_dyn = nt - dyn_lo;
     unsigned int *const ticket = a.tickets;
@@ -774,57 +871,15 @@
         }
         ring.tile[s] = t;
         if (t != kNoTile) {
-            CRP_CHECK(a, t < nt && t / k < G, 11);
-            ring.rbase[s] = s_rangepref[t / k];
+            CRP_CHECK(a, t < nt, 11);
             mbar_expect(&ring.full[s], kRecBytes + kPrefWords * 8);
             bulk_copy(stage(s), record(t), kRecBytes, &ring.full[s]);
-            bulk_copy(ring.pref[s], a.warp_pref + (size_t)t * kPrefWords, kPrefWords * 8, &ring.full[s]);
+            bulk_copy(ring.pref[s], a.pref + (size_t)t * kPrefWords, kPrefWords * 8, &ring.full[s]);
         } else {
             mbar_arrive(&ring.full[s]);
         }
     };
-    ring_reset(ring, false, false);
-    dbg_stamp(4);
     if (kScore) mbar_wait(&s_tabbar, 0);
-    {
-        const bool xchg = a.world > 1;
-        for (uint32_t sg = cta * kThreads + tid; sg < a.seg_stride; sg += G * kThreads) {
-            unsigned long long plus = 0, minus = 0;
-            if (sg < a.n_seg) {
-                const uint32_t f = a.seg_first_tile ? a.seg_first_tile[sg] : 0u;
-                const uint32_t c = a.seg_tile_count ? a.seg_tile_count[sg] : a.n_tiles;
-                if (c) {
-                    const unsigned long long cnt = s_rangepref[(f + c - 1) / k] + a.warp_pref[(size_t)(f + c - 1) * kPrefWords + kWarps] -
-                                                   (s_rangepref[f / k] + a.warp_pref[(size_t)f * kPrefWords]);
-                    plus = cnt >> 32;
-                    minus = cnt & 0xFFFFFFFFull;
-                }
-            }
-            a.seg_counts[sg] = plus;
-            a.seg_counts[a.seg_stride + sg] = minus;
-            if (a.seg_counts_host) {
-                a.seg_counts_host[sg] = plus;
-                a.seg_counts_host[a.seg_stride + sg] = minus;
-            }
-            if (xchg) {
-                CRP_CHECK(a, (size_t)(a.rank + 1) * 2 * a.seg_stride <= (size_t)kMaxPeers * 2 * 32768, 12);
-                const size_t at = (size_t)a.rank * 2 * a.seg_stride + sg;
-                for (uint32_t p = 0; p < a.world; ++p) {
-                    a.peer_gather[p][at] = plus;
-                    a.peer_gather[p][at + a.seg_stride] = minus;
-                }
-            }
-        }
-        if (xchg && cta * kThreads < a.seg_stride) {
-            __threadfence_system();
-            __syncthreads();
-            if (tid == 0) {
-                const uint32_t writers = min(G, (a.seg_stride + kThreads - 1) / kThreads);
-                __threadfence_system();
-                if (atomicAdd(a.tickets + 1, 1u) == writers - 1) xchg_publish(a);
-            }
-        }
-    }
     if (tid == 0) {
         if (pre) mbar_arrive(&ring.full[0]);
         else produce_emit(0, 0);
@@ -840,14 +895,22 @@
         const uint4 *rec = stage(s);
         const uint4 d = rec[0];
         const TileDesc td = {d.x, d.y, d.z, d.w};
-        const unsigned long long tile_pref = ring.pref[s][0];
-        const unsigned long long base = (first_pre ? s_rangepref[t_pre / k] : ring.rbase[s]) + tile_pref;
-        const unsigned long long off = ring.pref[s][warp] - tile_pref;
-        const unsigned long long tot = ring.pref[s][kWarps] - tile_pref;
+        const bool zs = tile_in_start_zone((int32_t)td.t_start, l), zone = zs || tile_in_end_zone((int32_t)td.t_start, (int32_t)td.L, l);
+        unsigned long long p0, pw, pw1, pe;
+        if (zone) {
+            const unsigned long long *z = a.zone_pref + (size_t)(first_pre ? t_pre : ring.tile[s]) * kPrefWords;
+            p0 = __ldcg(z), pw = __ldcg(z + warp), pw1 = __ldcg(z + warp + 1), pe = __ldcg(z + kWarps);
+        } else {
+            p0 = ring.pref[s][0], pw = ring.pref[s][warp], pw1 = ring.pref[s][warp + 1], pe = ring.pref[s][kWarps];
+        }
+        const uint32_t ci = 2 * td.segment + (zs ? 0u : 1u);
+        const unsigned long long base = p0 - (td.segment < kCorrCache ? s_corr[ci] : __ldcg(a.seg_corr + ci));
+        const unsigned long long off = pw - p0;
+        const unsigned long long tot = pe - p0;
         const uint32_t np = (uint32_t)(tot >> 32), nm = (uint32_t)tot;
         const uint32_t base_p = (uint32_t)(base >> 32), base_m = (uint32_t)base;
         const uint32_t wordA = 64 * warp + lane;
-        const bool busy = ring.pref[s][warp + 1] != ring.pref[s][warp];
+        const bool busy = pw1 != pw;
         Hits h = {0u, 0u, 0u, 0u};
         uint32_t epA = 0, emA = 0, epB = 0, emB = 0;
         if (busy) {
@@ -869,7 +932,7 @@
 #ifdef CRP_CHECKED
             {
                 const uint32_t mine = totA + __shfl_sync(0xFFFFFFFFu, iB, 31);
-                const unsigned long long nxt = ring.pref[s][warp + 1] - ring.pref[s][warp];
+                const unsigned long long nxt = pw1 - pw;
                 CRP_CHECK(a, (uint32_t)(nxt >> 32) == (mine & 0xFFFFu) && (uint32_t)nxt == (mine >> 16), 7);
                 if (np <= (uint32_t)kListCap && nm <= (uint32_t)kListCap)
                     CRP_CHECK(a, epA + __popc(h.pA) <= np && epB + __popc(h.pB) <= np && emA + __popc(h.mA) <= nm && emB + __popc(h.mB) <= nm, 10);
@@ -883,6 +946,13 @@
         }
         CRP_CHECK(a, ring.tile[s] == kNoTile || first_pre || ring.tile[s] < nt, 8);
         CRP_CHECK(a, (unsigned long long)base_p + np <= 0xFFFFFFFFull && (unsigned long long)base_m + nm <= 0xFFFFFFFFull, 9);
+        {
+            const uint32_t sg = td.segment, f = seg_geometry(a, sg).x;
+            const unsigned long long lo = a.pref[(size_t)f * kPrefWords] - __ldcg(a.seg_corr + 2 * sg);
+            const unsigned long long c_p = __ldcg(a.seg_counts + sg), c_m = __ldcg(a.seg_counts + a.seg_stride + sg);
+            CRP_CHECK(a, sg < a.n_seg && base_p >= (uint32_t)(lo >> 32) && base_m >= (uint32_t)lo &&
+                             (unsigned long long)base_p + np <= (lo >> 32) + c_p && (unsigned long long)base_m + nm <= (lo & 0xFFFFFFFFull) + c_m, 16);
+        }
 #endif
         if (np <= (uint32_t)kListCap && nm <= (uint32_t)kListCap) {
             if (busy) {
@@ -911,8 +981,9 @@
             }
         }
         __syncthreads();
-    }
-    dbg_stamp(5);
+        if (n == 0) dbg_stamp(2);
+    }
+    dbg_stamp(3);
     if (a.world > 1 && cta == 0) xchg_wait(a);
 }
 
```
